# ThomasZiegler/RS-aware-differential-SfM

Hardware: AMD Instinct MI355X
Metric: Mpixels/sec RS depth+pose solve, 1280x720 pair (higher is better)
Workload: dtype f64

## Files before the change

### include/rsdsfm.h

```cpp
#ifndef RSDSFM_H
#define RSDSFM_H

#include <stddef.h>
#include <stdint.h>

#ifdef __cplusplus
extern "C" {
#endif

#define RSDSFM_OK 0
#define RSDSFM_ERR_INVALID (-1)
#define RSDSFM_ERR_HIP (-2)
#define RSDSFM_ERR_NO_DEVICE (-3)
#define RSDSFM_ERR_NUMERIC (-4)
#define RSDSFM_ERR_PENDING (-5)
#define RSDSFM_ERR_PEER (-6)

#define RSDSFM_DEPTH_CLOSED_FORM 0
#define RSDSFM_DEPTH_CERES_LM 1

#define RSDSFM_K_COMPAT 0
#define RSDSFM_K_FIXED 1

#define RSDSFM_FLOW_COMPAT_RANK 0
// ... 82 lines not shown
                  const double v_in[3], const double w_in[3], double k_in, int const_acceleration,
                  int flow_index_mode, double* inliers_out_3m, double v_out[3], double w_out[3], double* k_out,
                  rsdsfm_lm_summary* summary_or_null);
int rsdsfm_last_ransac_tag(rsdsfm_ctx* ctx, uint64_t* tag, int64_t* cache_hits_or_null);
int rsdsfm_refine_from_ransac(rsdsfm_ctx* ctx, uint64_t ransac_tag, const double* flow2n, int64_t n_flow, int64_t m, const double* inliers_3m,
                              const double* alpha_m, const double* alpha_k_m, const int64_t* inlier_idx_or_null, const double v_in[3],
                              const double w_in[3], double k_in, int const_acceleration, int flow_index_mode, double* inliers_out_3m,
                              double v_out[3], double w_out[3], double* k_out, rsdsfm_lm_summary* summary_or_null);
#define RSDSFM_REFINE_TRACE_COLS 8
#define RSDSFM_TRACE_REJECTED 0.0
#define RSDSFM_TRACE_ACCEPTED 1.0
#define RSDSFM_TRACE_INVALID 2.0
#define RSDSFM_TRACE_PARAMETER_TOL 3.0
#define RSDSFM_TRACE_FUNCTION_TOL 4.0
#define RSDSFM_TRACE_ACCEPTED_GRADIENT_TOL 5.0
int rsdsfm_set_refine_trace(rsdsfm_ctx* ctx, int32_t rows);
int rsdsfm_get_refine_trace(rsdsfm_ctx* ctx, double* trace_rows_x_8, int32_t rows);
int rsdsfm_flatten(rsdsfm_ctx* ctx, const double* flow_img_rows_cols_2, int32_t rows, int32_t cols, double fx,
                   double fy, double cx, double cy, double gamma, double flow_threshold, double* q2n,
                   double* u2n, double* alpha_n, double* alpha_k_n, int64_t* n_out);
int rsdsfm_depth_map(rsdsfm_ctx* ctx, double* inliers_3m_inout, int64_t m, double v_inout[3], double fx,
                     double fy, double cx, double cy, int32_t rows, int32_t cols,
                     double* depth_map_colmajor, int32_t* xs_or_null, int32_t* ys_or_null, int* flipped);
int rsdsfm_pose_table(rsdsfm_ctx* ctx, const double v[3], const double w[3], double k, double gamma,
                      int32_t rows, double* R_rows9, double* t_rows3);

int rsdsfm_estimate_inverse_depths_dev(rsdsfm_ctx* ctx, const double* d_q2n, const double* d_u2n, int64_t n,
                                       const double v[3], const double w[3], double k, const double* d_alpha_n,
                                       const double* d_alpha_k_n, int depth_mode, double* d_inv_depth_n);
int rsdsfm_flatten_dev(rsdsfm_ctx* ctx, const double* d_flow_img, int32_t rows, int32_t cols, double fx, double fy,
                       double cx, double cy, double gamma, double flow_threshold, double* d_q2n, double* d_u2n,
                       double* d_alpha_n, double* d_alpha_k_n, int64_t* n_out);
int rsdsfm_depth_map_dev(rsdsfm_ctx* ctx, double* d_inliers_3m_inout, int64_t m, double v_inout[3], double fx, double fy,
                         double cx, double cy, int32_t rows, int32_t cols, double* d_depth_map_colmajor,
                         int32_t* d_xs_or_null, int32_t* d_ys_or_null, int* flipped);
int rsdsfm_pose_table_dev(rsdsfm_ctx* ctx, const double v[3], const double w[3], double k, double gamma, int32_t rows,
                          double* d_R_rows9, double* d_t_rows3);
typedef struct rsdsfm_frame_params {
    int32_t ransac_trials;
    int32_t use_acceleration_mode;
    int32_t use_refinement;
    int32_t depth_mode;
    int32_t k_sign_mode;
    int32_t flow_index_mode;
    int32_t use_global_shutter_mode;
    int32_t struct_bytes;
    double ransac_tol;
    double flow_threshold;
    uint64_t seed;
} rsdsfm_frame_params;

void rsdsfm_frame_params_init(rsdsfm_frame_params* params);

typedef struct rsdsfm_frame_result {
    int64_t n_points, num_inliers;
    int32_t best_trial, flipped;
    double ransac_w[3], ransac_v[3], ransac_k;
    double w[3], v[3], k;
    rsdsfm_lm_summary refine_summary;
    const double* d_inliers;
    const int64_t* d_inlier_idx;
    const int32_t* d_scanline;
} rsdsfm_frame_result;

int rsdsfm_solve_frame_dev(rsdsfm_ctx* ctx, const double* d_flow_img, int32_t rows, int32_t cols, double fx, double fy,
                           double cx, double cy, double gamma, const rsdsfm_frame_params* params,
                           double* d_depth_map_colmajor, double* d_R_rows9_or_null, double* d_t_rows3_or_null,
                           rsdsfm_frame_result* result);
typedef struct rsdsfm_frame_job {
    const double* d_flow_img;
    int32_t rows, cols;
    double fx, fy, cx, cy, gamma;
    double* d_depth_map_colmajor;
    double* d_R_rows9_or_null;
    double* d_t_rows3_or_null;
    uint64_t seed;
} rsdsfm_frame_job;
int rsdsfm_solve_frames_dev(rsdsfm_ctx* ctx, const rsdsfm_frame_job* jobs, int32_t count, const rsdsfm_frame_params* params,
                            rsdsfm_frame_result* results);
int rsdsfm_set_sequence_lanes(rsdsfm_ctx* ctx, int32_t lanes);
int rsdsfm_set_frame_side_flatten(rsdsfm_ctx* ctx, int mode);
int rsdsfm_set_frame_tail(rsdsfm_ctx* ctx, int mode);
int rsdsfm_set_frame_handoff(rsdsfm_ctx* ctx, int mode);
int rsdsfm_set_frame_predict(rsdsfm_ctx* ctx, int mode);
int rsdsfm_lma_predict_stats(rsdsfm_ctx* ctx, int64_t* hypotheses, int64_t* ended_where_predicted);
int rsdsfm_set_lma_operands(rsdsfm_ctx* ctx, int mode);
int rsdsfm_ransac_dev(rsdsfm_ctx* ctx, const double* d_q2n, const double* d_u2n, const double* d_alpha_n,
                      const double* d_alpha_k_n, int64_t n, int use_alpha_k, int32_t iterations, double tolerance,
                      const int32_t* samples_9xT_or_null, uint64_t seed, int depth_mode, int k_sign_mode,
                      rsdsfm_ransac_out* out);
int rsdsfm_refine_dev(rsdsfm_ctx* ctx, const double* d_flow2n, int64_t n_flow, int64_t m, const double* d_inliers_3m,
                      const double* d_alpha_m, const double* d_alpha_k_m, const int64_t* d_inlier_idx_or_null,
                      const double v_in[3], const double w_in[3], double k_in, int const_acceleration,
                      int flow_index_mode, double* d_inliers_out_3m, double v_out[3], double w_out[3], double* k_out,
                      rsdsfm_lm_summary* summary_or_null);
int rsdsfm_estimate_inverse_depths_batch_dev(rsdsfm_ctx* const* ctxs, int32_t count, const double* const* d_q2n,
                                             const double* const* d_u2n, const int64_t* n, const double* v_count_x3,
                                             const double* w_count_x3, const double* k_count, const double* const* d_alpha_n,
                                             const double* const* d_alpha_k_n, double* const* d_inv_depth_n);
int rsdsfm_depth_lm_batch_launch_dev(rsdsfm_ctx* const* ctxs, int32_t count, const double* const* d_q2n, const double* const* d_u2n,
                                     const int64_t* n, const double* v_count_x3, const double* w_count_x3, const double* k_count,
                                     const double* const* d_alpha_n, const double* const* d_alpha_k_n, double* const* d_inv_depth_n);
int rsdsfm_depth_lm_launch_dev(rsdsfm_ctx* ctx, const double* d_q2n, const double* d_u2n, int64_t n,
                               const double v[3], const double w[3], double k, const double* d_alpha_n,
                               const double* d_alpha_k_n, double* d_inv_depth_n, int launch_id);
int rsdsfm_depth_lm_sums_row_size(void);
int rsdsfm_depth_lm_reduce_dev(rsdsfm_ctx* ctx, int64_t n_shard, double* d_row_out);
int rsdsfm_depth_lm_decide_rows_dev(rsdsfm_ctx* ctx, const double* d_rows, int32_t nrows, int64_t n_total, int launch_id);
int rsdsfm_depth_lm_state(rsdsfm_ctx* ctx, int32_t* status, int32_t* next_launch, rsdsfm_lm_summary* summary_or_null);
int rsdsfm_depth_finish_dev(rsdsfm_ctx* ctx, const double* d_q2n, const double* d_u2n, int64_t n,
                            const double v[3], const double w[3], double k, const double* d_alpha_n,
                            const double* d_alpha_k_n, double* d_inv_depth_n, rsdsfm_lm_summary* summary_or_null,
                            int32_t* extra_launches);

int rsdsfm_flatten_slab_dev(rsdsfm_ctx* ctx, const double* d_img_slab, int32_t rows, int32_t slab_cols, int32_t col0,
                            double fx, double fy, double cx, double cy, double gamma, double thr, double* d_q2n,
                            double* d_u2n, double* d_alpha_n, double* d_alpha_k_n, int64_t* n_out);
int rsdsfm_sample_indices(int64_t n, int32_t iterations, uint64_t seed, int32_t* samples);
int rsdsfm_minimal9_dev(rsdsfm_ctx* ctx, const double* d_q9, const double* d_u9, const double* d_alpha9,
                        const double* d_alpha_k9, int32_t count, int use_alpha_k, int k_sign_mode, double* d_hyp);
int rsdsfm_minimal9_probe_dev(rsdsfm_ctx* ctx, const double* d_q9, const double* d_u9, const double* d_alpha9, const double* d_alpha_k9,
                              int32_t count, int use_alpha_k, int k_sign_mode, int use_cores, double* d_hyp, double* d_probe4);
size_t rsdsfm_tile_lm_state_bytes(void);
size_t rsdsfm_tile_best_bytes(void);
int32_t rsdsfm_tile_ransac_row_size(void);
int32_t rsdsfm_tile_ransac_batch(void);
int rsdsfm_tile_ransac_lm_rows_dev(rsdsfm_ctx* ctx, const double* d_q2n, const double* d_u2n, const double* d_alpha_n,
                                   const double* d_alpha_k_n, int64_t n_shard, const double* d_hyp, int32_t count,
                                   const void* d_states, int32_t round, double tolerance, double* d_rows);
int rsdsfm_tile_ransac_decide_dev(rsdsfm_ctx* ctx, const double* d_rows_all, int32_t nranks, int32_t count, void* d_states,
                                  int64_t n_total, int32_t round, int32_t* d_flags, int32_t* d_scored, double* d_trial_count,
                                  double* d_trial_err);
int rsdsfm_tile_ransac_score_rows_dev(rsdsfm_ctx* ctx, const double* d_q2n, const double* d_u2n, const double* d_alpha_n,
                                      const double* d_alpha_k_n, int64_t n_shard, const double* d_hyp, int32_t count,
                                      const void* d_states, int depth_mode, double tolerance, const int32_t* d_scored_or_null,
                                      double* d_rows);
int rsdsfm_tile_ransac_score_merge_dev(rsdsfm_ctx* ctx, const double* d_rows_all, int32_t nranks, int32_t count,
                                       const int32_t* d_scored_or_null, double* d_trial_count, double* d_trial_err);
int rsdsfm_tile_ransac_pick_dev(rsdsfm_ctx* ctx, const double* d_trial_count, const double* d_trial_err, int32_t iterations,
                                const double* d_hyp, void* d_best);
int rsdsfm_tile_ransac_final_dev(rsdsfm_ctx* ctx, const double* d_q2n, const double* d_u2n, const double* d_alpha_n,
                                 const double* d_alpha_k_n, int64_t n_shard, void* d_best, const void* d_states, int depth_mode,
                                 double tolerance, double* d_inv_depth_n, uint8_t* d_mask_n, int64_t* d_inlier_idx,
                                 double* d_inliers3m, double* d_out_alpha, double* d_out_alpha_k, rsdsfm_ransac_out* out);
int64_t rsdsfm_tile_ransac_global_inliers(rsdsfm_ctx* ctx, const void* d_best);
int rsdsfm_tile_refine_begin_dev(rsdsfm_ctx* ctx, const double* d_flow2n, int64_t n_flow, int64_t m_shard, const double* d_inl3m,
                                 const double* d_alpha_m, const double* d_alpha_k_m, const int64_t* d_inlier_idx,
                                 const double v_in[3], const double w_in[3], double k_in, int const_acceleration,
                                 int flow_index_mode);
int32_t rsdsfm_tile_refine_row_size(int const_acceleration, int32_t stage);
int rsdsfm_tile_refine_rows_dev(rsdsfm_ctx* ctx, int32_t stage, double* d_row);
int rsdsfm_tile_refine_apply_dev(rsdsfm_ctx* ctx, int32_t stage, const double* d_rows_all, int32_t nranks, int64_t m_total);
int rsdsfm_tile_refine_poll(rsdsfm_ctx* ctx, double v_out[3], double w_out[3], double* k_out, rsdsfm_lm_summary* summary);
int rsdsfm_tile_refine_finish_dev(rsdsfm_ctx* ctx, double* d_inl_out3m);
int rsdsfm_tile_zsum_dev(rsdsfm_ctx* ctx, const double* d_inl3m, int64_t m_shard, double* d_zsum1);
int rsdsfm_tile_depth_map_dev(rsdsfm_ctx* ctx, double* d_inl3m, int64_t m_shard, const double* d_zsums_all, int32_t nranks,
                              int64_t m_total, double v_inout[3], double fx, double fy, double cx, double cy, int32_t rows,
                              int32_t col0, int32_t slab_cols, double* d_depth_slab, int32_t* d_xs_or_null,
                              int32_t* d_ys_or_null, int* flipped);

#define RSDSFM_DIST_ID_BYTES 128
int rsdsfm_dist_unique_id(void* id_128_bytes);
int rsdsfm_dist_init(rsdsfm_ctx* ctx, int32_t nranks, int32_t rank, const void* id_128_bytes);
int rsdsfm_dist_adopt(rsdsfm_ctx* ctx, void* nccl_comm, int32_t nranks, int32_t rank);
typedef int (*rsdsfm_all_gather_fn)(void* user, const void* d_send, void* d_recv, size_t bytes_per_rank, void* hip_stream);
typedef int (*rsdsfm_all_reduce_sum_f64_fn)(void* user, double* d_buf, size_t count, void* hip_stream);
// ... 78 lines not shown
```

### rs-aware-differential-sfm_amd/csrc/capi.hip

```cpp
#include <string.h>

#include <algorithm>
#include <new>
#include <vector>

#include <chrono>
#include <thread>

#include "rsdsfm_internal.hpp"

namespace rsdsfm {

int fail(Ctx* c, int code, const char* msg) {
    if (c) c->err = msg;
    return code;
}

int ensure_stage(Ctx* c, size_t bytes) {
    c->stage_gen += 1;
    if (bytes <= c->stage_bytes) return RSDSFM_OK;
    RSDSFM_HIP_CHECK(c, hipStreamSynchronize(c->stream));
    if (c->d_stage) RSDSFM_HIP_CHECK(c, hipFree(c->d_stage));
    c->d_stage = nullptr;
    c->stage_bytes = 0;
// ... 126 lines not shown
              hipHostMalloc(reinterpret_cast<void**>(&c->h_lm), sizeof(LmState), hipHostMallocDefault) == hipSuccess &&
              hipMemset(c->d_tickets, 0, sizeof(unsigned) * 64) == hipSuccess &&
              hipMemset(c->d_lm, 0, sizeof(LmState)) == hipSuccess;
    if (ok) {
        memset(c->h_lm, 0, sizeof(LmState));
        c->h_lm->predict = 1;
        c->h_lm->status = 1;
        ok = hipMemcpy(c->d_lm, c->h_lm, sizeof(LmState), hipMemcpyHostToDevice) == hipSuccess;
    }
    if (!ok) {
        rsdsfm_destroy(ctx);
        return RSDSFM_ERR_HIP;
    }
    *out = ctx;
    return RSDSFM_OK;
}

void rsdsfm_destroy(rsdsfm_ctx* ctx) {
    if (!ctx) return;
    Ctx* c = &ctx->c;
    DeviceGuard device_guard_(c);
    (void)hipSetDevice(c->device);
    if (c->stream) (void)hipStreamSynchronize(c->stream);
    frame_release(c);
    flow_release(c);
    flow_check_release(c);
    rectify_dense_release(c);
    link_release(c);
    fuse_release(c);
    last_frame_release(c);
    if (c->d_partials) (void)hipFree(c->d_partials);
    if (c->d_tickets) (void)hipFree(c->d_tickets);
    if (c->d_lm) (void)hipFree(c->d_lm);
    if (c->h_lm) (void)hipHostFree(c->h_lm);
    if (c->d_stage) (void)hipFree(c->d_stage);
    if (c->d_ws) (void)hipFree(c->d_ws);
    if (c->d_frame) (void)hipFree(c->d_frame);
    if (c->d_tile) (void)hipFree(c->d_tile);
    if (c->d_refine_trace) (void)hipFree(c->d_refine_trace);
    if (c->d_core_flag) (void)hipFree(c->d_core_flag);
    delete static_cast<RefineBuffers*>(c->tile_session);
    if (c->h_pinned) (void)hipHostFree(c->h_pinned);
    dist_release(c);
    for (unsigned* p : c->d_claim)
        if (p) (void)hipFree(p);
    if (c->ev_ready) (void)hipEventDestroy(c->ev_ready);
    for (hipEvent_t e : c->ev_prof)
        if (e) (void)hipEventDestroy(e);
    if (c->d_clk_probe) (void)hipFree(c->d_clk_probe);
    if (c->d_lma_list) (void)hipFree(c->d_lma_list);
    if (c->own_stream && c->stream) (void)hipStreamDestroy(c->stream);
    delete ctx;
}

const char* rsdsfm_last_error(const rsdsfm_ctx* ctx) { return ctx ? ctx->c.err.c_str() : "null context"; }

int rsdsfm_synchronize(rsdsfm_ctx* ctx) {
    CTX_OR_FAIL(ctx);
    RSDSFM_HIP_CHECK(c, hipStreamSynchronize(c->stream));
    return RSDSFM_OK;
}

int rsdsfm_set_depth_variant(rsdsfm_ctx* ctx, int variant) {
    CTX_OR_FAIL(ctx);
    if (variant < 0 || variant > 3) return fail(c, RSDSFM_ERR_INVALID, "depth variant must be 0 (default), 1 (LDS-DMA), 2 (decision fused into launch 0) or 3 (separate decide kernel)");
    RSDSFM_HIP_CHECK(c, hipStreamSynchronize(c->stream));
    c->depth_variant = variant;
    return RSDSFM_OK;
}

int rsdsfm_set_profiling(rsdsfm_ctx* ctx, int on) {
    CTX_OR_FAIL(ctx);
    if (on && !c->ev_prof[0]) {
        RSDSFM_HIP_CHECK(c, hipEventCreate(&c->ev_prof[0]));
        RSDSFM_HIP_CHECK(c, hipEventCreate(&c->ev_prof[1]));
        RSDSFM_HIP_CHECK(c, hipMalloc((void**)&c->d_clk_probe, 4 * sizeof(unsigned long long)));
        RSDSFM_HIP_CHECK(c, hipMemsetAsync(c->d_clk_probe, 0, 4 * sizeof(unsigned long long), c->stream));
    }
    c->profile = on != 0;
    c->prof_pending = false;
    return RSDSFM_OK;
}

int rsdsfm_profile_last_ms(rsdsfm_ctx* ctx, const char* what, double* ms) {
    CTX_OR_FAIL(ctx);
    if (what && ms && !strncmp(what, "refine_rf_phase", 15) && ((what[15] >= '0' && what[15] <= '9') || (what[15] >= 'a' && what[15] <= 'f')) && !what[16]) {
        static unsigned long long h[16];
        if (what[15] == '0') {
            int rc = refine_rf_read_stamps(c, h);
            if (rc != RSDSFM_OK) return fail(c, RSDSFM_ERR_INVALID, "no phase stamps: set RSDSFM_RF_STAMPS=1 before the first refinement");
        }
        const int k = what[15] <= '9' ? what[15] - '0' : what[15] - 'a' + 10;
        *ms = k == 4 ? (double)h[4] : k >= 8 ? (double)(long long)(h[k] - h[8]) * 0.01 : (double)h[k] * 0.01;
        return RSDSFM_OK;
    }
    const bool clock = what && !strcmp(what, "ransac_lm_round0_clock_mhz");
    const int which = !what ? -1 : clock || !strcmp(what, "ransac_lm_round0") ? 0 : !strcmp(what, "depth_lm_batch") ? 1 : -1;
    if (which < 0 || !ms)
        return fail(c, RSDSFM_ERR_INVALID, "unknown profile record (known: \"ransac_lm_round0\", \"ransac_lm_round0_clock_mhz\", \"depth_lm_batch\")");
    if (!c->prof_pending || c->prof_what != which)
        return fail(c, RSDSFM_ERR_INVALID, "no such profile record: enable rsdsfm_set_profiling and run a RANSAC (LM mode) / a batched dense depth solve first");
    RSDSFM_HIP_CHECK(c, hipEventSynchronize(c->ev_prof[1]));
    if (clock) {
        unsigned long long h[4];
        RSDSFM_HIP_CHECK(c, hipMemcpyAsync(h, c->d_clk_probe, sizeof(h), hipMemcpyDeviceToHost, c->stream));
        RSDSFM_HIP_CHECK(c, hipStreamSynchronize(c->stream));
        if (h[3] <= h[1] || h[2] <= h[0]) return fail(c, RSDSFM_ERR_INVALID, "the bracketed launch left no clock stamps");
        *ms = (double)(h[2] - h[0]) * 100.0 / (double)(h[3] - h[1]);
        return RSDSFM_OK;
    }
    float f = 0.f;
    RSDSFM_HIP_CHECK(c, hipEventElapsedTime(&f, c->ev_prof[0], c->ev_prof[1]));
    *ms = (double)f;
    return RSDSFM_OK;
}

int rsdsfm_set_refine_trace(rsdsfm_ctx* ctx, int32_t rows) {
    CTX_OR_FAIL(ctx);
    if (rows < 0 || rows > 4096) return fail(c, RSDSFM_ERR_INVALID, "refine trace: 0 <= rows <= 4096");
    if (rows != c->refine_trace_rows) {
        RSDSFM_HIP_CHECK(c, hipStreamSynchronize(c->stream));
        if (c->d_refine_trace) RSDSFM_HIP_CHECK(c, hipFree(c->d_refine_trace));
        c->d_refine_trace = nullptr;
        c->refine_trace_rows = 0;
        if (rows > 0) {
            RSDSFM_HIP_CHECK(c, hipMalloc((void**)&c->d_refine_trace, (size_t)rows * kRefineTraceCols * sizeof(double)));
            c->refine_trace_rows = rows;
        }
    }
    if (c->d_refine_trace)
        RSDSFM_HIP_CHECK(c, hipMemsetAsync(c->d_refine_trace, 0xFF, (size_t)rows * kRefineTraceCols * sizeof(double), c->stream));
    return RSDSFM_OK;
}

int rsdsfm_get_refine_trace(rsdsfm_ctx* ctx, double* out, int32_t rows) {
    CTX_OR_FAIL(ctx);
    if (!out || rows < 1) return fail(c, RSDSFM_ERR_INVALID, "refine trace: null output or rows < 1");
    if (!c->d_refine_trace) return fail(c, RSDSFM_ERR_INVALID, "no refine trace: call rsdsfm_set_refine_trace(ctx, rows) before the refinement");
    if (rows > c->refine_trace_rows) return fail(c, RSDSFM_ERR_INVALID, "refine trace: more rows requested than rsdsfm_set_refine_trace reserved");
    RSDSFM_HIP_CHECK(c, hipMemcpyAsync(out, c->d_refine_trace, (size_t)rows * kRefineTraceCols * sizeof(double), hipMemcpyDeviceToHost, c->stream));
    RSDSFM_HIP_CHECK(c, hipStreamSynchronize(c->stream));
    return RSDSFM_OK;
}

int rsdsfm_set_ransac_speculation(rsdsfm_ctx* ctx, int k0) {
    CTX_OR_FAIL(ctx);
    if (k0 != 0 && k0 != 2 && k0 != KMAX) return fail(c, RSDSFM_ERR_INVALID, "ransac speculation depth must be 0 (automatic, default), 2 or 3");
    c->ransac_k0 = k0;
    return RSDSFM_OK;
}

int rsdsfm_set_ransac_math(rsdsfm_ctx* ctx, int mode) {
    CTX_OR_FAIL(ctx);
    if (mode < 0 || mode > 1) return fail(c, RSDSFM_ERR_INVALID, "ransac math: 0 = in-range function cores with restart (default), 1 = standard functions");
    c->ransac_math_mode = mode;
    return RSDSFM_OK;
}

int rsdsfm_ransac_restarts(rsdsfm_ctx* ctx, int64_t* count) {
    CTX_OR_FAIL(ctx);
    if (!count) return fail(c, RSDSFM_ERR_INVALID, "ransac restarts: null output");
    int64_t total = c->ransac_restarts;
    for (rsdsfm_ctx* lane : c->lanes) total += lane->c.ransac_restarts;
    *count = total;
    return RSDSFM_OK;
}

int rsdsfm_set_lm_arithmetic(rsdsfm_ctx* ctx, int mode) {
    CTX_OR_FAIL(ctx);
    if (mode < 0 || mode > 2)
        return fail(c, RSDSFM_ERR_INVALID, "LM arithmetic: 0 = analytic trajectory with guards (default), 1 = iterate by iterate, 2 = 0 with the frame solve's count-only pass forced");
    c->lm_arithmetic = mode == 1 ? 1 : 0;
    c->lma_count_only_force = mode == 2;
    c->lma_hold = c->lma_unique_run = 0;
    dist_reset_hold(c);
    for (rsdsfm_ctx* lane : c->lanes)
        lane->c.lm_arithmetic = c->lm_arithmetic, lane->c.lma_count_only_force = c->lma_count_only_force, lane->c.lma_hold = lane->c.lma_unique_run = 0;
    return RSDSFM_OK;
}

int rsdsfm_lma_count_only(rsdsfm_ctx* ctx, int64_t* runs, int64_t* lazy_runs) {
    CTX_OR_FAIL(ctx);
    if (!runs) return fail(c, RSDSFM_ERR_INVALID, "lma count only: null output");
    int64_t a = c->lma_count_only_runs, b = c->lma_lazy_runs;
    for (rsdsfm_ctx* lane : c->lanes) a += lane->c.lma_count_only_runs, b += lane->c.lma_lazy_runs;
    *runs = a;
    if (lazy_runs) *lazy_runs = b;
    return RSDSFM_OK;
}

int rsdsfm_lma_predict_stats(rsdsfm_ctx* ctx, int64_t* hypotheses, int64_t* ended_where_predicted) {
    CTX_OR_FAIL(ctx);
    if (!hypotheses || !ended_where_predicted) return fail(c, RSDSFM_ERR_INVALID, "lma predict stats: null output");
    int64_t h = 0, e = 0;
    auto add = [&](Ctx* x) -> int {
        if (!x->d_core_flag) return RSDSFM_OK;
        DeviceGuard guard(x);
        unsigned long long w[2] = {0, 0};
        RSDSFM_HIP_CHECK(c, hipStreamSynchronize(x->stream));
        RSDSFM_HIP_CHECK(c, hipMemcpy(w, x->d_core_flag + 4, sizeof(w), hipMemcpyDeviceToHost));
        h += (int64_t)w[0], e += (int64_t)w[1];
        return RSDSFM_OK;
    };
    int rc = add(c);
    for (rsdsfm_ctx* lane : c->lanes)
        if (rc == RSDSFM_OK) rc = add(&lane->c);
    if (rc != RSDSFM_OK) return rc;
    *hypotheses = h;
    *ended_where_predicted = e;
    return RSDSFM_OK;
}

int rsdsfm_lma_restarts(rsdsfm_ctx* ctx, int64_t* count, int32_t* last_guards) {
    CTX_OR_FAIL(ctx);
    if (!count) return fail(c, RSDSFM_ERR_INVALID, "lma restarts: null output");
    int64_t total = c->lma_restarts;
    int guards = c->lma_last_guard;
    for (rsdsfm_ctx* lane : c->lanes) total += lane->c.lma_restarts, guards |= lane->c.lma_last_guard;
    *count = total;
    if (last_guards) *last_guards = guards;
    return RSDSFM_OK;
}

int rsdsfm_set_refine_arithmetic(rsdsfm_ctx* ctx, int mode) {
    CTX_OR_FAIL(ctx);
    if (mode != 0 && mode != 1) return fail(c, RSDSFM_ERR_INVALID, "refine arithmetic: 0 = radius-factorised (default), 1 = iterate by iterate");
    c->refine_arithmetic = mode;
    for (rsdsfm_ctx* lane : c->lanes) lane->c.refine_arithmetic = mode;
    return RSDSFM_OK;
}

int rsdsfm_refine_restarts(rsdsfm_ctx* ctx, int64_t* runs, int64_t* restarts, int64_t* resolves_or_null, int32_t* last_guard_or_null) {
    CTX_OR_FAIL(ctx);
    if (!runs || !restarts) return fail(c, RSDSFM_ERR_INVALID, "refine restarts: null output");
    int64_t n = c->refine_rf_runs, r = c->refine_rf_restarts, s = c->refine_rf_resolves;
    int guard = c->refine_rf_last_guard;
    for (rsdsfm_ctx* lane : c->lanes) {
        n += lane->c.refine_rf_runs, r += lane->c.refine_rf_restarts, s += lane->c.refine_rf_resolves;
        if (lane->c.refine_rf_last_guard) guard = lane->c.refine_rf_last_guard;
    }
    *runs = n, *restarts = r;
    if (resolves_or_null) *resolves_or_null = s;
    if (last_guard_or_null) *last_guard_or_null = guard;
    return RSDSFM_OK;
}

int rsdsfm_depth_restarts(rsdsfm_ctx* ctx, int64_t* count) {
    CTX_OR_FAIL(ctx);
    if (!count) return fail(c, RSDSFM_ERR_INVALID, "depth restarts: null output");
    *count = c->depth_restarts;
    return RSDSFM_OK;
}

int rsdsfm_set_true_flow_search(rsdsfm_ctx* ctx, int mode) {
    CTX_OR_FAIL(ctx);
    if (mode < 0 || mode > 2) return fail(c, RSDSFM_ERR_INVALID, "true-flow search mode: 0 = automatic, 1 = exhaustive, 2 = interval-pruned");
    c->true_flow_exhaustive = mode;
    return RSDSFM_OK;
}

const char* rsdsfm_kernel_name(const char* entry_point) {
    if (!entry_point) return "";
    if (!strcmp(entry_point, "estimate_inverse_depths_lm")) return RSDSFM_FUSED ? "depth_lm_kernel<1, false>" : "depth_lm_kernel<1, true>";
    if (!strcmp(entry_point, "estimate_inverse_depths_closed_form")) return "depth_closed_form_kernel";
    return "";
}

int rsdsfm_estimate_inverse_depths_dev(rsdsfm_ctx* ctx, const double* d_q, const double* d_u, int64_t n,
                                       const double v[3], const double w[3], double k, const double* d_alpha,
                                       const double* d_alpha_k, int depth_mode, double* d_rho) {
    CTX_OR_FAIL(ctx);
    if (n < 0 || !v || !w) return fail(c, RSDSFM_ERR_INVALID, "bad arguments");
    if (n > 0 && (!d_q || !d_u || !d_alpha || !d_alpha_k || !d_rho)) return fail(c, RSDSFM_ERR_INVALID, "null device pointer");
    if (!aligned_to(16, d_q, d_u, d_alpha, d_alpha_k, d_rho)) return fail(c, RSDSFM_ERR_INVALID, "device pointers must be 16-byte aligned");
    Pose pose;
    memcpy(pose.v, v, sizeof(pose.v));
    memcpy(pose.w, w, sizeof(pose.w));
    pose.k = k;
    if (depth_mode == RSDSFM_DEPTH_CLOSED_FORM) return depth_closed_form_launch(c, d_q, d_u, d_alpha, d_alpha_k, n, pose, d_rho);
    if (depth_mode != RSDSFM_DEPTH_CERES_LM) return fail(c, RSDSFM_ERR_INVALID, "unknown depth_mode");
    if (c->depth_variant == 2) {
        int rcf = depth_lm_fused_launch(c, d_q, d_u, d_alpha, d_alpha_k, n, pose, d_rho);
        if (rcf != RSDSFM_OK) return rcf;
        rcf = depth_lm_launch(c, d_q, d_u, d_alpha, d_alpha_k, n, pose, d_rho, 1);
        c->lm_issued_k = 2;
        c->lm_issued_d = 1;
        return rcf;
    }
    if (depth_lma_allowed(c, n)) {
        Ctx* cs1[1] = {c};
        const double *q1[1] = {d_q}, *u1[1] = {d_u}, *a1[1] = {d_alpha}, *ak1[1] = {d_alpha_k};
        double* r1[1] = {d_rho};
        int rc0 = depth_lma_batch_launch(cs1, 1, q1, u1, a1, ak1, &n, &pose, r1);
        c->lm_issued_k = 1;
        c->lm_issued_d = 1;
        return rc0;
    }
    if (c->depth_variant == 0) {
        int rc0 = depth_lm_launch(c, d_q, d_u, d_alpha, d_alpha_k, n, pose, d_rho, 0, true);
        if (rc0 != RSDSFM_OK) return rc0;
        rc0 = depth_lm_decide_apply_launch(c, d_q, d_u, d_alpha, d_alpha_k, n, pose, d_rho);
        c->lm_issued_k = 1;
        c->lm_issued_d = 1;
        return rc0;
    }
    int rc = depth_lm_launch(c, d_q, d_u, d_alpha, d_alpha_k, n, pose, d_rho, 0);
    if (rc != RSDSFM_OK) return rc;
    rc = depth_lm_decide_launch(c, n, 0);
    if (rc != RSDSFM_OK) return rc;
    rc = depth_lm_launch(c, d_q, d_u, d_alpha, d_alpha_k, n, pose, d_rho, 1);
    c->lm_issued_k = 2;
    c->lm_issued_d = 1;
    return rc;
}

static int depth_batch_common(rsdsfm_ctx* const* ctxs, int32_t count, const double* const* d_q, const double* const* d_u, const int64_t* n,
                              const double* v3, const double* w3, const double* k, const double* const* d_alpha,
                              const double* const* d_alpha_k, double* const* d_rho, int launch0_only) {
    if (!ctxs || count < 1 || !ctxs[0]) return RSDSFM_ERR_INVALID;
    Ctx* c = &ctxs[0]->c;
    DeviceGuard device_guard_(c);
    if (count > kDepthBatchMax) return fail(c, RSDSFM_ERR_INVALID, "at most 8 solves per batched launch");
    if (!d_q || !d_u || !n || !v3 || !w3 || !k || !d_alpha || !d_alpha_k || !d_rho) return fail(c, RSDSFM_ERR_INVALID, "null argument array");
    Ctx* cs[kDepthBatchMax];
    Pose poses[kDepthBatchMax];
    for (int i = 0; i < count; ++i) {
// ... 238 lines not shown
```

### rs-aware-differential-sfm_amd/csrc/frame_host.hip

```cpp
#include <stdlib.h>
#include <string.h>

#include <atomic>

#include <algorithm>
#include <new>

#include "rsdsfm_internal.hpp"
#include "sequence_host.hpp"

namespace rsdsfm {

static std::atomic<int> g_frames_in_flight[64];
int frames_in_flight(const Ctx* c) { return g_frames_in_flight[c->device & 63].load(std::memory_order_relaxed); }

int alpha_ones_launch(Ctx* c, double* d_alpha, int64_t n);
int flatten_device(Ctx* c, const double* d_img, int32_t rows, int32_t cols, int32_t col0, double fx, double fy, double cx, double cy, double gamma,
                   double thr, double* d_q, double* d_u, double* d_alpha, double* d_alpha_k, int64_t* n_out);

struct FrameRun {
    rsdsfm_frame_job job;
    rsdsfm_frame_params prm;
    size_t N = 0;
    int64_t n = 0;
// ... 124 lines not shown
                RSDSFM_HIP_CHECK(c, hipMalloc(reinterpret_cast<void**>(&c->d_flat_counters), 2 * sizeof(unsigned long long)));
                RSDSFM_HIP_CHECK(c, hipMemsetAsync(c->d_flat_counters, 0, 2 * sizeof(unsigned long long), c->stream));
            }
            F->dense = DenseFlatten();
            F->dense.thr = prm->flow_threshold;
            F->dense.d_q = F->d_q, F->dense.d_u = F->d_u, F->dense.d_alpha = F->d_a, F->dense.d_alpha_k = F->d_ak;
            F->dense.d_counters = c->d_flat_counters;
            F->dense.total_out = count_host(c);
            F->dense_in_launch = true;
        } else if (side == 2) {
            F->join = [c, F, d_flat_counts, d_flat_offsets]() -> int {
                const rsdsfm_frame_job& J2 = F->job;
                int rc2 = flatten_launch(c, J2.d_flow_img, J2.rows, J2.cols, 0, J2.fx, J2.fy, J2.cx, J2.cy, J2.gamma, F->prm.flow_threshold, F->d_q, F->d_u, F->d_a,
                                         F->d_ak, d_flat_counts, d_flat_offsets, count_host(c), nullptr);
                if (rc2 == RSDSFM_OK && F->prm.use_global_shutter_mode) rc2 = alpha_ones_launch(c, F->d_a, (int64_t)F->N);
                return rc2;
            };
        } else if (side == 1) {
            rc = ensure_side_stream(c);
            if (rc != RSDSFM_OK) return rc;
            RSDSFM_HIP_CHECK(c, hipEventRecord(c->ev_fork, c->stream));
            RSDSFM_HIP_CHECK(c, hipStreamWaitEvent(c->aux_stream, c->ev_fork, 0));
            {
                StreamSwap on_side(c, c->aux_stream);
                rc = flatten_launch(c, J.d_flow_img, rows, cols, 0, fx, fy, cx, cy, gamma, prm->flow_threshold, F->d_q, F->d_u, F->d_a, F->d_ak,
                                    d_flat_counts, d_flat_offsets, count_host(c), nullptr);
                if (rc == RSDSFM_OK && prm->use_global_shutter_mode) rc = alpha_ones_launch(c, F->d_a, n);
            }
            if (rc != RSDSFM_OK) return rc;
            RSDSFM_HIP_CHECK(c, hipEventRecord(c->ev_join, c->aux_stream));
            F->join = [c]() -> int {
                RSDSFM_HIP_CHECK(c, hipStreamWaitEvent(c->stream, c->ev_join, 0));
                return RSDSFM_OK;
            };
        } else {
            rc = flatten_enqueue(c, J.d_flow_img, rows, cols, fx, fy, cx, cy, gamma, prm->flow_threshold, F->d_q, F->d_u, F->d_a, F->d_ak, count_host(c));
            if (rc != RSDSFM_OK) return rc;
        }
    } else {
        rc = flatten_device(c, J.d_flow_img, rows, cols, 0, fx, fy, cx, cy, gamma, prm->flow_threshold, F->d_q, F->d_u, F->d_a, F->d_ak, &n);
        if (rc != RSDSFM_OK) return rc;
        *count_host(c) = n;
    }
    if (prm->use_global_shutter_mode && !F->side_flatten) {
        rc = alpha_ones_launch(c, F->d_a, n);
        if (rc != RSDSFM_OK) return rc;
    }
    F->n = n;
    memset(&F->ro, 0, sizeof(F->ro));
    F->ro.inlier_idx = F->d_idx;
    F->ro.inliers = F->d_inl;
    F->ro.alpha = F->d_in_a;
    F->ro.alpha_k = F->d_in_ak;
    F->ro.mask = F->d_mask;
    F->m_known = -1;
    F->tail = [c, F](const RefineBuffers& B) -> int {
        const rsdsfm_frame_job& J2 = F->job;
        const RefineState* st = B.state;
        const int64_t m_arg = F->m_known >= 0 ? F->m_known : F->n;
        const int64_t* m_dev = F->m_known >= 0 ? nullptr : &st->m;
        PoseTableOut pt;
        if (J2.d_R_rows9_or_null && J2.d_t_rows3_or_null)
            pt.R = J2.d_R_rows9_or_null, pt.t = J2.d_t_rows3_or_null, pt.rows = J2.rows, pt.gamma = J2.gamma, pt.wk_dev = st->p + 3;
        if (B.claim.on)
            return depth_map_decided_launch(c, F->d_inl_ref, m_arg, F->d_zpartials, refine_finish_grid(c, B), B, J2.d_depth_map_colmajor, F->d_zheader,
                                            header_host(c), st->p, m_dev, &pt);
        return depth_map_slab_launch(c, F->d_inl_ref, m_arg, F->d_zpartials, refine_finish_grid(c, B), m_arg, nullptr, J2.fx, J2.fy, J2.cx, J2.cy, J2.rows,
                                     0, J2.cols, J2.d_depth_map_colmajor, nullptr, F->d_ys, F->d_zheader, header_host(c), st->p, m_dev, &pt);
    };
    F->claim = FinishClaim();
    if (c->frame_tail == 0) {
        F->claim.on = true;
        F->claim.fx = J.fx, F->claim.fy = J.fy, F->claim.cx = J.cx, F->claim.cy = J.cy;
        F->claim.rows = rows, F->claim.cols = cols;
        F->claim.ys = F->d_ys;
    }
    F->spec_tail = [c, F](const RansacBest* d_best) -> int {
        return refine_begin(c, F->d_u, F->n, F->n, F->d_inl, F->d_in_a, F->d_in_ak, F->d_idx, nullptr, nullptr, 0.0, F->prm.use_acceleration_mode,
                            F->prm.flow_index_mode, F->d_inl_ref, &F->tail, d_best, F->d_refine_ws, &F->refine, state_host(c), F->d_zpartials, false,
                            &F->claim, F->ransac.direct_final ? &F->ransac.handoff : nullptr);
    };
    F->refinement_enqueued = false;
    F->ahead = prm->use_refinement && c->ransac_spec_miss < 2;
    F->d_local_idx = (c->frame_handoff == 0 && F->ahead && F->claim.on && c->lm_arithmetic == 0 && c->refine_arithmetic == 0 && !c->refine_stage_separate)
                         ? d_local_idx : nullptr;
    F->open = true;
    g_frames_in_flight[c->device & 63].fetch_add(1, std::memory_order_relaxed);
    F->counted = true;
    F->rc_begin = ransac_begin(c, F->d_q, F->d_u, F->d_a, F->d_ak, n, prm->use_acceleration_mode, prm->ransac_trials, prm->ransac_tol, nullptr, J.seed,
                               prm->depth_mode, prm->k_sign_mode, &F->ro, prm->use_refinement ? &F->spec_tail : nullptr, &F->refinement_enqueued, &F->ransac,
                               F->side_flatten ? &F->direct : nullptr, F->side_flatten && !F->dense_in_launch ? &F->join : nullptr,
                               F->dense_in_launch ? &F->dense : nullptr, F->ahead, true,
                               F->claim.on && prm->use_refinement ? refine_flag_words(F->d_refine_ws) : nullptr, F->d_local_idx);
    return RSDSFM_OK;
}

int frame_finish(Ctx* c, FrameRun* F, rsdsfm_frame_result* res) {
    if (!F->open) return fail(c, RSDSFM_ERR_INVALID, "no frame solve in flight");
    F->open = false;
    FrameInFlightEnd in_flight_end_{c, F};
    const rsdsfm_frame_job& J = F->job;
    const rsdsfm_frame_params* prm = &F->prm;
    memset(res, 0, sizeof(*res));
    int rc = F->rc_begin;
    if (rc == RSDSFM_OK) rc = ransac_finish(c, &F->ransac);
    if (rc != RSDSFM_OK) RSDSFM_HIP_CHECK(c, hipStreamSynchronize(c->stream));
    if (F->side_flatten && c->aux_stream) RSDSFM_HIP_CHECK(c, hipStreamSynchronize(c->aux_stream));
    int64_t n = F->n;
    if (*count_host(c) < 0) {
        c->frame_dense_hint = 1;
        return rc != RSDSFM_OK ? rc : fail(c, RSDSFM_ERR_NUMERIC, "frame solve: the point count did not arrive");
    }
    bool counted = true;
    if (*count_host(c) != n) {
        if (F->dense_in_launch) {
            int64_t n_real = 0;
            rc = flatten_device(c, J.d_flow_img, J.rows, J.cols, 0, J.fx, J.fy, J.cx, J.cy, J.gamma, prm->flow_threshold, F->d_q, F->d_u, F->d_a, F->d_ak, &n_real);
            if (rc == RSDSFM_OK && prm->use_global_shutter_mode) rc = alpha_ones_launch(c, F->d_a, n_real);
            if (rc != RSDSFM_OK) return rc;
            *count_host(c) = n_real;
        }
        n = *count_host(c);
        F->n = n;
        F->refinement_enqueued = false;
        counted = false;
        rc = ransac_begin(c, F->d_q, F->d_u, F->d_a, F->d_ak, n, prm->use_acceleration_mode, prm->ransac_trials, prm->ransac_tol, nullptr, J.seed,
                          prm->depth_mode, prm->k_sign_mode, &F->ro, prm->use_refinement ? &F->spec_tail : nullptr, &F->refinement_enqueued, &F->ransac, nullptr, nullptr,
                          nullptr, F->ahead, true,
                               F->claim.on && prm->use_refinement ? refine_flag_words(F->d_refine_ws) : nullptr, F->d_local_idx);
        if (rc == RSDSFM_OK) rc = ransac_finish(c, &F->ransac);
        counted = rc == RSDSFM_OK;
    }
    c->frame_dense_hint = n == (int64_t)F->N ? 1 : 0;
    if (rc != RSDSFM_OK) return rc;
    if (counted) ransac_commit_hints(c, F->ransac);
    const rsdsfm_ransac_out& ro = F->ro;
    res->n_points = n;
    res->num_inliers = ro.num_inliers;
    res->best_trial = ro.best_trial;
    memcpy(res->ransac_w, ro.w, sizeof(ro.w));
    memcpy(res->ransac_v, ro.v, sizeof(ro.v));
    res->ransac_k = ro.k;
    double v[3], w[3], k = ro.k;
    for (int i = 0; i < 3; ++i) v[i] = ro.v[i], w[i] = ro.w[i];
    double* d_final = F->d_inl;
    int flipped = 0;
    F->m_known = ro.num_inliers;
    if (prm->use_refinement) {
        bool exact = false;
        if (F->refinement_enqueued) {
            rc = refine_poll(c, &F->refine, v, w, &k, &res->refine_summary);
            exact = rc == kRcRefineRestartExact;
        }
        if ((!F->refinement_enqueued || exact) && F->ransac.direct_final) {
            rc = ransac_scatter_launch(c, F->ransac.handoff);
            if (rc != RSDSFM_OK) return rc;
            F->ransac.direct_final = false;
        }
        if (!F->refinement_enqueued || exact)
            rc = refine_device(c, F->d_u, n, ro.num_inliers, F->d_inl, F->d_in_a, F->d_in_ak, F->d_idx, v, w, k, prm->use_acceleration_mode,
                               prm->flow_index_mode, F->d_inl_ref, v, w, &k, &res->refine_summary, &F->tail, F->d_zpartials, exact, &F->claim);
        if (rc != RSDSFM_OK) return rc;
        d_final = F->d_inl_ref;
        const double* h_header = header_host(c);
        flipped = h_header[0] != 0.0;
        v[0] = h_header[1], v[1] = h_header[2], v[2] = h_header[3];
    } else {
        rc = depth_map_device(c, d_final, ro.num_inliers, v, J.fx, J.fy, J.cx, J.cy, J.rows, J.cols, J.d_depth_map_colmajor, nullptr, F->d_ys, &flipped, w,
                              k, J.gamma, J.d_R_rows9_or_null, J.d_t_rows3_or_null);
        if (rc != RSDSFM_OK) return rc;
    }
    res->flipped = flipped;
    memcpy(res->v, v, sizeof(v));
    memcpy(res->w, w, sizeof(w));
    res->k = k;
    res->d_inliers = d_final;
    res->d_inlier_idx = F->d_idx;
    res->d_scanline = F->d_ys;
    return RSDSFM_OK;
}

FrameRun* frame_run_of(Ctx* c) {
    if (!c->frame_run) c->frame_run = new (std::nothrow) FrameRun();
    return static_cast<FrameRun*>(c->frame_run);
}

}

void frame_release(Ctx* c) {
    frame_uncount(c, static_cast<FrameRun*>(c->frame_run));
    delete static_cast<FrameRun*>(c->frame_run);
    c->frame_run = nullptr;
    for (rsdsfm_ctx* lane : c->lanes) rsdsfm_destroy(lane);
    c->lanes.clear();
    if (c->ev_fork) (void)hipEventDestroy(c->ev_fork);
    if (c->ev_join) (void)hipEventDestroy(c->ev_join);
    if (c->ev_seq) (void)hipEventDestroy(c->ev_seq);
    if (c->aux_stream) (void)hipStreamDestroy(c->aux_stream);
    if (c->d_flat_counters) (void)hipFree(c->d_flat_counters);
    c->d_flat_counters = nullptr;
    c->ev_fork = c->ev_join = c->ev_seq = nullptr;
    c->aux_stream = nullptr;
}

}

using namespace rsdsfm;

extern "C" {

void rsdsfm_frame_params_init(rsdsfm_frame_params* p) {
    if (!p) return;
    memset(p, 0, sizeof(*p));
    p->ransac_trials = 5;
    p->use_acceleration_mode = 0;
    p->use_refinement = 1;
    p->depth_mode = RSDSFM_DEPTH_CERES_LM;
    p->k_sign_mode = RSDSFM_K_COMPAT;
    p->flow_index_mode = RSDSFM_FLOW_COMPAT_RANK;
    p->use_global_shutter_mode = 0;
    p->struct_bytes = (int32_t)sizeof(rsdsfm_frame_params);
    p->ransac_tol = 0.05;
    p->flow_threshold = 1e-10;
    p->seed = 1;
}

int rsdsfm_solve_frame_dev(rsdsfm_ctx* ctx, const double* d_flow_img, int32_t rows, int32_t cols, double fx, double fy, double cx,
                           double cy, double gamma, const rsdsfm_frame_params* prm, double* d_depth_map, double* d_R_rows9,
                           double* d_t_rows3, rsdsfm_frame_result* res) {
    if (!ctx) return RSDSFM_ERR_INVALID;
    Ctx* c = &ctx->c;
    DeviceGuard device_guard_(c);
    if (!prm || !res) return fail(c, RSDSFM_ERR_INVALID, "bad arguments");
    FrameRun* F = frame_run_of(c);
// ... 1 lines not shown
    F->prm = *prm;
    F->job = rsdsfm_frame_job{d_flow_img, rows, cols, fx, fy, cx, cy, gamma, d_depth_map, d_R_rows9, d_t_rows3, prm->seed};
    int rc = frame_begin(c, F);
    if (rc != RSDSFM_OK) return rc;
    return frame_finish(c, F, res);
}

int rsdsfm_set_sequence_lanes(rsdsfm_ctx* ctx, int32_t lanes) {
    if (!ctx) return RSDSFM_ERR_INVALID;
    Ctx* c = &ctx->c;
    DeviceGuard device_guard_(c);
    if (lanes < 0 || lanes > 16) return fail(c, RSDSFM_ERR_INVALID, "lanes must be 0 (default) .. 16");
    c->seq_lanes = lanes;
    return RSDSFM_OK;
}

int rsdsfm_set_frame_tail(rsdsfm_ctx* ctx, int mode) {
    if (!ctx) return RSDSFM_ERR_INVALID;
    if (mode < 0 || mode > 1) return fail(&ctx->c, RSDSFM_ERR_INVALID, "mode must be 0 (short launch tail) or 1 (stage-by-stage launches)");
    ctx->c.frame_tail = mode;
    return RSDSFM_OK;
}

int rsdsfm_set_frame_handoff(rsdsfm_ctx* ctx, int mode) {
    if (!ctx) return RSDSFM_ERR_INVALID;
    if (mode < 0 || mode > 1) return fail(&ctx->c, RSDSFM_ERR_INVALID, "mode must be 0 (the first refinement pass gathers its inliers) or 1 (the compaction launch)");
    ctx->c.frame_handoff = mode;
    return RSDSFM_OK;
}

int rsdsfm_set_frame_predict(rsdsfm_ctx* ctx, int mode) {
    if (!ctx) return RSDSFM_ERR_INVALID;
    if (mode < 0 || mode > 2) return fail(&ctx->c, RSDSFM_ERR_INVALID, "mode must be 0 (the pixel pass fuses each hypothesis' predicted iterate), 1 (the two-iterate pass) or 2 (0 with the prediction inverted)");
    ctx->c.frame_predict = mode;
    for (rsdsfm_ctx* lane : ctx->c.lanes) lane->c.frame_predict = mode;
    return RSDSFM_OK;
}

int rsdsfm_set_lma_operands(rsdsfm_ctx* ctx, int mode) {
    if (!ctx) return RSDSFM_ERR_INVALID;
    if (mode < 0 || mode > 2) return fail(&ctx->c, RSDSFM_ERR_INVALID, "mode must be 0 (the pixel pass stages each pixel's operands once per workgroup), 1 (every lane loads its pixel's operands) or 2 (0 for every hypothesis count)");
    ctx->c.lma_operands = mode;
    for (rsdsfm_ctx* lane : ctx->c.lanes) lane->c.lma_operands = mode;
    return RSDSFM_OK;
}

int rsdsfm_set_frame_side_flatten(rsdsfm_ctx* ctx, int mode) {
    if (!ctx) return RSDSFM_ERR_INVALID;
    if (mode < 0 || mode > 3) return fail(&ctx->c, RSDSFM_ERR_INVALID, "mode must be 0 (flatten first), 1 (flatten on a second stream), 2 (flatten behind the minimal solver) or 3 (flatten inside the solver's launch)");
    ctx->c.frame_side_flatten = mode;
    return RSDSFM_OK;
}

}

namespace rsdsfm {

int sequence_lane_count(const Ctx* c, int count) { return std::max(1, std::min<int>(count, c->seq_lanes > 0 ? c->seq_lanes : kSequenceLanesDefault)); }

int solve_frames_run(Ctx* c, const rsdsfm_frame_job* jobs, int32_t count, const rsdsfm_frame_params* prm, rsdsfm_frame_result* results, const PairHook* hook) {
    const int L = sequence_lane_count(c, count);
    while ((int)c->lanes.size() < L - 1) {
        rsdsfm_ctx* lane = nullptr;
        int rc = rsdsfm_create(&lane, c->device, nullptr);
        if (rc != RSDSFM_OK) return fail(c, rc, "could not create a sequence lane");
        c->lanes.push_back(lane);
    }
    auto lane_ctx = [&](int l) -> Ctx* { return l == 0 ? c : &c->lanes[(size_t)l - 1]->c; };
    if (L > 1) {
        if (!c->ev_seq) RSDSFM_HIP_CHECK(c, hipEventCreateWithFlags(&c->ev_seq, hipEventDisableTiming));
        RSDSFM_HIP_CHECK(c, hipEventRecord(c->ev_seq, c->stream));
    }
    for (int l = 1; l < L; ++l) {
        Ctx* lc = lane_ctx(l);
        RSDSFM_HIP_CHECK(c, hipStreamWaitEvent(lc->stream, c->ev_seq, 0));
        lc->ransac_k0 = c->ransac_k0;
        lc->ransac_math_mode = c->ransac_math_mode;
        lc->lm_arithmetic = c->lm_arithmetic;
        lc->refine_arithmetic = c->refine_arithmetic;
        lc->lma_count_only_force = c->lma_count_only_force;
        lc->frame_side_flatten = c->frame_side_flatten;
        lc->frame_tail = c->frame_tail;
        lc->frame_handoff = c->frame_handoff;
        lc->frame_predict = c->frame_predict;
        lc->lma_operands = c->lma_operands;
        lc->refine_stage_mode = c->refine_stage_mode;
    }
    for (int l = 0; l < L; ++l) lane_ctx(l)->refine_stage_separate = L > 1;
    int first_error = RSDSFM_OK;
    int in_flight[16];
    for (int l = 0; l < 16; ++l) in_flight[l] = -1;
    auto finish_lane = [&](int l) {
        const int i = in_flight[l];
        if (i < 0) return;
        in_flight[l] = -1;
        Ctx* lc = lane_ctx(l);
        int rc = frame_finish(lc, static_cast<FrameRun*>(lc->frame_run), &results[i]);
        if (rc != RSDSFM_OK && first_error == RSDSFM_OK) {
            first_error = rc;
            if (lc != c) c->err = "pair " + std::to_string(i) + ": " + lc->err;
        }
        if (rc == RSDSFM_OK && hook && first_error == RSDSFM_OK) {
            rc = (*hook)(lc, i, static_cast<FrameRun*>(lc->frame_run)->job, results[i]);
            if (rc != RSDSFM_OK) {
                first_error = rc;
                c->err = "pair " + std::to_string(i) + ": " + std::string(lc->err);
            }
        }
    };
    for (int i = 0; i < count && first_error == RSDSFM_OK; ++i) {
        const int l = i % L;
        finish_lane(l);
        if (first_error != RSDSFM_OK) break;
        Ctx* lc = lane_ctx(l);
        FrameRun* F = frame_run_of(lc);
        if (!F) {
            first_error = fail(c, RSDSFM_ERR_INVALID, "out of host memory");
            break;
        }
        F->prm = *prm;
        F->job = jobs[i];
        int rc = frame_begin(lc, F);
        if (rc != RSDSFM_OK) {
            first_error = rc;
            if (lc != c) c->err = "pair " + std::to_string(i) + ": " + lc->err;
            break;
        }
        in_flight[l] = i;
    }
    for (;;) {
        int best = -1;
        for (int l = 0; l < L; ++l)
            if (in_flight[l] >= 0 && (best < 0 || in_flight[l] < in_flight[best])) best = l;
        if (best < 0) break;
        finish_lane(best);
    }
    for (int l = 0; l < L; ++l) lane_ctx(l)->refine_stage_separate = false;
    return first_error;
}

}

extern "C" {

int rsdsfm_solve_frames_dev(rsdsfm_ctx* ctx, const rsdsfm_frame_job* jobs, int32_t count, const rsdsfm_frame_params* prm, rsdsfm_frame_result* results) {
    if (!ctx) return RSDSFM_ERR_INVALID;
    Ctx* c = &ctx->c;
    DeviceGuard device_guard_(c);
    if (count < 0 || !prm || (count > 0 && (!jobs || !results))) return fail(c, RSDSFM_ERR_INVALID, "bad arguments");
    if (count == 0) return RSDSFM_OK;
    for (int32_t i = 0; i < count; ++i)
        if (frame_job_check_aligned(c, jobs[i]) != RSDSFM_OK) return RSDSFM_ERR_INVALID;
    return solve_frames_run(c, jobs, count, prm, results, nullptr);
}

int rsdsfm_set_refine_stage(rsdsfm_ctx* ctx, int mode) {
    if (!ctx) return RSDSFM_ERR_INVALID;
    Ctx* c = &ctx->c;
    if (mode < 0 || mode > 2) return fail(c, RSDSFM_ERR_INVALID, "refine stage: 0 (automatic), 1 (in the next pass's prologue) or 2 (a launch of its own)");
    c->refine_stage_mode = mode;
    return RSDSFM_OK;
}

}
```

### rs-aware-differential-sfm_amd/csrc/refine_common.hpp

```cpp
#pragma once
#include "device_math.hpp"
#include "rsdsfm_internal.hpp"

namespace rsdsfm {
namespace {


constexpr int kFB = 512;
constexpr int kWorkgroupsPerCu = 1;

struct PassShape {
    int64_t m;
    int grid;
    bool live;
};
__device__ __forceinline__ PassShape pass_shape(const RefineState* __restrict__ st, int64_t m_arg) {
    PassShape ps;
    if (m_arg >= 0) {
        ps.m = m_arg, ps.grid = (int)gridDim.x, ps.live = true;
    } else {
        ps.m = st->m, ps.grid = st->grid, ps.live = (int)blockIdx.x < ps.grid;
    }
    return ps;
}
// ... 215 lines not shown
    __syncthreads();
    (void)s_red;
}

template <int NA, int NB>
__device__ __forceinline__ bool reduce_two_ranges_groups(const double* __restrict__ rows, int nblocks, int stride, int offA, int maxA, bool doA,
                                                         double (*s_grpA)[NA], int offB, int maxB, bool doB, double (*s_grpB)[NB], int tid) {
    using SA = ReduceShape<NA>;
    using SB = ReduceShape<NB>;
    static_assert(SA::W == 2 && SB::W == 2, "slot pairs");
    constexpr int U = 16;
    if (nblocks > U * SA::G || nblocks > U * SB::G) return false;
    const int gA = tid / SA::NH, spA = tid - gA * SA::NH, gB = tid / SB::NH, spB = tid - gB * SB::NH;
    const bool onA = doA && gA < SA::G, onB = doB && gB < SB::G;
    double2 vA[U], vB[U];
#pragma unroll
    for (int j = 0; j < U; ++j) {
        const int bj = gA + j * SA::G;
        vA[j] = (onA && bj < nblocks) ? reinterpret_cast<const double2*>(rows + (int64_t)bj * stride + offA)[spA] : make_double2(0.0, 0.0);
    }
#pragma unroll
    for (int j = 0; j < U; ++j) {
        const int bj = gB + j * SB::G;
        vB[j] = (onB && bj < nblocks) ? reinterpret_cast<const double2*>(rows + (int64_t)bj * stride + offB)[spB] : make_double2(0.0, 0.0);
    }
    if (onA) {
        const bool mx0 = (2 * spA == maxA), mx1 = (2 * spA + 1 == maxA);
        double a0 = 0.0, a1 = 0.0;
#pragma unroll
        for (int j = 0; j < U; ++j) {
            a0 = mx0 ? fmax(a0, vA[j].x) : a0 + vA[j].x;
            a1 = mx1 ? fmax(a1, vA[j].y) : a1 + vA[j].y;
        }
        s_grpA[gA][2 * spA] = a0;
        s_grpA[gA][2 * spA + 1] = a1;
    }
    if (onB) {
        const bool mx0 = (2 * spB == maxB), mx1 = (2 * spB + 1 == maxB);
        double a0 = 0.0, a1 = 0.0;
#pragma unroll
        for (int j = 0; j < U; ++j) {
            a0 = mx0 ? fmax(a0, vB[j].x) : a0 + vB[j].x;
            a1 = mx1 ? fmax(a1, vB[j].y) : a1 + vB[j].y;
        }
        s_grpB[gB][2 * spB] = a0;
        s_grpB[gB][2 * spB + 1] = a1;
    }
    return true;
}

template <int NP>
struct Counts {
    static constexpr int TRI = NP * (NP + 1) / 2;
    static constexpr int NINIT = 1 + NP + NP + 1 + 1 + 1;
    static constexpr int INIT_MAX = 1 + 2 * NP;
    static constexpr int NSCHUR = 2 * TRI + 2 * NP;
    static constexpr int NBACK = 3 + 1 + NP + 1 + 1 + 1 + 1;
    static constexpr int BACK_MAX = 3 + 1 + NP;
};

template <int NP>
struct SlotRow {
    using CT = Counts<NP>;
    static constexpr int OFF_BACK = CT::NSCHUR;
    static constexpr int NW = CT::NSCHUR + CT::NBACK + ((CT::NBACK & 1) ? 1 : 0);
    static constexpr bool SPECULATES = NP == 6;
};


__device__ __forceinline__ double uniform_d(double x) {
    const int lo = __builtin_amdgcn_readfirstlane(__double2loint(x)), hi = __builtin_amdgcn_readfirstlane(__double2hiint(x));
    return __hiloint2double(hi, lo);
}

__device__ __forceinline__ void state_to_lds(RefineState* s_st, const RefineState* __restrict__ st_in) {
    static_assert(sizeof(RefineState) % 8 == 0 && sizeof(RefineState) / 8 <= kFB, "copied as 8-byte words, one per thread");
    if (threadIdx.x < sizeof(RefineState) / 8) reinterpret_cast<double*>(s_st)[threadIdx.x] = reinterpret_cast<const double*>(st_in)[threadIdx.x];
    __syncthreads();
}
__device__ __forceinline__ void state_from_lds(RefineState* __restrict__ st_out, const RefineState* s_st) {
    if (threadIdx.x < sizeof(RefineState) / 8) reinterpret_cast<double*>(st_out)[threadIdx.x] = reinterpret_cast<const double*>(s_st)[threadIdx.x];
}

}
}
```

### rs-aware-differential-sfm_amd/csrc/refine_host.hip

```cpp
#include <string.h>

#include <algorithm>

#include "rsdsfm_internal.hpp"

namespace rsdsfm {

int refine_begin(Ctx* c, const double* d_flow, int64_t n_flow, int64_t m, const double* d_inl, const double* d_alpha,
                 const double* d_alpha_k, const int64_t* d_inlier_idx, const double v_in[3], const double w_in[3], double k_in,
                 int const_acceleration, int flow_index_mode, double* d_inl_out, const RefineTail* tail, const RansacBest* d_best,
                 void* ws_base, RefineRun* run, RefineState* hs_prefetch, double* d_zpartials, bool exact, const FinishClaim* claim,
                 const FrameHandoff* handoff) {
    const bool direct = handoff && handoff->local_idx;
    if (m < 0 || n_flow < 0 || (!d_best && (!v_in || !w_in))) return fail(c, RSDSFM_ERR_INVALID, "bad arguments");
    if (flow_index_mode != RSDSFM_FLOW_COMPAT_RANK && flow_index_mode != RSDSFM_FLOW_GATHERED) return fail(c, RSDSFM_ERR_INVALID, "unknown flow_index_mode");
    if (flow_index_mode == RSDSFM_FLOW_GATHERED && m > 0 && !d_inlier_idx) return fail(c, RSDSFM_ERR_INVALID, "gathered mode needs inlier_idx");
    if (m > 0 && (!d_flow || !d_inl || !d_alpha || !d_alpha_k || !d_inl_out)) return fail(c, RSDSFM_ERR_INVALID, "null device pointer");
    const int np = const_acceleration ? 7 : 6;
    const size_t M = (size_t)std::max<int64_t>(m, 1);
    const size_t npart = (size_t)(d_best ? refine_partials_doubles_cap(c) : refine_partials_doubles(c, m));
    int rc = RSDSFM_OK;
    if (!ws_base) {
        rc = ensure_ws(c, refine_workspace_bytes(c, m, d_best != nullptr));
        if (rc != RSDSFM_OK) return rc;
        ws_base = c->d_ws;
    }
    rc = ensure_pinned(c, sizeof(RefineState) + 64);
    if (rc != RSDSFM_OK) return rc;
    Arena ws(ws_base);
    RefineBuffers& B = run->B;
    B = RefineBuffers();
    B.flow = d_flow;
    B.n_flow = n_flow;
    B.m = m;
    B.m_on_device = d_best != nullptr;
    B.inl = d_inl;
    B.alpha = d_alpha;
    B.alpha_k = d_alpha_k;
    B.inlier_idx = d_inlier_idx;
    B.flow_index_mode = flow_index_mode;
    static_assert(sizeof(RefineState) % sizeof(int) == 0, "flag follows the state");
    char* state_block = ws.take<char>(sizeof(RefineState) + 64);
    B.state = reinterpret_cast<RefineState*>(state_block);
    B.uu = ws.take<double>(4 * M);
    B.beta = ws.take<double>(M);
    B.rho_a = ws.take<double>(M);
    B.rho_b = ws.take<double>(M);
    B.srho = ws.take<double>(M);
    B.partials = ws.take<double>(npart);
    B.bad_index = reinterpret_cast<int*>(state_block + sizeof(RefineState));
    B.zpartials = d_zpartials;
    if (claim && claim->on && d_zpartials) B.claim = *claim;
    run->np = np;
    run->rf = !exact && c->lm_arithmetic == 0 && c->refine_arithmetic == 0;
    if (run->rf) c->refine_rf_runs += 1;
    run->d_inl_out = d_inl_out;
    run->tail = tail;
    run->launched = 0;
    run->hint_prev = c->refine_iters_hint;
    run->hs = hs_prefetch ? hs_prefetch : static_cast<RefineState*>(c->h_pinned);
    run->prefetch = hs_prefetch != nullptr;
    run->prefetched = false;
    B.state_host = hs_prefetch;
    if (d_best && claim && claim->on && run->rf && !c->refine_stage_separate) {
        B.best_dev = d_best;
        if (direct) {
            B.handoff = *handoff;
            B.fin_xy = B.uu, B.fin_stride = 4;
        }
    } else if (direct) {
        return fail(c, RSDSFM_ERR_INVALID, "refinement: direct hand-off without the start state in the first pass");
    } else if (d_best) {
        rc = refine_state_from_best_launch(c, d_best, B, np);
        if (rc != RSDSFM_OK) return rc;
    } else {
        RefineState* hs = static_cast<RefineState*>(c->h_pinned);
        int* h_bad = reinterpret_cast<int*>(static_cast<char*>(c->h_pinned) + sizeof(RefineState));
        memset(hs, 0, sizeof(RefineState));
        hs->np = np;
        for (int i = 0; i < 3; ++i) {
            hs->p[i] = v_in[i];
            hs->p[3 + i] = w_in[i];
        }
        hs->p[6] = k_in;
        hs->termination = -1;
        hs->radius = kInitialRadius;
        hs->need_schur = 1;
        memset(h_bad, 0, kRefineStateBlockTail);
        RSDSFM_HIP_CHECK(c, hipMemcpyAsync(B.state, hs, sizeof(RefineState) + kRefineStateBlockTail, hipMemcpyHostToDevice, c->stream));
    }
    rc = refine_trace_reset(c);
    if (rc != RSDSFM_OK) return rc;
    if (!run->rf) {
        rc = refine_init_launch(c, B, np);
        if (rc != RSDSFM_OK) return rc;
    }
    const int hp = run->hint_prev;
    run->chunk = (hp >= 0 && hp <= 3) ? hp + 1 : (hp > 8 ? std::min(hp + 1, 28) : 7);
    return refine_enqueue_chunk(c, run);
}

int refine_enqueue_chunk(Ctx* c, RefineRun* run) {
    static const bool watch = getenv("RSDSFM_SYNC_WATCHDOG_S") != nullptr;
    if (watch) {
        const RefineBuffers B = run->B;
        const int launched = run->launched, chunk = run->chunk, rf = run->rf ? 1 : 0;
        set_sync_dumper([B, launched, chunk, rf](Ctx* cc) {
            fprintf(stderr, "[rsdsfm] last refinement chunk enqueued: slots [%d, %d), radius-factorised %d\n", launched, launched + chunk, rf);
            refine_rf_debug_dump(cc, B);
        });
    }
    if (run->rf) {
        for (int i = 0; i <= run->chunk; ++i) {
            const int g = run->launched + i;
            int rc = refine_rf_pass_launch(c, run->B, run->np, g, run->launched, nullptr, 0, -1, nullptr, i == run->chunk);
            if (rc != RSDSFM_OK) return rc;
        }
        run->launched += 1;
    } else {
        for (int i = 0; i < run->chunk; ++i) {
            int rc = refine_iter_launch(c, run->B, run->np, i, run->chunk);
            if (rc != RSDSFM_OK) return rc;
        }
    }
    run->launched += run->chunk;
    int rc = RSDSFM_OK;
    if (run->B.claim.on) {
        FinishClaim& C = run->B.claim;
        const int64_t npix = (int64_t)C.rows * C.cols;
        if (run->B.m >= ((int64_t)1 << 31)) return fail(c, RSDSFM_ERR_INVALID, "depth map: more than 2^31 inliers");
        rc = claim_map_acquire(c, 2, (size_t)std::max<int64_t>(std::max<int64_t>(npix, run->B.m), 1), &C.owner, &C.tag, &C.mask);
        if (rc != RSDSFM_OK) return rc;
    }
    rc = refine_finish_launch(c, run->B, run->d_inl_out);
    if (rc != RSDSFM_OK) return rc;
    run->tail_done = false;
    if (run->tail && !(run->hint_prev > run->launched + 1)) {
        rc = (*run->tail)(run->B);
        run->tail_done = true;
    }
    if (rc != RSDSFM_OK) return rc;
    if (run->prefetch) run->prefetched = true;
    return rc;
}

int refine_poll(Ctx* c, RefineRun* run, double v_out[3], double w_out[3], double* k_out, rsdsfm_lm_summary* summary) {
    if (!v_out || !w_out || !k_out) return fail(c, RSDSFM_ERR_INVALID, "bad arguments");
    RefineState* hs = run->hs;
    int* h_bad = reinterpret_cast<int*>(reinterpret_cast<char*>(hs) + sizeof(RefineState));
    for (bool first = true;; first = false) {
        if (!(first && run->prefetch && run->prefetched)) {
            if (!run->prefetch) RSDSFM_HIP_CHECK(c, hipMemcpyAsync(hs, run->B.state, sizeof(RefineState) + sizeof(int), hipMemcpyDeviceToHost, c->stream));
            if (int rcs = sync_stream(c, "refine_poll line 168")) return rcs;
        }
        if (*h_bad) return fail(c, RSDSFM_ERR_INVALID, "flow index out of range (flow has fewer columns than inliers / bad inlier_idx)");
        if (hs->termination == kTermRestartExact) {
            c->refine_rf_restarts += 1;
            c->refine_rf_last_guard = hs->rf_guard;
            return kRcRefineRestartExact;
        }
        if (hs->termination >= 0) {
            if (run->tail && !run->tail_done) {
                int rc = (*run->tail)(run->B);
                if (rc != RSDSFM_OK) return rc;
                run->tail_done = true;
                if (int rcs = sync_stream(c, "refine_poll line 181")) return rcs;
            }
            break;
        }
        if (run->launched > 8 * kMaxIter + 16) return fail(c, RSDSFM_ERR_NUMERIC, "refinement did not terminate");
        run->chunk = std::min(8, std::max(2, run->hint_prev - run->launched));
        int rc = refine_enqueue_chunk(c, run);
        if (rc != RSDSFM_OK) return rc;
    }
    c->refine_iters_hint = hs->slots;
    if (run->rf) c->refine_rf_resolves += hs->rf_resolves;
    for (int i = 0; i < 3; ++i) {
        v_out[i] = hs->p[i];
        w_out[i] = hs->p[3 + i];
    }
    *k_out = hs->p[6];
    if (summary) {
        summary->num_iterations = hs->iteration;
        summary->num_successful_steps = hs->num_successful;
        summary->num_unsuccessful_steps = hs->num_unsuccessful;
        summary->termination = hs->termination;
        summary->initial_cost = hs->initial_cost;
        summary->final_cost = hs->cost;
        summary->final_radius = hs->radius;
    }
    return RSDSFM_OK;
}

int* refine_flag_words(void* ws_base) {
    Arena ws(ws_base);
    return reinterpret_cast<int*>(ws.take<char>(sizeof(RefineState) + 64) + sizeof(RefineState));
}

size_t refine_workspace_bytes(const Ctx* c, int64_t m, bool m_on_device) {
    const size_t M = (size_t)std::max<int64_t>(m, 1);
    const size_t npart = (size_t)(m_on_device ? refine_partials_doubles_cap(c) : refine_partials_doubles(c, m));
    return Arena::need(sizeof(RefineState) + 64) + Arena::need(32 * M) + 4 * Arena::need(8 * M) + Arena::need(8 * npart) + Arena::need(64) + 1024;
}

int refine_device(Ctx* c, const double* d_flow, int64_t n_flow, int64_t m, const double* d_inl, const double* d_alpha,
                  const double* d_alpha_k, const int64_t* d_inlier_idx, const double v_in[3], const double w_in[3], double k_in,
                  int const_acceleration, int flow_index_mode, double* d_inl_out, double v_out[3], double w_out[3], double* k_out,
                  rsdsfm_lm_summary* summary, const RefineTail* tail, double* d_zpartials, bool exact, const FinishClaim* claim) {
    if (!v_out || !w_out || !k_out) return fail(c, RSDSFM_ERR_INVALID, "bad arguments");
    const double v0[3] = {v_in[0], v_in[1], v_in[2]}, w0[3] = {w_in[0], w_in[1], w_in[2]};
    for (int attempt = 0;; ++attempt) {
        RefineRun run;
        int rc = refine_begin(c, d_flow, n_flow, m, d_inl, d_alpha, d_alpha_k, d_inlier_idx, v0, w0, k_in, const_acceleration, flow_index_mode,
                              d_inl_out, tail, nullptr, nullptr, &run, nullptr, d_zpartials, exact || attempt > 0, claim);
        if (rc != RSDSFM_OK) return rc;
        rc = refine_poll(c, &run, v_out, w_out, k_out, summary);
        if (rc != kRcRefineRestartExact || attempt > 0) return rc == kRcRefineRestartExact ? fail(c, RSDSFM_ERR_NUMERIC, "refinement: restart loop") : rc;
    }
}

}

using namespace rsdsfm;

extern "C" {

int rsdsfm_refine_dev(rsdsfm_ctx* ctx, const double* d_flow, int64_t n_flow, int64_t m, const double* d_inl, const double* d_alpha,
                      const double* d_alpha_k, const int64_t* d_inlier_idx, const double v_in[3], const double w_in[3], double k_in,
                      int const_acceleration, int flow_index_mode, double* d_inl_out, double v_out[3], double w_out[3], double* k_out,
                      rsdsfm_lm_summary* summary) {
    if (!ctx) return RSDSFM_ERR_INVALID;
    DeviceGuard device_guard_(&ctx->c);
    if (!aligned_to(16, d_flow) || !aligned_to(8, d_inl, d_alpha, d_alpha_k, d_inlier_idx, d_inl_out))
        return fail(&ctx->c, RSDSFM_ERR_INVALID, "refine: the flow must be 16-byte aligned, the inlier arrays 8-byte aligned");
    return refine_device(&ctx->c, d_flow, n_flow, m, d_inl, d_alpha, d_alpha_k, d_inlier_idx, v_in, w_in, k_in, const_acceleration,
                         flow_index_mode, d_inl_out, v_out, w_out, k_out, summary, nullptr, nullptr);
}

// ... 82 lines not shown
```

### rs-aware-differential-sfm_amd/csrc/refine_kernels.hip

```cpp
#include "refine_common.hpp"

namespace rsdsfm {


template <int NP>
__global__ __launch_bounds__(kFB) void refine_init_kernel(const double2* __restrict__ flow, int64_t n_flow, int64_t m,
                                                         const double* __restrict__ inl, const double* __restrict__ alpha,
                                                         const double* __restrict__ alpha_k,
                                                         const int64_t* __restrict__ inlier_idx, int flow_index_mode,
                                                         const RefineState* __restrict__ st, double4* __restrict__ xyuv,
                                                         double* __restrict__ beta_out, double* __restrict__ rho0,
                                                         double* __restrict__ srho, double* __restrict__ partials,
                                                         int* __restrict__ bad_index, int want_zsum) {
    using CT = Counts<NP>;
    __shared__ double s_red[kFB / 64][CT::NINIT];
    const PassShape ps = pass_shape(st, m);
    if (!ps.live) return;
    m = ps.m;
    double p[7];
#pragma unroll
    for (int c = 0; c < 7; ++c) p[c] = st->p[c];
    double acc[CT::NINIT];
#pragma unroll
    for (int s = 0; s < CT::NINIT; ++s) acc[s] = 0.0;
// ... 366 lines not shown
        }
        st->cur ^= 1;
        st->zsum = s[CT::BACK_MAX + 2];
        st->cost = 0.5 * s[3];
        st->gmax = gmax;
        st->x_norm = sqrt(xsq);
        st->radius = radius_accept(st->radius, rel);
        st->decrease_factor = 2.0;
        st->num_successful += 1;
        if (gmax <= kGradientTol) st->termination = RSDSFM_TERM_GRADIENT;
        if (tr) tr[7] = gmax <= kGradientTol ? RSDSFM_TRACE_ACCEPTED_GRADIENT_TOL : RSDSFM_TRACE_ACCEPTED;
    } else {
        if (tr) tr[7] = RSDSFM_TRACE_REJECTED;
        st->num_unsuccessful += 1;
        st->radius = st->radius / st->decrease_factor;
        st->decrease_factor *= 2.0;
    }
    return st->termination < 0 && st->num_successful > successful_before ? 1 : 0;
}

template <int NP>
__global__ __launch_bounds__(kFB) void refine_decide_kernel(const double* __restrict__ partials, int nblocks,
                                                           RefineState* st, double* __restrict__ trace, int trace_rows) {
    using CT = Counts<NP>;
    __shared__ double s_red[kFB / 64][CT::NBACK];
    __shared__ double s[CT::NBACK];
    if (st->termination >= 0) return;
    const int solve_ok = st->solve_ok;
    if (solve_ok) reduce_partials<CT::NBACK>(partials, nblocks >= 0 ? nblocks : st->grid, CT::BACK_MAX, s_red, s);
    if (threadIdx.x != 0) return;
    (void)decide_serial<NP>(st, s, solve_ok, trace, trace_rows);
}

__global__ __launch_bounds__(kFB) void refine_finish_kernel(int64_t m, const double* __restrict__ inl,
                                                           const double* __restrict__ rho_a, const double* __restrict__ rho_b,
                                                           const RefineState* __restrict__ st, double* __restrict__ inl_out,
                                                           double* __restrict__ zpartials, RefineState* __restrict__ state_host,
                                                           const int* __restrict__ bad_index) {
    __shared__ double s_red[kFB / 64];
    if (state_host && blockIdx.x == 0) {
        static_assert(sizeof(RefineState) % 8 == 0, "copied as 8-byte words");
        for (int i = threadIdx.x; i < (int)(sizeof(RefineState) / 8); i += kFB)
            reinterpret_cast<double*>(state_host)[i] = reinterpret_cast<const double*>(st)[i];
        if (threadIdx.x == 0) *reinterpret_cast<int*>(reinterpret_cast<char*>(state_host) + sizeof(RefineState)) = *bad_index;
    }
    const double* __restrict__ rho = st->cur ? rho_b : rho_a;
    if (m < 0) m = st->m;
    const int64_t stride = (int64_t)gridDim.x * kFB;
    double acc = 0.0;
    for (int64_t i = (int64_t)blockIdx.x * kFB + threadIdx.x; i < m; i += stride) {
        inl_out[3 * i] = inl[3 * i];
        inl_out[3 * i + 1] = inl[3 * i + 1];
        const double z = 1.0 / rho[i];
        inl_out[3 * i + 2] = z;
        acc += z;
    }
    if (zpartials) {
        const double r = wave_sum(acc);
        if ((threadIdx.x & 63) == 0) s_red[threadIdx.x >> 6] = r;
        __syncthreads();
        if (threadIdx.x == 0) {
            double t = s_red[0];
            for (int w2 = 1; w2 < kFB / 64; ++w2) t += s_red[w2];
            zpartials[blockIdx.x] = t;
        }
    }
}

__global__ __launch_bounds__(kFB) void refine_finish_claim_kernel(int64_t m, const double* __restrict__ inl, const double* __restrict__ rho_a,
                                                                 const double* __restrict__ rho_b, const RefineState* __restrict__ st,
                                                                 double* __restrict__ inl_out, double* __restrict__ zpartials,
                                                                 RefineState* __restrict__ state_host, const int* __restrict__ bad_index,
                                                                 double fx, double fy, double cx, double cy, int rows, int ncols,
                                                                 unsigned* __restrict__ owner, unsigned tag, int32_t* __restrict__ ys,
                                                                 int xy_stride) {
    __shared__ double s_red[kFB / 64];
    if (state_host && blockIdx.x == 0) {
        for (int i = threadIdx.x; i < (int)(sizeof(RefineState) / 8); i += kFB)
            reinterpret_cast<double*>(state_host)[i] = reinterpret_cast<const double*>(st)[i];
        if (threadIdx.x == 0) *reinterpret_cast<int*>(reinterpret_cast<char*>(state_host) + sizeof(RefineState)) = *bad_index;
    }
    const double* __restrict__ rho = st->cur ? rho_b : rho_a;
    if (m < 0) m = st->m;
    const int64_t stride = (int64_t)gridDim.x * kFB;
    double acc = 0.0;
    for (int64_t i = (int64_t)blockIdx.x * kFB + threadIdx.x; i < m; i += stride) {
        const double xn = inl[xy_stride * i], yn = inl[xy_stride * i + 1];
        inl_out[3 * i] = xn;
        inl_out[3 * i + 1] = yn;
        const double z = 1.0 / rho[i];
        inl_out[3 * i + 2] = z;
        acc += z;
        const int x = (int)(fx * xn + cx + 0.5);
        const int y = (int)(fy * yn + cy + 0.5);
        ys[i] = y;
        if (x >= 0 && x < ncols && y >= 0 && y < rows) atomicMax(&owner[(int64_t)x * rows + y], tag | (unsigned)i);
    }
    const double r = wave_sum(acc);
    if ((threadIdx.x & 63) == 0) s_red[threadIdx.x >> 6] = r;
    __syncthreads();
    if (threadIdx.x == 0) {
        double t = s_red[0];
        for (int w2 = 1; w2 < kFB / 64; ++w2) t += s_red[w2];
        zpartials[blockIdx.x] = t;
    }
}

__global__ void refine_state_from_best_kernel(const RansacBest* __restrict__ best, RefineState* __restrict__ st, int np, int cap,
                                              int* __restrict__ bad_index) {
    if (threadIdx.x != 0 || blockIdx.x != 0) return;
    RefineState z;
    memset(&z, 0, sizeof(z));
    z.np = np;
    for (int i = 0; i < 3; ++i) {
        z.p[i] = best->hyp[3 + i];
        z.p[3 + i] = best->hyp[i];
    }
    z.p[6] = best->hyp[6];
    z.termination = -1;
    z.radius = kInitialRadius;
    z.need_schur = 1;
    const int64_t m = best->undecided ? 0 : best->num_inliers_scan;
    z.m = m;
    int64_t b = (m + kFB - 1) / kFB;
    if (b < 1) b = 1;
    if (b > cap) {
        const int64_t iters = (b + cap - 1) / cap;
        b = (b + iters - 1) / iters;
    }
    z.grid = (int)b;
    *st = z;
    bad_index[0] = 0;
    bad_index[4] = bad_index[5] = bad_index[6] = 0;
}

static inline int refine_grid_cap(const Ctx* c) { return c->num_cus * kWorkgroupsPerCu; }
static inline int refine_grid(const Ctx* c, int64_t m) {
    int64_t b = (m + kFB - 1) / kFB;
    const int64_t cap = (int64_t)c->num_cus * kWorkgroupsPerCu;
    if (b < 1) b = 1;
    if (b > cap) {
        const int64_t iters = (b + cap - 1) / cap;
        b = (b + iters - 1) / iters;
    }
    return (int)b;
}

static inline int refine_partials_half(const Ctx* c) { return refine_grid_cap(c) * SlotRow<7>::NW; }
constexpr int kStateDoubles = (int)((sizeof(RefineState) + 63) / 64 * 8);
int refine_partials_doubles_cap(const Ctx* c) { return 2 * refine_partials_half(c) + 2 * kStateDoubles + 8 + refine_rf_extra_doubles(); }
int refine_partials_half_doubles(const Ctx* c) { return refine_partials_half(c); }
int refine_state_doubles() { return kStateDoubles; }
int refine_partials_doubles(const Ctx* c, int64_t m) { (void)m; return refine_partials_doubles_cap(c); }
static inline double* rows_buffer(const Ctx* c, const RefineBuffers& B, int which) { return B.partials + (size_t)(which & 1) * refine_partials_half(c); }
static inline RefineState* chunk_state(const Ctx* c, const RefineBuffers& B, int which) {
    return reinterpret_cast<RefineState*>(B.partials + 2 * (size_t)refine_partials_half(c) + (size_t)(which & 1) * kStateDoubles);
}
static inline const RefineState* slot_state_in(const Ctx* c, const RefineBuffers& B, int j) { return j == 0 ? B.state : chunk_state(c, B, j - 1); }

int refine_state_from_best_launch(Ctx* c, const RansacBest* d_best, const RefineBuffers& B, int np) {
    hipLaunchKernelGGL(refine_state_from_best_kernel, dim3(1), dim3(64), 0, c->stream, d_best, B.state, np, refine_grid_cap(c), B.bad_index);
    RSDSFM_HIP_CHECK(c, hipGetLastError());
    return RSDSFM_OK;
}

template <int NP>
static int refine_init_t(Ctx* c, const RefineBuffers& B) {
    const int grid = B.m_on_device ? refine_grid_cap(c) : refine_grid(c, B.m);
    const int64_t m_arg = B.m_on_device ? -1 : B.m;
    hipLaunchKernelGGL(refine_init_kernel<NP>, dim3(grid), dim3(kFB), 0, c->stream, reinterpret_cast<const double2*>(B.flow), B.n_flow,
                       m_arg, B.inl, B.alpha, B.alpha_k, B.inlier_idx, B.flow_index_mode, B.state, reinterpret_cast<double4*>(B.uu),
                       B.beta, B.rho_a, B.srho, B.partials, B.bad_index, B.want_zsum ? 1 : 0);
    RSDSFM_HIP_CHECK(c, hipGetLastError());
    hipLaunchKernelGGL(refine_init_decide_kernel<NP>, dim3(1), dim3(kFB), 0, c->stream, B.partials, B.m_on_device ? -1 : grid, B.state, m_arg);
    RSDSFM_HIP_CHECK(c, hipGetLastError());
    return RSDSFM_OK;
}

template <int NV>
__global__ __launch_bounds__(kFB) void refine_row_kernel(const double* __restrict__ partials, int nblocks, int max_slot,
                                                        double* __restrict__ row, const RefineState* __restrict__ st = nullptr) {
    __shared__ double s_red[kFB / 64][NV];
    __shared__ double s[NV];
    if (nblocks < 0) nblocks = st->grid;
    reduce_partials<NV>(partials, nblocks, max_slot, s_red, s);
    if (threadIdx.x < NV) row[threadIdx.x] = s[threadIdx.x];
}

// ... 335 lines not shown
```

### rs-aware-differential-sfm_amd/csrc/refine_rf_kernels.hip

```cpp
#include "refine_common.hpp"

#ifndef RF_LOADS_ONLY
#define RF_LOADS_ONLY 0
#endif
#ifndef RF_NP7_PREFETCH
#define RF_NP7_PREFETCH 0
#endif

namespace rsdsfm {

namespace {

constexpr int kRfListCap = 64;
constexpr int kRfEntry = 8;

template <int NP>
struct RfRow {
    static constexpr int TRI = NP * (NP + 1) / 2;
    static constexpr int OFF_JTJ = 0, OFF_B = TRI, OFF_JTB = 2 * TRI, OFF_C = 2 * TRI + NP;
    static constexpr int NSCHUR = 2 * TRI + 2 * NP;
    static constexpr int MODEL = NSCHUR, STEPSQ = NSCHUR + 1, COST2 = NSCHUR + 2, XSQ = NSCHUR + 3, ZSUM = NSCHUR + 4, GMAX = NSCHUR + 5;
    static constexpr int NW = NSCHUR + 6;
    static constexpr int NF = TRI + NP;
    static_assert(NW % 2 == 0, "rows are read as double2");
};

struct RfExt {
    double sums[RfRow<7>::NSCHUR];
    double nlist;
    double list[kRfListCap * kRfEntry];
};
constexpr int kRfExtDoubles = (int)((sizeof(RfExt) + 63) / 64 * 8);
constexpr int kRfListDoubles = 2 + kRfListCap * kRfEntry;

enum RfGuard : int {
    kRfGuardNonFinite = 1, kRfGuardGradient = 2, kRfGuardModel = 3, kRfGuardParameter = 4, kRfGuardFunction = 5, kRfGuardQuality = 6,
    kRfGuardPivot = 7, kRfGuardList = 8, kRfGuardRadius = 9
};
constexpr double kBandGradient = 1e-4, kBandParameter = 1e-2, kBandFunction = 1e-4, kBandQuality = 1e-4, kBandModel = 1e-12, kBandPivot = 1e-9;

struct RfPoint {
    double v0, v1, v2, w0, w1, w2, k, c1, c2;
};
__device__ __forceinline__ RfPoint rf_point(const double* p) {
    RfPoint P;
    P.v0 = p[0], P.v1 = p[1], P.v2 = p[2], P.w0 = p[3], P.w1 = p[4], P.w2 = p[5], P.k = p[6];
    const double t = 2.0 + p[6];
    P.c1 = 2.0 / t;
    P.c2 = 2.0 / (t * t);
    return P;
}
__device__ __forceinline__ RfPoint rf_point_uniform(const RfPoint& Q) {
    RfPoint P;
    P.v0 = uniform_d(Q.v0), P.v1 = uniform_d(Q.v1), P.v2 = uniform_d(Q.v2), P.w0 = uniform_d(Q.w0), P.w1 = uniform_d(Q.w1), P.w2 = uniform_d(Q.w2);
    P.k = uniform_d(Q.k), P.c1 = uniform_d(Q.c1), P.c2 = uniform_d(Q.c2);
    return P;
}

struct RfGeom {
    double x, y, xy, xx1, yy1;
};
__device__ __forceinline__ RfGeom rf_geom(double x, double y) {
    RfGeom g;
    g.x = x, g.y = y, g.xy = x * y, g.xx1 = __builtin_fma(x, x, 1.0), g.yy1 = __builtin_fma(y, y, 1.0);
    return g;
}
__device__ __forceinline__ void rf_av(const RfGeom& g, double v0, double v1, double v2, double& a0, double& a1) {
    a0 = __builtin_fma(g.x, v2, -v0);
    a1 = __builtin_fma(g.y, v2, -v1);
}
__device__ __forceinline__ void rf_bw(const RfGeom& g, double w0, double w1, double w2, double& b0, double& b1) {
    b0 = __builtin_fma(g.y, w2, __builtin_fma(-g.xx1, w1, g.xy * w0));
    b1 = __builtin_fma(-g.x, w2, __builtin_fma(-g.xy, w1, g.yy1 * w0));
}
template <int NP>
__device__ __forceinline__ void rf_beta(double ab, double ak, const RfPoint& P, double& be, double& dbe) {
    if (NP == 6) {
        be = ab, dbe = 0.0;
    } else {
        be = P.c1 * __builtin_fma(P.k, ak, ab);
        dbe = P.c2 * __builtin_fma(2.0, ak, -ab);
    }
}
__device__ __forceinline__ bool rf_flagged(double h, double h0) { return !(h >= __builtin_fma(2.02e-6, h0, 2.02e-6) && h <= 1e30); }

template <int NP>
struct RfEval {
    double r0, r1, J0, J1, h, in0, in1;
    double P0[NP], P1[NP];
};
template <int NP>
__device__ __forceinline__ void rf_resid(const RfGeom& g, double ux, double uy, double be, const RfPoint& P, double rho, RfEval<NP>& o) {
    double a0, a1, b0, b1;
    rf_av(g, P.v0, P.v1, P.v2, a0, a1);
    rf_bw(g, P.w0, P.w1, P.w2, b0, b1);
    o.in0 = __builtin_fma(rho, a0, b0);
    o.in1 = __builtin_fma(rho, a1, b1);
// ... 181 lines not shown
        for (int a = 0; a < NP; ++a) {
            double ra = __builtin_fma(-psi, cur[RR::OFF_C + a], cur[RR::OFF_JTB + a]);
            if (have_F) ra -= F[RR::TRI + a];
            rhs[a] = ra * sp[a];
#pragma unroll
            for (int b = a; b < NP; ++b) {
                double mab = __builtin_fma(-psi, cur[RR::OFF_B + tri], cur[RR::OFF_JTJ + tri]);
                if (have_F) mab -= F[tri];
                double sab = (mab * sp[a]) * sp[b];
                if (a == b) sab = __builtin_fma(clampd((cur[RR::OFF_JTJ + tri] * sp[a]) * sp[a], kMinLmDiag, kMaxLmDiag), inv_radius, sab);
                S[a][b] = sab;
                S[b][a] = sab;
                ++tri;
            }
        }
    }
    int status = 1;
    double inv_d[NP];
#pragma unroll
    for (int j = 0; j < NP; ++j) {
        if (status == 1) {
            const double sjj = S[j][j];
            double d = sjj;
#pragma unroll
            for (int t = 0; t < j; ++t) d = __builtin_fma(-S[j][t], S[j][t], d);
            if (!(fabs(d) > kBandPivot * fabs(sjj)) || !(fabs(d) > 1e-200 && fabs(d) < 1e200)) {
                status = -1;
            } else if (d < 0.0) {
                status = 0;
            } else {
                const double id = rcp_core(sqrt_core(d));
                inv_d[j] = id;
#pragma unroll
                for (int i = j + 1; i < NP; ++i) {
                    double sacc = S[i][j];
#pragma unroll
                    for (int t = 0; t < j; ++t) sacc = __builtin_fma(-S[i][t], S[j][t], sacc);
                    S[i][j] = sacc * id;
                }
            }
        }
    }
    if (status != 1) return status;
    double yv[NP], yp[NP];
#pragma unroll
    for (int i = 0; i < NP; ++i) {
        double sacc = rhs[i];
#pragma unroll
        for (int t = 0; t < i; ++t) sacc = __builtin_fma(-S[i][t], yv[t], sacc);
        yv[i] = sacc * inv_d[i];
    }
#pragma unroll
    for (int i = NP - 1; i >= 0; --i) {
        double sacc = yv[i];
#pragma unroll
        for (int t = i + 1; t < NP; ++t) sacc = __builtin_fma(-S[t][i], yp[t], sacc);
        yp[i] = sacc * inv_d[i];
    }
    double stepsq = 0.0;
#pragma unroll
    for (int c = 0; c < 7; ++c) st->pc[c] = st->p[c], st->dp[c] = 0.0;
#pragma unroll
    for (int c = 0; c < NP; ++c) {
        const double d = -(yp[c] * sp[c]);
        st->yp[c] = yp[c];
        st->dp[c] = d;
        st->pc[c] = st->p[c] + d;
        stepsq = __builtin_fma(d, d, stepsq);
    }
    st->stepsq_p = stepsq;
    return 1;
}

__device__ __forceinline__ bool rf_in_band(double value, double threshold, double band) { return fabs(value - threshold) <= band * fabs(threshold); }

__device__ __forceinline__ void rf_restart(RefineState* st, int guard) {
    st->termination = kTermRestartExact;
    st->rf_guard = guard;
}

template <int NP>
__device__ __forceinline__ void rf_apply_body(RefineState* st, RfStageLds<NP>& L, const double* __restrict__ rows, int nrows, int row_stride, RfLists lists,
                              const RfExt* __restrict__ ext_in, RfExt* __restrict__ ext_out, int64_t m_total, double* __restrict__ trace, int trace_rows,
                              unsigned long long* tks = nullptr, unsigned long long* beat = nullptr) {
    using RR = RfRow<NP>;
    const int tid = threadIdx.x;
#define RF_BEAT(code) do { if (beat && tid == 0) beat[1] = (beat[1] & ~255ull) | (code); } while (0)
    RF_BEAT(10);
    if (tid == 0) L.bad = 0;
    rf_reduce_rows_groups<RR::NW>(rows, nrows, row_stride, L.grp, tid);
    int ntot = 0;
    bool overflow = false;
    for (int r = 0; r < lists.nlists; ++r) {
        const int n = lists.counts[(size_t)r * lists.count_stride];
        overflow = overflow || n > kRfListCap || n < 0;
        ntot += n;
    }
    overflow = overflow || ntot > kRfListCap;
    __syncthreads();
    reduce_partials_slots<RR::NW>(L.grp, RR::GMAX, L.s, tid);
    if (tid < RR::NW && !(fabs(L.s[tid]) < 1e300)) L.bad = 1;
    __syncthreads();
    if (tks) tks[0] = wall_clock64();
    RF_BEAT(11);
    const bool first = st->iteration == 0 && st->num_unsuccessful == 0 && st->slots == 0;
    if (tid == 0) {
        const double* s = L.s;
        int action = 0;
        st->slots += 1;
        double* tr = (trace && st->iteration >= 1 && st->iteration <= trace_rows) ? trace + (int64_t)(st->iteration - 1) * kRefineTraceCols : nullptr;
        const bool finite = L.bad == 0;
        if (!finite || overflow) {
            rf_restart(st, overflow ? kRfGuardList : kRfGuardNonFinite);
            action = 2;
        } else if (first) {
            double gmax = s[RR::GMAX], xsq = s[RR::XSQ];
            int tri = 0;
#pragma unroll
            for (int c = 0; c < NP; ++c) {
                st->sp[c] = 1.0 / (1.0 + sqrt(s[RR::OFF_JTJ + tri]));
                tri += NP - c;
                gmax = fmax(gmax, fabs(s[RR::OFF_JTB + c]));
                xsq = __builtin_fma(st->p[c], st->p[c], xsq);
            }
            st->cost = 0.5 * s[RR::COST2];
            st->initial_cost = st->cost;
            st->zsum = s[RR::ZSUM];
            st->gmax = gmax;
            st->x_norm = sqrt(xsq);
            st->radius = kInitialRadius;
            st->decrease_factor = 2.0;
            action = 1;
            if (m_total == 0 || gmax <= kGradientTol) st->termination = RSDSFM_TERM_GRADIENT, action = 2;
            if (m_total != 0 && rf_in_band(gmax, kGradientTol, kBandGradient)) rf_restart(st, kRfGuardGradient), action = 2;
        } else {
            const double model_change = s[RR::MODEL];
            if (tr) {
                tr[0] = (double)st->iteration, tr[1] = st->cost, tr[3] = model_change, tr[5] = st->radius;
                tr[2] = tr[4] = tr[6] = __builtin_nan("");
            }
            if (fabs(model_change) <= kBandModel * st->cost) {
                rf_restart(st, kRfGuardModel);
                action = 2;
            } else if (!(model_change > 0.0)) {
                if (tr) tr[7] = RSDSFM_TRACE_INVALID;
                st->num_unsuccessful += 1;
                st->invalid_run += 1;
                if (st->invalid_run >= kMaxInvalid)
                    st->termination = RSDSFM_TERM_FAILURE, action = 2;
                else
                    st->radius *= 0.5;
            } else {
                st->invalid_run = 0;
                const double step_norm = sqrt(st->stepsq_p + s[RR::STEPSQ]);
                const double ccost = 0.5 * s[RR::COST2];
                const double ptol = kParameterTol * (st->x_norm + kParameterTol);
                const double cost_change = st->cost - ccost;
                const double ftol = kFunctionTol * st->cost;
                const double rel = cost_change / model_change;
                if (tr) tr[2] = ccost, tr[6] = step_norm;
                if (rf_in_band(step_norm, ptol, kBandParameter)) {
                    rf_restart(st, kRfGuardParameter), action = 2;
                } else if (step_norm <= ptol) {
                    if (tr) tr[7] = RSDSFM_TRACE_PARAMETER_TOL;
                    st->termination = RSDSFM_TERM_PARAMETER, action = 2;
                } else if (rf_in_band(fabs(cost_change), ftol, kBandFunction)) {
                    rf_restart(st, kRfGuardFunction), action = 2;
                } else if (fabs(cost_change) <= ftol) {
                    if (tr) tr[7] = RSDSFM_TRACE_FUNCTION_TOL;
// ... 123 lines not shown
        if (!again) break;
        resolve = true;
    }
    RF_BEAT(30);
    if (ext_out) {
        if (tid < RR::NSCHUR) ext_out->sums[tid] = L.cur[tid];
        const int n = L.nlist;
        for (int q = tid; q < n * kRfEntry; q += kFB) ext_out->list[q] = L.list[q];
        if (tid == 0) ext_out->nlist = (double)n;
    }
    RF_BEAT(31);
#undef RF_BEAT
}

struct RfPassArgs {
    int64_t m;
    const double4* xyuv_in;
    double4* xyuv_out;
    double* beta;
    const double* alpha;
    const double* alpha_k;
    double* rho_a;
    double* rho_b;
    const RefineState* st_in;
    RefineState* st_out;
    const double* rows_prev;
    int nrows_prev, row_stride;
    RfLists lists_prev;
    int* list_count;
    double* list_entries;
    int* list_count_zero;
    const RfExt* ext_in;
    RfExt* ext_out;
    double* partials;
    double* trace;
    int trace_rows;
    int64_t m_total;
    const int64_t* m_total_dev;
    const double2* flow;
    int64_t n_flow;
    const double* inl;
    const int64_t* inlier_idx;
    int flow_index_mode;
    int* bad_index;
    unsigned long long* beat;
    int slot;
    const RansacBest* best;
    int grid_cap;
    unsigned long long* stamps;
    const uint32_t* local_idx;
    const int64_t* block_counts;
    int nblocks;
    int64_t chunk;
    const double2* q_px;
    const double* alpha_px;
    const double* alpha_k_px;
    const double* rho_px;
    int64_t* inlier_idx_out;
    double* alpha_out;
    double* alpha_k_out;
    RansacBest* best_pub;
    RansacBest* best_host;
};

struct RfLoad {
    double4 c4;
    double rho, ab, ak;
};
template <int NP>
__device__ __forceinline__ RfLoad rf_load(const RfPassArgs& A, const double* __restrict__ rho, int64_t i, bool live) {
    RfLoad l;
    l.c4 = make_double4(0.0, 0.0, 0.0, 0.0), l.rho = 0.0, l.ab = 0.0, l.ak = 0.0;
    if (live) {
        l.c4 = A.xyuv_in[i];
        l.rho = rho[i];
        if (NP == 6) {
            l.ab = A.beta[i];
        } else {
            l.ab = A.alpha[i], l.ak = A.alpha_k[i];
        }
    }
    return l;
}

}

template <int NP, bool FIRST, bool ZSUM, bool DIRECT = false>
__global__ __launch_bounds__(kFB) void refine_rf_pass_kernel(const RfPassArgs A) {
    static_assert(FIRST || !DIRECT, "only the first pass gathers");
    using RR = RfRow<NP>;
    __shared__ uint32_t s_off[DIRECT ? kRfHandoffBlocks + 1 : 1];
    __shared__ uint32_t s_coarse[64];
    static_assert(kRfHandoffBlocks == 64 * 32, "rounds of the search");
    __shared__ uint32_t s_wtot[kFB / 64];
    __shared__ RfStageLds<NP> s_stage;
    __shared__ double s_red[kFB / 64][RR::NW];
    __shared__ RefineState s_state;
    const bool stamp = A.stamps && blockIdx.x == 0 && threadIdx.x == 0;
    if (A.beat && threadIdx.x == 0) {
        if (A.beat[7]) atomicAdd(&A.beat[2], 1ull);
        if (blockIdx.x == 0) A.beat[0] = ((unsigned long long)A.slot << 8) | 1;
        if (blockIdx.x < 512) A.beat[8 + blockIdx.x] = ((unsigned long long)A.slot << 8) | 1;
    }
    __shared__ unsigned long long tk[8];
    if (stamp) {
#pragma unroll
        for (int i = 0; i < 8; ++i) tk[i] = 0;
    }
    if (stamp) tk[0] = wall_clock64();
    int64_t m_direct = 0;
    if (DIRECT) {
        const int tid = threadIdx.x, lane = tid & 63, wv = tid >> 6;
        const int nb = A.nblocks;
        if (!A.best->undecided) {
            constexpr int kPer = (kRfHandoffBlocks + kFB - 1) / kFB;
            const int per = (nb + kFB - 1) / kFB;
            uint32_t cnt[kPer], sum = 0;
#pragma unroll
            for (int j = 0; j < kPer; ++j) {
                const int b = tid * per + j;
                cnt[j] = (j < per && b < nb) ? (uint32_t)A.block_counts[b] : 0u;
                sum += cnt[j];
            }
            uint32_t inc = sum;
#pragma unroll
            for (int off = 1; off < 64; off <<= 1) {
                const uint32_t t = __shfl_up(inc, off, 64);
                if (lane >= off) inc += t;
            }
            if (lane == 63) s_wtot[wv] = inc;
            __syncthreads();
            uint32_t wbase = 0, total = 0;
#pragma unroll
            for (int w2 = 0; w2 < kFB / 64; ++w2) {
                const uint32_t v = s_wtot[w2];
                if (w2 < wv) wbase += v;
                total += v;
            }
            uint32_t run = wbase + inc - sum;
#pragma unroll
            for (int j = 0; j < kPer; ++j) {
                const int b = tid * per + j;
                if (j < per && b < nb) {
                    s_off[b] = run;
                    run += cnt[j];
                }
            }
            if (tid == 0) s_off[nb] = total;
            m_direct = (int64_t)total;
            __syncthreads();
            if (tid < 64) s_coarse[tid] = tid * 32 < nb ? s_off[tid * 32] : 0xFFFFFFFFu;
            if (blockIdx.x == 0 && tid == 0) {
                A.best_pub->num_inliers_scan = m_direct;
                if (A.best_host) A.best_host->num_inliers_scan = m_direct;
            }
        }
    }
    if (FIRST && A.best) {
        if (threadIdx.x < sizeof(RefineState) / 8) reinterpret_cast<unsigned long long*>(&s_state)[threadIdx.x] = 0ull;
        __syncthreads();
        if (threadIdx.x == 0) {
            RefineState& z = s_state;
            z.np = NP;
            for (int i = 0; i < 3; ++i) {
                z.p[i] = A.best->hyp[3 + i];
                z.p[3 + i] = A.best->hyp[i];
// ... 80 lines not shown
            const double ihm = flagged ? 0.0 : rcp_core(flagged ? 1.0 : o.h);
            rf_schur_accumulate<NP>(o, ihm, acc);
            if (flagged) rf_list_append(A.list_count, A.list_entries, x, y, f.x, f.y, ab, ak, rho, i);
        };
        if (DIRECT) {
            const int lane = threadIdx.x & 63;
            auto rank_pixel = [&](int64_t iw) -> int64_t {
                if (iw >= m) return 0;
                const uint32_t r0 = (uint32_t)iw, r = r0 + (uint32_t)lane;
                const int c = __popcll(__ballot(s_coarse[lane] <= r0)) - 1;
                const int t = c * 32 + lane;
                const int b_lo = c * 32 + __popcll(__ballot(lane < 32 && t <= A.nblocks && s_off[t] <= r0)) - 1;
                if (r >= (uint32_t)m) return 0;
                int b = b_lo;
                while (s_off[b + 1] <= r) ++b;
                return (int64_t)A.local_idx[(int64_t)b * A.chunk + (r - s_off[b])];
            };
            struct Rec {
                double2 q, f;
                double rho, al, ak;
                int64_t p;
            };
            auto load = [&](int64_t i, int64_t p) {
                Rec r;
                r.q = r.f = make_double2(0.0, 0.0), r.rho = r.al = r.ak = 0.0, r.p = p;
                if (i < m) {
                    int64_t fi = (A.flow_index_mode == RSDSFM_FLOW_GATHERED) ? p : i;
                    if (fi < 0 || fi >= A.n_flow) {
                        *A.bad_index = 1;
                        fi = 0;
                    }
                    r.f = A.flow[fi];
                    r.q = A.q_px[p];
                    r.rho = A.rho_px[p];
                    r.al = A.alpha_px[p], r.ak = A.alpha_k_px[p];
                }
                return r;
            };
            auto turn = [&](const Rec& r, int64_t i) {
                const double z = 1.0 / r.rho;
                const double rho = 1.0 / z;
                A.inlier_idx_out[i] = r.p;
                if (NP == 7) A.alpha_out[i] = r.al, A.alpha_k_out[i] = r.ak;
                body(i, r.q.x, r.q.y, rho, r.al, r.ak, r.f);
            };
            const int64_t iw0 = i0 - lane;
            if (NP == 6) {
                Rec r0 = load(i0, rank_pixel(iw0));
                Rec r1 = load(i0 + stride, rank_pixel(iw0 + stride));
                int64_t p2 = rank_pixel(iw0 + 2 * stride);
                for (int64_t iw = iw0; iw < m; iw += stride) {
                    const int64_t i = iw + lane;
                    const Rec r2 = load(i + 2 * stride, p2);
                    p2 = rank_pixel(iw + 3 * stride);
                    if (i < m) turn(r0, i);
                    r0 = r1;
                    r1 = r2;
                }
            } else {
                int64_t p0 = rank_pixel(iw0), p1 = rank_pixel(iw0 + stride);
                for (int64_t iw = iw0; iw < m; iw += stride) {
                    const int64_t i = iw + lane;
                    const Rec r = load(i, p0);
                    p0 = p1;
                    p1 = rank_pixel(iw + 2 * stride);
                    if (i < m) turn(r, i);
                }
            }
        } else {
            for (int64_t i = i0; i < m; i += stride) {
                int64_t fi = (A.flow_index_mode == RSDSFM_FLOW_GATHERED) ? A.inlier_idx[i] : i;
                if (fi < 0 || fi >= A.n_flow) {
                    *A.bad_index = 1;
                    fi = 0;
                }
                const double2 f = A.flow[fi];
                const double x = A.inl[3 * i], y = A.inl[3 * i + 1];
                const double rho = 1.0 / A.inl[3 * i + 2];
                const double al = A.alpha[i], ak = A.alpha_k[i];
                body(i, x, y, rho, al, ak, f);
            }
        }
    } else {
        RfPoint Pq = rf_point(st->p), Pcq = rf_point(st->pc);
        const RfPoint P = rf_point_uniform(Pq), Pc = rf_point_uniform(Pcq);
        double dp[7];
#pragma unroll
        for (int c = 0; c < 7; ++c) dp[c] = uniform_d(st->dp[c]);
        const double inv_radius = uniform_d(1.0 / st->radius);
        const double psi = uniform_d(1.0 / (1.0 + 1.0 / st->radius));
        const double* __restrict__ rho = st->cur ? A.rho_b : A.rho_a;
        double* __restrict__ cand = st->cur ? A.rho_a : A.rho_b;
        auto body = [&](const RfLoad& l0, int64_t i) {
            const double x = l0.c4.x, y = l0.c4.y, ux = l0.c4.z, uy = l0.c4.w, rh = l0.rho;
            const RfGeom g = rf_geom(x, y);
            double be, dbe, bec, dbec, be0, dbe0;
            rf_beta<NP>(l0.ab, l0.ak, P, be, dbe);
            rf_beta<NP>(l0.ab, l0.ak, Pc, bec, dbec);
            rf_beta<NP>(l0.ab, l0.ak, P0, be0, dbe0);
            RfEval<NP> o;
            rf_resid<NP>(g, ux, uy, be, P, rh, o);
            double da0, da1, db0, db1;
            rf_av(g, dp[0], dp[1], dp[2], da0, da1);
            rf_bw(g, dp[3], dp[4], dp[5], db0, db1);
            double t0 = be * __builtin_fma(rh, da0, db0), t1 = be * __builtin_fma(rh, da1, db1);
            if (NP == 7) {
                const double dk = dbe * dp[6];
                t0 = __builtin_fma(dk, o.in0, t0);
                t1 = __builtin_fma(dk, o.in1, t1);
            }
            double a00, a10;
            rf_av(g, P0.v0, P0.v1, P0.v2, a00, a10);
            const double h0 = (be0 * be0) * __builtin_fma(a00, a00, a10 * a10);
            const double gJ = __builtin_fma(o.J0, o.r0, o.J1 * o.r1), tJ = __builtin_fma(o.J0, t0, o.J1 * t1);
            const bool flagged = rf_flagged(o.h, h0);
            double drho = -((psi * (gJ + tJ)) * rcp_core(flagged ? 1.0 : o.h));
            if (__builtin_amdgcn_ballot_w64(flagged) != 0) {
                if (flagged) {
                    asm volatile("; listed inlier: exact e-block inverse" ::: "memory");
                    double sr, E0, E1;
                    const double ete_inv = rf_ete_inv_exact(o.J0, o.J1, h0, inv_radius, sr, E0, E1);
                    drho = -((ete_inv * (sr * (gJ + tJ))) * sr);
                }
            }
            const double m0 = __builtin_fma(o.J0, drho, t0), m1 = __builtin_fma(o.J1, drho, t1);
            acc[RR::MODEL] -= __builtin_fma(m0, __builtin_fma(0.5, m0, o.r0), m1 * __builtin_fma(0.5, m1, o.r1));
            const double cd = rh + drho;
            cand[i] = cd;
            acc[RR::STEPSQ] = __builtin_fma(drho, drho, acc[RR::STEPSQ]);
            RfEval<NP> oc;
            rf_resid<NP>(g, ux, uy, bec, Pc, cd, oc);
            rf_jac<NP>(g, bec, dbec, cd, oc);
            acc[RR::COST2] = __builtin_fma(oc.r0, oc.r0, __builtin_fma(oc.r1, oc.r1, acc[RR::COST2]));
            acc[RR::GMAX] = fmax(acc[RR::GMAX], fabs(__builtin_fma(oc.J0, oc.r0, oc.J1 * oc.r1)));
            acc[RR::XSQ] = __builtin_fma(cd, cd, acc[RR::XSQ]);
            if (ZSUM) acc[RR::ZSUM] += 1.0 / cd;
            const bool flagged_c = rf_flagged(oc.h, h0);
            const double ihm = flagged_c ? 0.0 : rcp_core(flagged_c ? 1.0 : oc.h);
            rf_schur_accumulate<NP>(oc, ihm, acc, lds_c);
            if (flagged_c) rf_list_append(A.list_count, A.list_entries, x, y, ux, uy, l0.ab, l0.ak, cd, i);
        };
        const int64_t last = m - 1;
        if (NP == 6) {
            RfLoad l0 = rf_load<NP>(A, rho, i0, i0 <= last);
            RfLoad l1 = rf_load<NP>(A, rho, i0 + stride, i0 + stride <= last);
            for (int64_t i = i0; i < m; i += stride) {
                const int64_t i2 = i + 2 * stride;
                const RfLoad l2 = rf_load<NP>(A, rho, i2, i2 <= last);
#if RF_LOADS_ONLY
                acc[0] += l0.c4.x + l0.c4.y + l0.c4.z + l0.c4.w + l0.rho + l0.ab;
                cand[i] = l0.rho;
#else
                body(l0, i);
#endif
                l0 = l1;
                l1 = l2;
            }
        } else {
#if RF_NP7_PREFETCH == 1
            RfLoad l0 = rf_load<NP>(A, rho, i0, i0 <= last);
            for (int64_t i = i0; i < m; i += stride) {
                const RfLoad l1 = rf_load<NP>(A, rho, i + stride, i + stride <= last);
                body(l0, i);
                l0 = l1;
            }
#else
            for (int64_t i = i0; i < m; i += stride) body(rf_load<NP>(A, rho, i, true), i);
#endif
        }
    }
    if (kLdsC) {
        int tri = 0;
#pragma unroll
        for (int a = 0; a < NP; ++a) {
            acc[RR::OFF_C + a] = lds_c[a * kFB];
            tri += NP - 1 - a;
            acc[RR::OFF_JTJ + tri] = lds_c[(NP + a) * kFB];
            acc[RR::OFF_B + tri] = lds_c[(2 * NP + a) * kFB];
            tri += 1;
        }
    }
    if (A.beat && threadIdx.x == 0 && blockIdx.x < 512) A.beat[8 + blockIdx.x] = ((unsigned long long)A.slot << 8) | 3;
    if (A.beat && (threadIdx.x & 63) == 0 && blockIdx.x < 64) A.beat[8 + 256 + blockIdx.x * 4 + 0] |= 1ull << (threadIdx.x >> 6);
    if (A.beat && blockIdx.x == 0 && threadIdx.x == 0) A.beat[0] = ((unsigned long long)A.slot << 8) | 3;
    if (stamp) tk[3] = wall_clock64();
    if (A.stamps && blockIdx.x == 0 && (threadIdx.x & 63) == 0) A.stamps[8 + (threadIdx.x >> 6)] += wall_clock64();
    static_assert(RR::GMAX == RR::NW - 1, "the max slot is the row's last");
    block_reduce_store_halving<RR::NW>(acc, s_red, A.partials + (int64_t)blockIdx.x * RR::NW);
    if (A.beat && threadIdx.x == 0) {
        if (A.beat[7]) atomicAdd(&A.beat[3], 1ull);
        if (blockIdx.x == 0) A.beat[0] = ((unsigned long long)A.slot << 8) | 4;
        if (blockIdx.x < 512) A.beat[8 + blockIdx.x] = ((unsigned long long)A.slot << 8) | 4;
    }
    if (stamp) {
        tk[4] = wall_clock64();
        A.stamps[0] += tk[1] - tk[0], A.stamps[1] += tk[2] - tk[1], A.stamps[2] += tk[3] - tk[2], A.stamps[3] += tk[4] - tk[3], A.stamps[4] += 1;
        if (tk[4 + 0]) A.stamps[5] += tk[4 + 0] - tk[1], A.stamps[6] += tk[4 + 1] - tk[4 + 0], A.stamps[7] += tk[2] - tk[4 + 1];
    }
}

template <int NP>
__global__ __launch_bounds__(kFB) void refine_rf_apply_kernel(const double* __restrict__ rows, int nrows, int row_stride, RfLists lists,
                                                             const RefineState* __restrict__ st_in, RefineState* __restrict__ st_out,
                                                             const RfExt* __restrict__ ext_in, RfExt* __restrict__ ext_out, int64_t m_total,
                                                             const int64_t* __restrict__ m_total_dev, double* __restrict__ trace, int trace_rows,
                                                             unsigned long long* __restrict__ beat, int slot) {
    __shared__ RfStageLds<NP> s_stage;
    __shared__ RefineState s_state;
    if (beat && threadIdx.x == 0) beat[1] = ((unsigned long long)slot << 8) | 1;
    state_to_lds(&s_state, st_in);
    RefineState* st = &s_state;
    if (st->termination < 0 && st->pending_apply) {
        const int64_t mt = m_total_dev ? *m_total_dev : (m_total >= 0 ? m_total : st->m);
        rf_apply_body<NP>(st, s_stage, rows, nrows >= 0 ? nrows : st->grid, row_stride, lists, ext_in, ext_out, mt, trace, trace_rows, nullptr, beat);
    }
    __syncthreads();
    if (beat && threadIdx.x == 0) beat[1] = ((unsigned long long)slot << 8) | 40;
    if (threadIdx.x == 0) st->pending_apply = 0;
    __syncthreads();
    state_from_lds(st_out, st);
}

template <int NP>
__global__ __launch_bounds__(kFB) void refine_rf_row_kernel(const double* __restrict__ partials, int nblocks, const RefineState* __restrict__ st,
                                                           const int* __restrict__ list_count, const double* __restrict__ list_entries,
                                                           double* __restrict__ row) {
    using RR = RfRow<NP>;
    __shared__ double s_grp[ReduceShape<RR::NW>::G][RR::NW];
    __shared__ double s[RR::NW];
    if (nblocks < 0) nblocks = st->grid;
    reduce_partials_groups<RR::NW>(partials, nblocks, RR::GMAX, s_grp, threadIdx.x, RR::NW, 0);
    __syncthreads();
    reduce_partials_slots<RR::NW>(s_grp, RR::GMAX, s, threadIdx.x);
    __syncthreads();
    if (threadIdx.x < RR::NW) row[threadIdx.x] = s[threadIdx.x];
    const int n = *list_count;
    double* lr = row + RR::NW;
    if (threadIdx.x == 0) {
        reinterpret_cast<int*>(lr)[0] = n;
        reinterpret_cast<int*>(lr)[1] = 0;
        lr[1] = 0.0;
    }
    if ((int)threadIdx.x < n && n <= kRfListCap) {
        const double* e = list_entries + (size_t)threadIdx.x * kRfEntry;
        int rank = 0;
        for (int j = 0; j < n; ++j) rank += (list_entries[(size_t)j * kRfEntry + 7] < e[7]) ? 1 : 0;
#pragma unroll
        for (int q = 0; q < kRfEntry; ++q) lr[2 + (size_t)rank * kRfEntry + q] = e[q];
    }
}


int refine_rf_extra_doubles() { return 3 * kRfListCap * kRfEntry + 2 * kRfExtDoubles + 8; }
int refine_rf_row_doubles(int np) { return (np == 7 ? RfRow<7>::NW : RfRow<6>::NW) + kRfListDoubles; }

namespace {
static_assert(kWorkgroupsPerCu == 1, "rf_grid_cap and the cap of RefineState::grid (refine_state_from_best_kernel) agree only at one workgroup per CU");
inline int rf_grid_cap(const Ctx* c) { return c->num_cus; }
inline int rf_grid(const Ctx* c, int64_t m) {
    int64_t b = (m + kFB - 1) / kFB;
    const int64_t cap = rf_grid_cap(c);
    if (b < 1) b = 1;
    if (b > cap) {
        const int64_t iters = (b + cap - 1) / cap;
        b = (b + iters - 1) / iters;
    }
    return (int)b;
}
struct RfLayout {
    double* rows[2];
    RefineState* cs[2];
    double* list[3];
    RfExt* ext[2];
};
static_assert(RfRow<7>::NW <= SlotRow<7>::NW && RfRow<6>::NW <= SlotRow<7>::NW, "the rows buffer is sized by SlotRow<7>::NW doubles per workgroup");
inline RfLayout rf_layout(const Ctx* c, const RefineBuffers& B) {
    RfLayout Lo;
    double* base = B.partials;
    const size_t half = (size_t)refine_partials_half_doubles(c);
    Lo.rows[0] = base, Lo.rows[1] = base + half;
    double* p = base + 2 * half;
    const size_t sd = (size_t)refine_state_doubles();
    Lo.cs[0] = reinterpret_cast<RefineState*>(p), Lo.cs[1] = reinterpret_cast<RefineState*>(p + sd);
    p += 2 * sd + 8;
    for (int i = 0; i < 3; ++i) Lo.list[i] = p + (size_t)i * kRfListCap * kRfEntry;
    p += 3 * kRfListCap * kRfEntry;
    Lo.ext[0] = reinterpret_cast<RfExt*>(p), Lo.ext[1] = reinterpret_cast<RfExt*>(p + kRfExtDoubles);
    return Lo;
}
inline int rf_mod3(int g) { return ((g % 3) + 3) % 3; }
inline int* rf_list_count(const RefineBuffers& B, int g) { return refine_rf_counters(B) + rf_mod3(g); }
inline double* rf_list_entries(const RfLayout& Lo, int g) { return Lo.list[rf_mod3(g)]; }
inline RfLists rf_lists_of(const RfLayout& Lo, const RefineBuffers& B, int g, const double* rows_all, int nranks, int nw) {
    RfLists l;
    if (rows_all) {
        l.counts = reinterpret_cast<const int*>(rows_all + nw), l.count_stride = 2 * (nw + kRfListDoubles);
        l.entries = rows_all + nw + 2, l.entry_stride = nw + kRfListDoubles, l.nlists = nranks;
    } else {
        l.counts = rf_list_count(B, g), l.count_stride = 0, l.entries = rf_list_entries(Lo, g), l.entry_stride = 0, l.nlists = 1;
    }
    return l;
}

struct RfBeat {
    const Ctx* c;
    unsigned long long* words;
};
RfBeat g_beats[32];
int g_nbeats = 0;
unsigned long long* rf_beat(Ctx* c) {
    static const bool on = getenv("RSDSFM_SYNC_WATCHDOG_S") != nullptr && getenv("RSDSFM_NO_BEAT") == nullptr;
    if (!on) return nullptr;
    for (int i = 0; i < g_nbeats; ++i)
        if (g_beats[i].c == c) return g_beats[i].words;
    if (g_nbeats >= 32) return nullptr;
    unsigned long long* w = nullptr;
    if (hipHostMalloc((void**)&w, 64 + 8 * 512, hipHostMallocDefault) != hipSuccess) return nullptr;
    for (int i = 0; i < 8 + 512; ++i) w[i] = 0;
    w[7] = getenv("RSDSFM_BEAT_COUNT_WORKGROUPS") ? 1 : 0;
    g_beats[g_nbeats].c = c, g_beats[g_nbeats].words = w;
    ++g_nbeats;
    return w;
}
unsigned long long* rf_stamps(Ctx* c) {
    static int on = -1;
    static unsigned long long* buf = nullptr;
    if (on < 0) {
        const char* e = getenv("RSDSFM_RF_STAMPS");
        on = (e && e[0] == '1') ? 1 : 0;
        if (on && (hipMalloc(&buf, 128) != hipSuccess || hipMemset(buf, 0, 128) != hipSuccess)) buf = nullptr;
    }
    (void)c;
    return buf;
}
template <int NP, bool ZSUM>
void rf_pass_launch_t(Ctx* c, const RfPassArgs& A, bool first, int grid) {
    if (first && A.local_idx)
        hipLaunchKernelGGL((refine_rf_pass_kernel<NP, true, ZSUM, true>), dim3(grid), dim3(kFB), 0, c->stream, A);
    else if (first)
        hipLaunchKernelGGL((refine_rf_pass_kernel<NP, true, ZSUM>), dim3(grid), dim3(kFB), 0, c->stream, A);
    else
        hipLaunchKernelGGL((refine_rf_pass_kernel<NP, false, ZSUM>), dim3(grid), dim3(kFB), 0, c->stream, A);
}
}

int refine_rf_pass_launch(Ctx* c, const RefineBuffers& B, int np, int g, int g_first, const double* rows_all_prev, int nranks, int64_t m_total,
                          const int64_t* m_total_dev, bool publish) {
    const RfLayout Lo = rf_layout(c, B);
    const int grid = B.m_on_device ? rf_grid_cap(c) : rf_grid(c, B.m);
    const int nw = np == 7 ? RfRow<7>::NW : RfRow<6>::NW;
    RfPassArgs A = {};
    A.m = B.m_on_device ? -1 : B.m;
    A.xyuv_in = reinterpret_cast<const double4*>(B.uu);
    A.xyuv_out = reinterpret_cast<double4*>(B.uu);
    A.beta = B.beta;
    A.alpha = B.alpha;
    A.alpha_k = B.alpha_k;
    A.rho_a = B.rho_a;
    A.rho_b = B.rho_b;
    A.st_in = g == g_first ? B.state : Lo.cs[(g - 1) & 1];
    A.st_out = publish ? B.state : Lo.cs[g & 1];
    if (rows_all_prev)
        A.rows_prev = rows_all_prev, A.nrows_prev = nranks, A.row_stride = nw + kRfListDoubles;
    else
        A.rows_prev = Lo.rows[(g - 1) & 1], A.nrows_prev = B.m_on_device ? -1 : grid, A.row_stride = nw;
    A.lists_prev = rf_lists_of(Lo, B, g - 1, rows_all_prev, nranks, nw);
    A.list_count = rf_list_count(B, g);
    A.list_entries = rf_list_entries(Lo, g);
    A.list_count_zero = rf_list_count(B, g + 1);
    A.ext_in = Lo.ext[(g - 1) & 1];
    A.ext_out = Lo.ext[g & 1];
    A.partials = Lo.rows[g & 1];
    A.trace = c->d_refine_trace;
    A.trace_rows = c->refine_trace_rows;
    A.m_total = m_total;
    A.m_total_dev = m_total_dev;
    A.flow = reinterpret_cast<const double2*>(B.flow);
    A.n_flow = B.n_flow;
    A.inl = B.inl;
    A.inlier_idx = B.inlier_idx;
    A.flow_index_mode = B.flow_index_mode;
    A.bad_index = B.bad_index;
    A.best = g == 0 ? B.best_dev : nullptr;
    A.grid_cap = rf_grid_cap(c);
    A.stamps = rf_stamps(c);
    A.beat = rf_beat(c);
    A.slot = g;
    const bool first = g == 0;
    if (first && B.handoff.local_idx) {
        const FrameHandoff& H = B.handoff;
        if (!A.best || H.nblocks > kRfHandoffBlocks || H.n > (int64_t)INT32_MAX) return fail(c, RSDSFM_ERR_INVALID, "refinement: direct hand-off without its preconditions");
        A.local_idx = H.local_idx, A.block_counts = H.block_counts, A.nblocks = H.nblocks, A.chunk = H.chunk;
        A.q_px = reinterpret_cast<const double2*>(H.q), A.alpha_px = H.alpha, A.alpha_k_px = H.alpha_k, A.rho_px = H.rho;
        A.inlier_idx_out = H.inlier_idx, A.alpha_out = H.out_alpha, A.alpha_k_out = H.out_alpha_k;
        A.best_pub = H.best, A.best_host = H.best_host;
    }
    if (np == 7) {
        if (B.want_zsum) rf_pass_launch_t<7, true>(c, A, first, grid); else rf_pass_launch_t<7, false>(c, A, first, grid);
    } else {
        if (B.want_zsum) rf_pass_launch_t<6, true>(c, A, first, grid); else rf_pass_launch_t<6, false>(c, A, first, grid);
    }
    RSDSFM_HIP_CHECK(c, hipGetLastError());
    return RSDSFM_OK;
}

int refine_rf_apply_launch(Ctx* c, const RefineBuffers& B, int np, int g, bool to_published, const double* rows_all, int nranks, int64_t m_total,
                           const int64_t* m_total_dev) {
    const RfLayout Lo = rf_layout(c, B);
    const int grid = B.m_on_device ? rf_grid_cap(c) : rf_grid(c, B.m);
    const int nw = np == 7 ? RfRow<7>::NW : RfRow<6>::NW;
    const double* rows = rows_all ? rows_all : Lo.rows[g & 1];
    const int nrows = rows_all ? nranks : (B.m_on_device ? -1 : grid);
    const int stride = rows_all ? nw + kRfListDoubles : nw;
    const RfLists lists = rf_lists_of(Lo, B, g, rows_all, nranks, nw);
    RefineState* st_io = Lo.cs[g & 1];
    if (np == 7)
        hipLaunchKernelGGL(refine_rf_apply_kernel<7>, dim3(1), dim3(kFB), 0, c->stream, rows, nrows, stride, lists, st_io, to_published ? B.state : st_io,
                           Lo.ext[g & 1], Lo.ext[(g + 1) & 1], m_total, m_total_dev, c->d_refine_trace, c->refine_trace_rows, rf_beat(c), g);
    else
        hipLaunchKernelGGL(refine_rf_apply_kernel<6>, dim3(1), dim3(kFB), 0, c->stream, rows, nrows, stride, lists, st_io, to_published ? B.state : st_io,
                           Lo.ext[g & 1], Lo.ext[(g + 1) & 1], m_total, m_total_dev, c->d_refine_trace, c->refine_trace_rows, rf_beat(c), g);
    RSDSFM_HIP_CHECK(c, hipGetLastError());
    return RSDSFM_OK;
}

int refine_rf_row_launch(Ctx* c, const RefineBuffers& B, int np, int g, double* row) {
    const RfLayout Lo = rf_layout(c, B);
    const int grid = B.m_on_device ? rf_grid_cap(c) : rf_grid(c, B.m);
    if (np == 7)
        hipLaunchKernelGGL(refine_rf_row_kernel<7>, dim3(1), dim3(kFB), 0, c->stream, Lo.rows[g & 1], B.m_on_device ? -1 : grid, static_cast<const RefineState*>(Lo.cs[g & 1]),
                           rf_list_count(B, g), rf_list_entries(Lo, g), row);
    else
        hipLaunchKernelGGL(refine_rf_row_kernel<6>, dim3(1), dim3(kFB), 0, c->stream, Lo.rows[g & 1], B.m_on_device ? -1 : grid, static_cast<const RefineState*>(Lo.cs[g & 1]),
                           rf_list_count(B, g), rf_list_entries(Lo, g), row);
    RSDSFM_HIP_CHECK(c, hipGetLastError());
    return RSDSFM_OK;
}

void refine_rf_debug_dump(Ctx* c, const RefineBuffers& B) {
    const RfLayout Lo = rf_layout(c, B);
    hipStream_t s2 = nullptr;
    if (hipStreamCreateWithFlags(&s2, hipStreamNonBlocking) != hipSuccess) return;
    RefineState h[3];
    int cnt[8] = {0, 0, 0, 0, 0, 0, 0, 0};
    const RefineState* src[3] = {B.state, Lo.cs[0], Lo.cs[1]};
    for (int i = 0; i < 3; ++i) (void)hipMemcpyAsync(&h[i], src[i], sizeof(RefineState), hipMemcpyDeviceToHost, s2);
    (void)hipMemcpyAsync(cnt, B.bad_index, sizeof(int) * 8, hipMemcpyDeviceToHost, s2);
    if (hipStreamSynchronize(s2) != hipSuccess) {
        fprintf(stderr, "[rsdsfm] refinement dump: the copies did not complete either\n");
        return;
    }
    const char* names[3] = {"published", "chunk state 0", "chunk state 1"};
    for (int i = 0; i < 3; ++i)
        fprintf(stderr, "[rsdsfm] %s: np %d termination %d iteration %d slots %d pending_apply %d rf %d guard %d cur %d solve_ok %d m %lld grid %d radius %g cost %g successful %d unsuccessful %d invalid_run %d\n",
                names[i], h[i].np, h[i].termination, h[i].iteration, h[i].slots, h[i].pending_apply, h[i].rf, h[i].rf_guard, h[i].cur, h[i].solve_ok, (long long)h[i].m, h[i].grid, h[i].radius,
                h[i].cost, h[i].num_successful, h[i].num_unsuccessful, h[i].invalid_run);
    fprintf(stderr, "[rsdsfm] bad_index %d, list counters %d %d %d (m_on_device %d, m %lld)\n", cnt[0], cnt[4], cnt[5], cnt[6], (int)B.m_on_device, (long long)B.m);
    for (int i = 0; i < g_nbeats; ++i)
        fprintf(stderr, "[rsdsfm] context %p%s: last pass slot %llu phase %llu; pass workgroups started %llu, left %llu; last stage kernel slot %llu phase %llu\n", (const void*)g_beats[i].c, g_beats[i].c == c ? " (the waiting one)" : "",
                g_beats[i].words[0] >> 8, g_beats[i].words[0] & 255, g_beats[i].words[2], g_beats[i].words[3], g_beats[i].words[1] >> 8, g_beats[i].words[1] & 255);
    for (int i = 0; i < g_nbeats; ++i) {
        if (g_beats[i].c != c) continue;
        int hist[16] = {0};
        const unsigned long long last = g_beats[i].words[0] >> 8;
        fprintf(stderr, "[rsdsfm] workgroups of the waiting context's pass (slot %llu) not at phase 4 / 9:", last);
        for (int b = 0; b < 256; ++b) {
            const unsigned long long w = g_beats[i].words[8 + b];
            hist[w & 15] += 1;
            if ((w & 255) != 4 && (w & 255) != 9) fprintf(stderr, " [%d: slot %llu phase %llu]", b, w >> 8, w & 255);
        }
        fprintf(stderr, "\n[rsdsfm] phase histogram:");
        for (int p = 0; p < 10; ++p) fprintf(stderr, " %d:%d", p, hist[p]);
        fprintf(stderr, "\n");
    }
}

int refine_rf_read_stamps(Ctx* c, unsigned long long out[16]) {
    unsigned long long* b = rf_stamps(c);
    if (!b) return RSDSFM_ERR_INVALID;
    RSDSFM_HIP_CHECK(c, hipStreamSynchronize(c->stream));
    RSDSFM_HIP_CHECK(c, hipMemcpy(out, b, 128, hipMemcpyDeviceToHost));
    RSDSFM_HIP_CHECK(c, hipMemset(b, 0, 128));
    return RSDSFM_OK;
}

}
```

### rs-aware-differential-sfm_amd/csrc/rsdsfm_internal.hpp

```cpp
#pragma once

#include <hip/hip_runtime.h>
#include <stdint.h>

#include <functional>
#include <string>
#include <vector>

#include "../../include/rsdsfm.h"

namespace rsdsfm {

constexpr int kMaxIter = 50;
constexpr int kRefineTraceCols = RSDSFM_REFINE_TRACE_COLS;
constexpr double kInitialRadius = 1e4;
constexpr double kMaxRadius = 1e16;
constexpr double kMinRadius = 1e-32;
constexpr double kMinRelDecrease = 1e-3;
constexpr double kMinLmDiag = 1e-6;
constexpr double kMaxLmDiag = 1e32;
constexpr double kFunctionTol = 1e-6;
constexpr double kGradientTol = 1e-10;
static_assert(kGradientTol < 1.0, "the indicator encoding of the gradient-maximum slots needs kGradientTol < 1");
constexpr double kParameterTol = 1e-8;
// ... 76 lines not shown
    double* d_partials = nullptr;
    unsigned* d_tickets = nullptr;
    LmState* d_lm = nullptr;
    LmState* h_lm = nullptr;
    int lm_issued_k = 0;
    int true_flow_exhaustive = 0;
    int ransac_fused_base = 2;
    int ransac_score_idle = kScoreIdleLimit;
    int refine_iters_hint = -1;
    int ransac_standard_math = 0;
    int* d_core_flag = nullptr;
    int core_epoch = 0;
    int ransac_math_mode = 0;
    int64_t ransac_restarts = 0;
    int lm_arithmetic = 0;
    int lma_hold = 0;
    bool lma_count_only_force = false;
    int64_t lma_count_only_runs = 0, lma_lazy_runs = 0;
    int lma_unique_run = 0;
    int64_t lma_restarts = 0;
    int64_t lma_handed_over = 0;
    int lma_last_guard = 0;
    int* d_lma_list = nullptr;
    int depth_lma_parity = 0;
    int lma_cand[2] = {2, 1};
    int ransac_spec_miss = 0;
    int frame_dense_hint = 1;
    int lm_issued_d = 0;
    int depth_epoch = 0;
    int depth_standard_math = 0;
    int64_t depth_restarts = 0;
    int depth_core_launch = 0;
    int prof_what = 0;
    void* d_stage = nullptr;
    size_t stage_bytes = 0;
    void* d_ws = nullptr;
    size_t ws_bytes = 0;
    void* d_frame = nullptr;
    size_t frame_bytes = 0;
    void* h_pinned = nullptr;
    hipEvent_t ev_ready = nullptr;
    size_t pinned_bytes = 0;
    int num_cus = 256;
    int ransac_k0 = 0;
    int ransac_not_one_step = -1;
    bool profile = false;
    hipEvent_t ev_prof[2] = {nullptr, nullptr};
    unsigned long long* d_clk_probe = nullptr;
    bool prof_pending = false;
    double* d_refine_trace = nullptr;
    int refine_trace_rows = 0;
    int depth_variant = 0;
    void* d_tile = nullptr;
    size_t tile_bytes = 0;
    void* tile_session = nullptr;
    int tile_np = 0;
    void* flow_pair = nullptr;
    void* flow_clip = nullptr;
    int flow_batch = 0;
    void* flow_check = nullptr;
    void* link = nullptr;
    void* fuse = nullptr;
    void* last_frame = nullptr;
    void* rectify_dense = nullptr;
    unsigned* d_claim[3] = {nullptr, nullptr, nullptr};
    size_t claim_words[3] = {0, 0, 0};
    unsigned claim_epoch[3] = {0, 0, 0};
    void* dist = nullptr;
    void* frame_run = nullptr;
    hipStream_t aux_stream = nullptr;
    hipEvent_t ev_fork = nullptr, ev_join = nullptr, ev_seq = nullptr;
    int frame_side_flatten = 3;
    int frame_tail = 0;
    int frame_handoff = 0;
    int frame_predict = 0;
    int lma_operands = 0;
    unsigned long long* d_flat_counters = nullptr;
    int seq_lanes = 0;
    int refine_stage_mode = 0;
    bool refine_stage_separate = false;
    int refine_arithmetic = 0;
    int64_t refine_rf_runs = 0, refine_rf_restarts = 0, refine_rf_resolves = 0;
    int refine_rf_last_guard = 0;
    struct RansacCache {
        uint64_t tag = 0, stage_gen = 0;
        const double *d_u = nullptr, *d_inl = nullptr, *d_alpha = nullptr, *d_alpha_k = nullptr;
        const int64_t* d_idx = nullptr;
        int64_t n = 0, m = 0;
        const void* h_u = nullptr;
        double u_probe[16] = {0};
        double inl_probe[16] = {0};
    } ransac_cache;
    uint64_t stage_gen = 0, ransac_tag_counter = 0;
    int64_t refine_cache_hits = 0;
    std::vector<rsdsfm_ctx*> lanes;
    int occlusion_search = 0;
    int plate_estimator = 0;
};
constexpr int kSequenceLanesDefault = 3;
void dist_release(Ctx* c);
void dist_reset_hold(Ctx* c);
void frame_release(Ctx* c);
void flow_release(Ctx* c);
void flow_check_release(Ctx* c);
void rectify_dense_release(Ctx* c);
void link_release(Ctx* c);
void fuse_release(Ctx* c);
void last_frame_release(Ctx* c);

constexpr int kDepthBlock = 256;
constexpr int kDepthMaxBlocks = 512;
constexpr int kDecideBlock = 256;
constexpr int kDepthBatchMax = 8;

#define RSDSFM_HIP_CHECK(ctx, expr)                                                            \
    do {                                                                                       \
        hipError_t _e = (expr);                                                                \
        if (_e != hipSuccess) {                                                                \
            (ctx)->err = std::string(#expr) + ": " + hipGetErrorString(_e);                    \
            return RSDSFM_ERR_HIP;                                                             \
        }                                                                                      \
    } while (0)

struct DeviceGuard {
    int prev = -1;
    bool switched = false;
    explicit DeviceGuard(const Ctx* c) {
        if (hipGetDevice(&prev) == hipSuccess && prev != c->device) switched = hipSetDevice(c->device) == hipSuccess;
    }
    ~DeviceGuard() {
        if (switched) (void)hipSetDevice(prev);
    }
    DeviceGuard(const DeviceGuard&) = delete;
    DeviceGuard& operator=(const DeviceGuard&) = delete;
};

int fail(Ctx* c, int code, const char* msg);
template <class... P>
inline bool aligned_to(uintptr_t bytes, const P*... p) {
    return ((reinterpret_cast<uintptr_t>(p) | ... | (uintptr_t)0) & (bytes - 1)) == 0;
}
int ensure_stage(Ctx* c, size_t bytes);
struct XferItem {
    void* host;
    const void* dev;
    size_t bytes;
};
struct XferUp {
    void* dev;
    const void* host;
    size_t bytes;
};
int xfer_h2d(Ctx* c, void* d_dst, const void* h_src, size_t bytes);
int xfer_h2d_many(Ctx* c, const XferUp* items, int count);
int xfer_d2h(Ctx* c, void* h_dst, const void* d_src, size_t bytes);
int xfer_d2h_many(Ctx* c, const XferItem* items, int count);
bool xfer_trace_on();
void xfer_trace(const char* label);
void xfer_trace_span(const char* label, double us);
void xfer_trace_dump(const char* what);
int ensure_ws(Ctx* c, size_t bytes);
int sync_stream(Ctx* c, const char* where);
void set_sync_dumper(std::function<void(Ctx*)> f);
int ensure_pinned(Ctx* c, size_t bytes);

struct Arena {
// ... 78 lines not shown
int minimal9_launch(Ctx* c, const double* q, const double* u, const double* alpha, const double* alpha_k,
                    const int32_t* samples, int T, int use_alpha_k, int k_sign_mode, double* hyp_out, void* zero_begin = nullptr,
                    size_t zero_bytes = 0, const Minimal9Direct* direct = nullptr);
struct DenseFlatten {
    double thr = 0.0;
    double *d_q = nullptr, *d_u = nullptr, *d_alpha = nullptr, *d_alpha_k = nullptr;
    unsigned long long* d_counters = nullptr;
    int64_t* total_out = nullptr;
};
int minimal9_flatten_launch(Ctx* c, const int32_t* samples, int T, int use_alpha_k, int k_sign_mode, double* hyp_out, void* zero_begin, size_t zero_bytes,
                            const Minimal9Direct& direct, double thr, double* d_q, double* d_u, double* d_alpha, double* d_alpha_k,
                            unsigned long long* d_counters, int64_t* total_out, int* pred_steps = nullptr, int pred_invert = 0);
}

namespace rsdsfm {
int ransac_pixel_grid(const Ctx* c, int64_t n);
int ransac_lm_partials_doubles(const Ctx* c, int64_t n, int batch);
int ransac_lm_round_launch(Ctx* c, const double* q, const double* u, const double* a, const double* ak, int64_t n,
                           const double* hyp, int T, LmState* states, double* partials, int* flags, int* scored,
                           double* trial_count, double* trial_err, int round, double tol, int k0, int fused_base, bool core_math,
                           const int* m9_core_flag = nullptr, int m9_core_epoch = 0, int* unscored_list = nullptr);
int ransac_score_launch(Ctx* c, const double* q, const double* u, const double* a, const double* ak, int64_t n,
                        const double* hyp, int T, const LmState* states, int depth_mode, double tol, const int* scored,
                        double* partials, double* trial_count, double* trial_err, const int* unscored_list = nullptr, const int* unscored_count = nullptr);
int ransac_pick_launch(Ctx* c, const double* trial_count, const double* trial_err, int T, const double* hyp, RansacBest* best,
                       RansacBest* best_host = nullptr, const int* d_flags = nullptr, int* h_flags = nullptr, int scored_ahead = 0,
                       const double* cnt_rt = nullptr, int cnt_stride = 0, int nranks = 0, int64_t* m_all = nullptr, double tie_margin = 0.0,
                       PickLazy lazy = PickLazy());
int ransac_final_launch(Ctx* c, const double* q, const double* u, const double* a, const double* ak, int64_t n,
                        RansacBest* best, const LmState* states, int depth_mode, double tol, double* rho, uint8_t* mask,
                        int64_t* block_counts, int64_t* block_offsets, int64_t* inlier_idx, double* inliers,
                        double* out_alpha, double* out_alpha_k, RansacBest* best_host = nullptr, int* zero_words = nullptr,
                        uint32_t* local_idx = nullptr, FrameHandoff* handoff = nullptr);
int ransac_scatter_launch(Ctx* c, const FrameHandoff& H);
int ransac_rows_doubles();
int ransac_lm_rows_launch(Ctx* c, const double* q, const double* u, const double* a, const double* ak, int64_t n,
                          const double* hyp, int T, const LmState* states, double* partials, int round, double tol, double* rows,
                          int* core_flags = nullptr, const int* m9_flag = nullptr, int m9_epoch = 0);
int ransac_rows_payload_doubles(int T, bool core_trailer);
int ransac_decide_rows_launch(Ctx* c, const double* rows_all, int nranks, int T, LmState* states, int64_t n_total, int round,
                              int* flags, int* scored, double* trial_count, double* trial_err, bool core_trailer = false,
                              double* cnt_rt = nullptr, int cnt_stride = 0);
int ransac_score_rows_launch(Ctx* c, const double* q, const double* u, const double* a, const double* ak, int64_t n,
                             const double* hyp, int T, const LmState* states, int depth_mode, double tol, const int* scored,
                             double* partials, double* rows);
int ransac_score_merge_launch(Ctx* c, const double* rows_all, int nranks, int T, const int* scored, double* trial_count,
                              double* trial_err, double* cnt_rt = nullptr, int cnt_stride = 0);
void sample_indices(int64_t n, int T, uint64_t seed, int32_t* out);
int64_t ransac_lma_partials_doubles(const Ctx* c, int64_t n, int batch);
size_t ransac_lma_list_ints(int batch);
int ransac_lma_launch(Ctx* c, const double* q, const double* u, const double* a, const double* ak, int64_t n, const double* hyp, int T,
                      LmState* states, double* partials, int* flags, int* scored, double* trial_count, double* trial_err, double tol,
                      const int* cand_steps, int ncand, int* irr_count, int* irr_list, int* unscored_list, int* guard_word,
                      const int* m9_core_flag = nullptr, int m9_core_epoch = 0, bool count_only = false, const int* pred_steps = nullptr,
                      unsigned long long* pred_stats = nullptr, bool pred_discard = false,
                      bool k_uniform = false, double k_value = 0.0);
int ransac_lma_rows_doubles();
int ransac_lma_rows_launch(Ctx* c, const double* q, const double* u, const double* a, const double* ak, int64_t n, const double* hyp, int T,
                           double* partials, double tol, const int* cand_steps, int ncand, int* irr_count, int* irr_list, double* rows);
int ransac_lma_decide_rows_launch(Ctx* c, const double* rows_all, int nranks, int64_t rank_stride, int T, int64_t n_total, const double* hyp,
                                  LmState* states, int* flags, int* scored, double* trial_count, double* trial_err, double tol, const int* cand_steps,
                                  int ncand, int* unscored_list, int* guard_word, double* cnt_rt, int cnt_stride, const int* m9_core_flag = nullptr,
                                  int m9_core_epoch = 0);
}

namespace rsdsfm {
struct RefineState {
    int32_t np, cur, iteration, invalid_run, num_successful, num_unsuccessful, termination, solve_ok;
    double p[7], pc[7], sp[7], yp[7];
    double radius, decrease_factor, cost, initial_cost, x_norm, gmax, stepsq_p;
    int64_t m;
    int32_t grid;
    int32_t need_schur;
    double zsum;
    int32_t slots;
    int32_t spec_miss_run;
    int32_t pending_apply;
    int32_t rf;
    double dp[7];
    double p0[7];
    int32_t rf_guard, rf_resolves;
};
constexpr int kTermRestartExact = 64;
struct FinishClaim {
    bool on = false;
    double fx = 0.0, fy = 0.0, cx = 0.0, cy = 0.0;
    int rows = 0, cols = 0;
    int32_t* ys = nullptr;
    unsigned* owner = nullptr;
    unsigned tag = 0, mask = 0;
};
struct RefineBuffers {
    const double* flow;
    int64_t n_flow, m;
    bool m_on_device = false;
    const double* inl;
    const double* alpha;
    const double* alpha_k;
    const int64_t* inlier_idx;
    int flow_index_mode;
    RefineState* state;
    double* uu;
    double* beta;
    double* rho_a;
    double* rho_b;
    double* srho;
    double* partials;
    int* bad_index;
    RefineState* state_host = nullptr;
    double* zpartials = nullptr;
    const RansacBest* best_dev = nullptr;
    FinishClaim claim;
    FrameHandoff handoff;
    const double* fin_xy = nullptr;
    int fin_stride = 3;
    bool want_zsum = false;
};
size_t ransac_pinned_bytes(int T);
typedef std::function<int(const RansacBest*)> RansacSpecTail;
struct RansacRun {
    int pc = 0;
    const double *d_q = nullptr, *d_u = nullptr, *d_a = nullptr, *d_ak = nullptr;
    int64_t n = 0;
    int T = 0, Tn = 1, batch = 1, depth_mode = 0, use_alpha_k = 0, k_sign_mode = 0, k0 = 0, fused_base = 0;
    double tol = 0.0;
    rsdsfm_ransac_out* out = nullptr;
    const RansacSpecTail* spec_tail = nullptr;
    bool* spec_tail_held = nullptr;
    int core_epoch = 0;
    int* d_unscored = nullptr;
    bool core_math = true;
    bool analytic = false;
    bool lma_restarted = false;
    int* refine_flag_words = nullptr;
    uint32_t* d_local_idx = nullptr;
    FrameHandoff handoff;
    bool direct_final = false;
    bool count_only = false;
    int lazy_rounds = 0;
    int shared_best = 0;
    double tie_margin = 0.0;
    int lma_guard = 0;
    bool lma_tie_seen = false;
    int lma_cand[2] = {2, 1}, lma_cand_next[2] = {0, 0};
    int *d_irr_count = nullptr, *d_irr_list = nullptr;
    int* d_pred_steps = nullptr;
    bool own_pass = false;
    bool restarted = false;
    bool tail_ahead = true;
    const Minimal9Direct* direct = nullptr;
    const DenseFlatten* dense = nullptr;
    const std::function<int()>* after_minimal9 = nullptr;
    std::vector<int32_t> samples;
    double *d_hyp = nullptr, *d_partials = nullptr, *d_tcount = nullptr, *d_terr = nullptr, *d_rho = nullptr;
    char* zero_begin = nullptr;
    size_t zero_bytes = 0;
    LmState* d_states = nullptr;
    int *d_scored = nullptr, *d_flags = nullptr;
    RansacBest* d_best = nullptr;
    int64_t *d_bcounts = nullptr, *d_boffs = nullptr;
    uint8_t* d_mask = nullptr;
    RansacBest* h_best = nullptr;
    int* h_running = nullptr;
    double *h_tcount = nullptr, *h_terr = nullptr, *h_hyp = nullptr;
    LmState* h_states = nullptr;
    int32_t* h_samples_pinned = nullptr;
    int b0 = 0, B = 0, round = 0;
    bool need_score = true, final_done = false, spec_scored = false, tail_enqueued = false, spec_final = false;
    int not_one_step = 0, fused_base_next = 0, score_hint_next = -1;
    bool hints_ready = false;
};
int ransac_begin(Ctx* c, const double* d_q, const double* d_u, const double* d_a, const double* d_ak, int64_t n, int use_alpha_k, int T,
                 double tol, const int32_t* h_samples, uint64_t seed, int depth_mode, int k_sign_mode, rsdsfm_ransac_out* out,
                 const RansacSpecTail* spec_tail, bool* spec_tail_held, RansacRun* run, const Minimal9Direct* direct,
                 const std::function<int()>* after_minimal9, const DenseFlatten* dense = nullptr, bool tail_ahead = true, bool count_only = false,
                 int* refine_flag_words = nullptr, uint32_t* local_idx = nullptr);
int ransac_finish(Ctx* c, RansacRun* run);
void ransac_commit_hints(Ctx* c, const RansacRun& run);
int flatten_enqueue(Ctx* c, const double* d_img, int32_t rows, int32_t cols, double fx, double fy, double cx, double cy, double gamma,
                    double thr, double* d_q, double* d_u, double* d_alpha, double* d_alpha_k, int64_t* h_total);
typedef std::function<int(const RefineBuffers&)> RefineTail;
int refine_finish_grid(const Ctx* c, const RefineBuffers& B);
int depth_map_decided_launch(Ctx* c, double* d_inl, int64_t m, const double* d_zsums, int nz, const RefineBuffers& B, double* d_depth_map,
                             double* d_header, double* h_header, const double* v_dev, const int64_t* m_dev, const PoseTableOut* pt);
struct RefineRun {
    RefineBuffers B;
    int np = 6, launched = 0, chunk = 5, hint_prev = -1;
    bool rf = false;
    double* d_inl_out = nullptr;
    const RefineTail* tail = nullptr;
    RefineState* hs = nullptr;
    bool prefetch = false, prefetched = false;
    bool tail_done = false;
};
constexpr size_t kPinnedTail = 1024;
size_t refine_workspace_bytes(const Ctx* c, int64_t m, bool m_on_device);
int refine_begin(Ctx* c, const double* d_flow, int64_t n_flow, int64_t m, const double* d_inl, const double* d_alpha,
                 const double* d_alpha_k, const int64_t* d_inlier_idx, const double v_in[3], const double w_in[3], double k_in,
                 int const_acceleration, int flow_index_mode, double* d_inl_out, const RefineTail* tail, const RansacBest* d_best,
                 void* ws_base, RefineRun* run, RefineState* hs_prefetch, double* d_zpartials, bool exact = false,
                 const FinishClaim* claim = nullptr, const FrameHandoff* handoff = nullptr);
constexpr int kRcRefineRestartExact = 1;
int refine_device(Ctx* c, const double* d_flow, int64_t n_flow, int64_t m, const double* d_inl, const double* d_alpha,
                  const double* d_alpha_k, const int64_t* d_inlier_idx, const double v_in[3], const double w_in[3], double k_in,
                  int const_acceleration, int flow_index_mode, double* d_inl_out, double v_out[3], double w_out[3], double* k_out,
                  rsdsfm_lm_summary* summary, const RefineTail* tail, double* d_zpartials, bool exact = false, const FinishClaim* claim = nullptr);
int refine_enqueue_chunk(Ctx* c, RefineRun* run);
int frames_in_flight(const Ctx* c);
int refine_poll(Ctx* c, RefineRun* run, double v_out[3], double w_out[3], double* k_out, rsdsfm_lm_summary* summary);
int refine_partials_doubles(const Ctx* c, int64_t m);
int refine_partials_doubles_cap(const Ctx* c);
int refine_state_from_best_launch(Ctx* c, const RansacBest* d_best, const RefineBuffers& B, int np);
int* refine_flag_words(void* ws_base);
inline int refine_trace_reset(Ctx* c) {
    if (!c->d_refine_trace) return RSDSFM_OK;
    return hipMemsetAsync(c->d_refine_trace, 0xFF, (size_t)c->refine_trace_rows * kRefineTraceCols * sizeof(double), c->stream) == hipSuccess ? RSDSFM_OK : RSDSFM_ERR_HIP;
}
int refine_init_launch(Ctx* c, const RefineBuffers& B, int np);
int refine_rf_pass_launch(Ctx* c, const RefineBuffers& B, int np, int g, int g_first, const double* rows_all_prev, int nranks, int64_t m_total,
                          const int64_t* m_total_dev, bool publish = false);
int refine_rf_apply_launch(Ctx* c, const RefineBuffers& B, int np, int g, bool to_published, const double* rows_all, int nranks, int64_t m_total,
                           const int64_t* m_total_dev);
int refine_rf_row_launch(Ctx* c, const RefineBuffers& B, int np, int g, double* row);
int refine_rf_row_doubles(int np);
void refine_rf_debug_dump(Ctx* c, const RefineBuffers& B);
int refine_rf_read_stamps(Ctx* c, unsigned long long out[16]);
int refine_rf_extra_doubles();
int refine_partials_half_doubles(const Ctx* c);
int refine_state_doubles();
inline int* refine_rf_counters(const RefineBuffers& B) { return B.bad_index + 4; }
int refine_iter_launch(Ctx* c, const RefineBuffers& B, int np, int j, int chunk);
int refine_finish_launch(Ctx* c, const RefineBuffers& B, double* inl_out);
int refine_stage_row_doubles(int np, int stage);
int refine_slot_row_doubles(int np);
int refine_slot_partials_doubles(const Ctx* c, int64_t m);
int refine_slot_rows_launch(Ctx* c, const RefineBuffers& B, int np, double* row, int j, const double* rows_all_prev, int nranks);
int refine_slot_apply_launch(Ctx* c, const RefineBuffers& B, int np, const double* rows_all, int nranks, int chunk);
int refine_stage_rows_launch(Ctx* c, const RefineBuffers& B, int np, int stage, double* row);
int refine_stage_apply_launch(Ctx* c, const RefineBuffers& B, int np, int stage, const double* rows_all, int nranks, int64_t m_total,
                              const int64_t* m_total_dev = nullptr);
}

namespace rsdsfm {
int back_project_launch(Ctx* c, const unsigned char* d_img, const double* d_depth_cm, const double* d_R, const double* d_t, double fx,
                        double fy, double cx, double cy, int rows, int cols, int mode, int q5_mode, unsigned char* d_gs, float* d_c3d);
int interpolate_cracky_launch(Ctx* c, const unsigned char* d_in, int rows, int cols, int offset, unsigned char* d_out);
int rectify_frame_launch(Ctx* c, const double* d_inl, int64_t m, const unsigned char* d_img, const double* d_depth_cm, const double* d_R,
                         const double* d_t, double fx, double fy, double cx, double cy, int rows, int cols, int mode, int q5_mode, int offset,
                         unsigned char* d_preview, unsigned char* d_gs, float* d_c3d, unsigned char* d_fixed, double* d_partials);
int depth_preview_launch(Ctx* c, const double* d_inl, int64_t m, double fx, double fy, double cx, double cy, int rows, int cols,
                         unsigned char* d_out, double* d_partials);
}

struct rsdsfm_ctx {
    rsdsfm::Ctx c;
};
```

Baseline: 1992.

## Run radius-factorised refinement as one persistent kernel with grid barriers

Adds a persistent refine kernel that runs all LM iterations inside a single launch, with software grid barriers built on atomic counters, a done-flag wait, and a fused finish/claim step. It targets the per-iteration kernel launch and host round-trip cost of the radius-factorised refinement. If a barrier waits past its tick limit, the kernel reports a restart code and the host falls back to per-iteration launches. This brings a risk of spin-waiting and of wasted work when residency is not guaranteed. The path is the default (mode 0) when eligible: a dense frame hint is set, only one frame is in flight, and the grid fits.

```diff
diff --git a/include/rsdsfm.h b/include/rsdsfm.h
--- a/include/rsdsfm.h
+++ b/include/rsdsfm.h
@@ -188,6 +188,8 @@
 int rsdsfm_set_frame_side_flatten(rsdsfm_ctx* ctx, int mode);
 int rsdsfm_set_frame_tail(rsdsfm_ctx* ctx, int mode);
 int rsdsfm_set_frame_handoff(rsdsfm_ctx* ctx, int mode);
+int rsdsfm_set_refine_persist(rsdsfm_ctx* ctx, int mode);
+int rsdsfm_refine_persist_stats(rsdsfm_ctx* ctx, int64_t* runs, int64_t* trips);
 int rsdsfm_set_frame_predict(rsdsfm_ctx* ctx, int mode);
 int rsdsfm_lma_predict_stats(rsdsfm_ctx* ctx, int64_t* hypotheses, int64_t* ended_where_predicted);
 int rsdsfm_set_lma_operands(rsdsfm_ctx* ctx, int mode);
diff --git a/rs-aware-differential-sfm_amd/csrc/capi.hip b/rs-aware-differential-sfm_amd/csrc/capi.hip
--- a/rs-aware-differential-sfm_amd/csrc/capi.hip
+++ b/rs-aware-differential-sfm_amd/csrc/capi.hip
@@ -232,16 +232,23 @@
     return RSDSFM_OK;
 }
 
+static unsigned long long g_rf_stamps[16];
+
 int rsdsfm_profile_last_ms(rsdsfm_ctx* ctx, const char* what, double* ms) {
     CTX_OR_FAIL(ctx);
     if (what && ms && !strncmp(what, "refine_rf_phase", 15) && ((what[15] >= '0' && what[15] <= '9') || (what[15] >= 'a' && what[15] <= 'f')) && !what[16]) {
-        static unsigned long long h[16];
+        unsigned long long* const h = g_rf_stamps;
         if (what[15] == '0') {
             int rc = refine_rf_read_stamps(c, h);
             if (rc != RSDSFM_OK) return fail(c, RSDSFM_ERR_INVALID, "no phase stamps: set RSDSFM_RF_STAMPS=1 before the first refinement");
         }
         const int k = what[15] <= '9' ? what[15] - '0' : what[15] - 'a' + 10;
         *ms = k == 4 ? (double)h[4] : k >= 8 ? (double)(long long)(h[k] - h[8]) * 0.01 : (double)h[k] * 0.01;
+        return RSDSFM_OK;
+    }
+    if (what && ms && !strncmp(what, "refine_rf_persist", 17) && what[17] >= '0' && what[17] <= '2' && !what[18]) {
+        const int k = what[17] - '0';
+        *ms = k == 2 ? (double)g_rf_stamps[10] : (double)g_rf_stamps[8 + k] * 0.01;
         return RSDSFM_OK;
     }
     const bool clock = what && !strcmp(what, "ransac_lm_round0_clock_mhz");
@@ -392,6 +399,23 @@
     *runs = n, *restarts = r;
     if (resolves_or_null) *resolves_or_null = s;
     if (last_guard_or_null) *last_guard_or_null = guard;
+    return RSDSFM_OK;
+}
+
+int rsdsfm_set_refine_persist(rsdsfm_ctx* ctx, int mode) {
+    CTX_OR_FAIL(ctx);
+    if (mode < 0 || mode > 2) return fail(c, RSDSFM_ERR_INVALID, "refine persist: 0 = one persistent launch where eligible (default), 1 = one launch per iteration, 2 = 0 with the wait limit at zero");
+    c->refine_persist = mode;
+    for (rsdsfm_ctx* lane : c->lanes) lane->c.refine_persist = mode;
+    return RSDSFM_OK;
+}
+
+int rsdsfm_refine_persist_stats(rsdsfm_ctx* ctx, int64_t* runs, int64_t* trips) {
+    CTX_OR_FAIL(ctx);
+    if (!runs || !trips) return fail(c, RSDSFM_ERR_INVALID, "refine persist stats: null output");
+    int64_t n = c->refine_persist_runs, t = c->refine_persist_trips;
+    for (rsdsfm_ctx* lane : c->lanes) n += lane->c.refine_persist_runs, t += lane->c.refine_persist_trips;
+    *runs = n, *trips = t;
     return RSDSFM_OK;
 }
 
diff --git a/rs-aware-differential-sfm_amd/csrc/frame_host.hip b/rs-aware-differential-sfm_amd/csrc/frame_host.hip
--- a/rs-aware-differential-sfm_amd/csrc/frame_host.hip
+++ b/rs-aware-differential-sfm_amd/csrc/frame_host.hip
@@ -230,6 +230,7 @@
     };
     F->refinement_enqueued = false;
     F->ahead = prm->use_refinement && c->ransac_spec_miss < 2;
+    F->claim.persist_ok = F->ahead && c->frame_dense_hint != 0;
     F->d_local_idx = (c->frame_handoff == 0 && F->ahead && F->claim.on && c->lm_arithmetic == 0 && c->refine_arithmetic == 0 && !c->refine_stage_separate)
                          ? d_local_idx : nullptr;
     F->open = true;
@@ -271,6 +272,7 @@
         n = *count_host(c);
         F->n = n;
         F->refinement_enqueued = false;
+        F->claim.persist_ok = false;
         counted = false;
         rc = ransac_begin(c, F->d_q, F->d_u, F->d_a, F->d_ak, n, prm->use_acceleration_mode, prm->ransac_trials, prm->ransac_tol, nullptr, J.seed,
                           prm->depth_mode, prm->k_sign_mode, &F->ro, prm->use_refinement ? &F->spec_tail : nullptr, &F->refinement_enqueued, &F->ransac, nullptr, nullptr,
@@ -298,6 +300,14 @@
         bool exact = false;
         if (F->refinement_enqueued) {
             rc = refine_poll(c, &F->refine, v, w, &k, &res->refine_summary);
+            if (rc == kRcRefineRestartLaunches) {
+                RSDSFM_HIP_CHECK(c, hipMemsetAsync(refine_flag_words(F->d_refine_ws), 0, kRefineStateBlockTail, c->stream));
+                F->claim.persist_ok = false;
+                rc = F->spec_tail(F->ransac.d_best);
+                if (rc != RSDSFM_OK) return rc;
+                RSDSFM_HIP_CHECK(c, hipStreamSynchronize(c->stream));
+                rc = refine_poll(c, &F->refine, v, w, &k, &res->refine_summary);
+            }
             exact = rc == kRcRefineRestartExact;
         }
         if ((!F->refinement_enqueued || exact) && F->ransac.direct_final) {
@@ -465,6 +475,7 @@
         lc->frame_side_flatten = c->frame_side_flatten;
         lc->frame_tail = c->frame_tail;
         lc->frame_handoff = c->frame_handoff;
+        lc->refine_persist = c->refine_persist;
         lc->frame_predict = c->frame_predict;
         lc->lma_operands = c->lma_operands;
         lc->refine_stage_mode = c->refine_stage_mode;
diff --git a/rs-aware-differential-sfm_amd/csrc/refine_common.hpp b/rs-aware-differential-sfm_amd/csrc/refine_common.hpp
--- a/rs-aware-differential-sfm_amd/csrc/refine_common.hpp
+++ b/rs-aware-differential-sfm_amd/csrc/refine_common.hpp
@@ -321,5 +321,44 @@
     if (threadIdx.x < sizeof(RefineState) / 8) reinterpret_cast<double*>(st_out)[threadIdx.x] = reinterpret_cast<const double*>(s_st)[threadIdx.x];
 }
 
-}
-}
+struct FinishClaimArgs {
+    const double* inl;
+    int xy_stride;
+    double* inl_out;
+    double* zpartials;
+    double fx, fy, cx, cy;
+    int rows, ncols;
+    unsigned* owner;
+    unsigned tag;
+    int32_t* ys;
+};
+__device__ __forceinline__ void finish_claim_body(const FinishClaimArgs& F, int64_t m, const double* __restrict__ inl, const double* __restrict__ rho,
+                                                  double* __restrict__ inl_out, double* __restrict__ zpartials, unsigned* __restrict__ owner,
+                                                  int32_t* __restrict__ ys, double* s_red) {
+    const int64_t stride = (int64_t)gridDim.x * kFB;
+    const int xy_stride = F.xy_stride;
+    double acc = 0.0;
+    for (int64_t i = (int64_t)blockIdx.x * kFB + threadIdx.x; i < m; i += stride) {
+        const double xn = inl[xy_stride * i], yn = inl[xy_stride * i + 1];
+        inl_out[3 * i] = xn;
+        inl_out[3 * i + 1] = yn;
+        const double z = 1.0 / rho[i];
+        inl_out[3 * i + 2] = z;
+        acc += z;
+        const int x = (int)(F.fx * xn + F.cx + 0.5);
+        const int y = (int)(F.fy * yn + F.cy + 0.5);
+        ys[i] = y;
+        if (x >= 0 && x < F.ncols && y >= 0 && y < F.rows) atomicMax(&owner[(int64_t)x * F.rows + y], F.tag | (unsigned)i);
+    }
+    const double r = wave_sum(acc);
+    if ((threadIdx.x & 63) == 0) s_red[threadIdx.x >> 6] = r;
+    __syncthreads();
+    if (threadIdx.x == 0) {
+        double t = s_red[0];
+        for (int w2 = 1; w2 < kFB / 64; ++w2) t += s_red[w2];
+        zpartials[blockIdx.x] = t;
+    }
+}
+
+}
+}
diff --git a/rs-aware-differential-sfm_amd/csrc/refine_host.hip b/rs-aware-differential-sfm_amd/csrc/refine_host.hip
--- a/rs-aware-differential-sfm_amd/csrc/refine_host.hip
+++ b/rs-aware-differential-sfm_amd/csrc/refine_host.hip
@@ -54,6 +54,8 @@
     run->np = np;
     run->rf = !exact && c->lm_arithmetic == 0 && c->refine_arithmetic == 0;
     if (run->rf) c->refine_rf_runs += 1;
+    run->persist = false;
+    run->first_grid_cap = 0;
     run->d_inl_out = d_inl_out;
     run->tail = tail;
     run->launched = 0;
@@ -67,6 +69,7 @@
         if (direct) {
             B.handoff = *handoff;
             B.fin_xy = B.uu, B.fin_stride = 4;
+            run->persist = c->refine_persist != 1 && claim->persist_ok && frames_in_flight(c) == 1 && refine_rf_persist_fits(c, np, B.want_zsum);
         }
     } else if (direct) {
         return fail(c, RSDSFM_ERR_INVALID, "refinement: direct hand-off without the start state in the first pass");
@@ -110,6 +113,28 @@
             refine_rf_debug_dump(cc, B);
         });
     }
+    if (run->rf && run->persist) {
+        if (run->launched != 0) return fail(c, RSDSFM_ERR_NUMERIC, "refinement: a persistent launch left its solve unfinished");
+        int rc = refine_rf_pass_launch(c, run->B, run->np, 0, 0, nullptr, 0, -1, nullptr, false);
+        if (rc != RSDSFM_OK) return rc;
+        run->first_grid_cap = refine_rf_grid_cap(c);
+        FinishClaim& C = run->B.claim;
+        const int64_t npix = (int64_t)C.rows * C.cols;
+        if (run->B.m >= ((int64_t)1 << 31)) return fail(c, RSDSFM_ERR_INVALID, "depth map: more than 2^31 inliers");
+        rc = claim_map_acquire(c, 2, (size_t)std::max<int64_t>(std::max<int64_t>(npix, run->B.m), 1), &C.owner, &C.tag, &C.mask);
+        if (rc != RSDSFM_OK) return rc;
+        rc = refine_rf_persist_launch(c, run->B, run->np, run->d_inl_out, run->first_grid_cap, c->refine_persist == 2 ? 0ull : kRfPersistWaitTicks);
+        if (rc != RSDSFM_OK) return rc;
+        run->launched = 1 + run->chunk;
+        run->tail_done = false;
+        if (run->tail) {
+            rc = (*run->tail)(run->B);
+            run->tail_done = true;
+        }
+        if (rc != RSDSFM_OK) return rc;
+        if (run->prefetch) run->prefetched = true;
+        return rc;
+    }
     if (run->rf) {
         for (int i = 0; i <= run->chunk; ++i) {
             const int g = run->launched + i;
@@ -154,6 +179,11 @@
             if (int rcs = sync_stream(c, "refine_poll line 168")) return rcs;
         }
         if (*h_bad) return fail(c, RSDSFM_ERR_INVALID, "flow index out of range (flow has fewer columns than inliers / bad inlier_idx)");
+        if (first && run->persist) c->refine_persist_runs += 1;
+        if (hs->termination == kTermRestartLaunches) {
+            c->refine_persist_trips += 1;
+            return kRcRefineRestartLaunches;
+        }
         if (hs->termination == kTermRestartExact) {
             c->refine_rf_restarts += 1;
             c->refine_rf_last_guard = hs->rf_guard;
diff --git a/rs-aware-differential-sfm_amd/csrc/refine_kernels.hip b/rs-aware-differential-sfm_amd/csrc/refine_kernels.hip
--- a/rs-aware-differential-sfm_amd/csrc/refine_kernels.hip
+++ b/rs-aware-differential-sfm_amd/csrc/refine_kernels.hip
@@ -472,28 +472,8 @@
     }
     const double* __restrict__ rho = st->cur ? rho_b : rho_a;
     if (m < 0) m = st->m;
-    const int64_t stride = (int64_t)gridDim.x * kFB;
-    double acc = 0.0;
-    for (int64_t i = (int64_t)blockIdx.x * kFB + threadIdx.x; i < m; i += stride) {
-        const double xn = inl[xy_stride * i], yn = inl[xy_stride * i + 1];
-        inl_out[3 * i] = xn;
-        inl_out[3 * i + 1] = yn;
-        const double z = 1.0 / rho[i];
-        inl_out[3 * i + 2] = z;
-        acc += z;
-        const int x = (int)(fx * xn + cx + 0.5);
-        const int y = (int)(fy * yn + cy + 0.5);
-        ys[i] = y;
-        if (x >= 0 && x < ncols && y >= 0 && y < rows) atomicMax(&owner[(int64_t)x * rows + y], tag | (unsigned)i);
-    }
-    const double r = wave_sum(acc);
-    if ((threadIdx.x & 63) == 0) s_red[threadIdx.x >> 6] = r;
-    __syncthreads();
-    if (threadIdx.x == 0) {
-        double t = s_red[0];
-        for (int w2 = 1; w2 < kFB / 64; ++w2) t += s_red[w2];
-        zpartials[blockIdx.x] = t;
-    }
+    const FinishClaimArgs F = {inl, xy_stride, inl_out, zpartials, fx, fy, cx, cy, rows, ncols, owner, tag, ys};
+    finish_claim_body(F, m, inl, rho, inl_out, zpartials, owner, ys, s_red);
 }
 
 __global__ void refine_state_from_best_kernel(const RansacBest* __restrict__ best, RefineState* __restrict__ st, int np, int cap,
diff --git a/rs-aware-differential-sfm_amd/csrc/refine_rf_kernels.hip b/rs-aware-differential-sfm_amd/csrc/refine_rf_kernels.hip
--- a/rs-aware-differential-sfm_amd/csrc/refine_rf_kernels.hip
+++ b/rs-aware-differential-sfm_amd/csrc/refine_rf_kernels.hip
@@ -13,6 +13,7 @@
 
 constexpr int kRfListCap = 64;
 constexpr int kRfEntry = 8;
+__host__ __device__ inline int rf_mod3(int g) { return ((g % 3) + 3) % 3; }
 
 template <int NP>
 struct RfRow {
@@ -360,9 +361,8 @@
 template <int NP>
 __device__ __forceinline__ void rf_apply_body(RefineState* st, RfStageLds<NP>& L, const double* __restrict__ rows, int nrows, int row_stride, RfLists lists,
                               const RfExt* __restrict__ ext_in, RfExt* __restrict__ ext_out, int64_t m_total, double* __restrict__ trace, int trace_rows,
-                              unsigned long long* tks = nullptr, unsigned long long* beat = nullptr) {
+                              unsigned long long* tks = nullptr, unsigned long long* beat = nullptr, const int tid = threadIdx.x) {
     using RR = RfRow<NP>;
-    const int tid = threadIdx.x;
 #define RF_BEAT(code) do { if (beat && tid == 0) beat[1] = (beat[1] & ~255ull) | (code); } while (0)
     RF_BEAT(10);
     if (tid == 0) L.bad = 0;
@@ -652,6 +652,93 @@
     }
     return l;
 }
+
+template <int NP>
+__device__ __forceinline__ void rf_lds_sums_to_registers(double (&acc)[RfRow<NP>::NW], const double* lds_c) {
+    using RR = RfRow<NP>;
+    int tri = 0;
+#pragma unroll
+    for (int a = 0; a < NP; ++a) {
+        acc[RR::OFF_C + a] = lds_c[a * kFB];
+        tri += NP - 1 - a;
+        acc[RR::OFF_JTJ + tri] = lds_c[(NP + a) * kFB];
+        acc[RR::OFF_B + tri] = lds_c[(2 * NP + a) * kFB];
+        tri += 1;
+    }
+}
+
+constexpr unsigned kRfBarrierBroken = 0x80000000u;
+constexpr unsigned kRfDoneState = 1u, kRfDoneBroken = 2u;
+
+__device__ __forceinline__ bool rf_grid_barrier(unsigned* word, unsigned target, unsigned long long wait_ticks, int* s_flag,
+                                                unsigned long long* waited = nullptr) {
+    __syncthreads();
+    if (threadIdx.x == 0) {
+        __builtin_amdgcn_fence(__ATOMIC_RELEASE, "agent");
+        unsigned v = __hip_atomic_fetch_add(word, 1u, __ATOMIC_RELAXED, __HIP_MEMORY_SCOPE_AGENT) + 1u;
+        const unsigned long long t0 = wall_clock64();
+        int ok = 0;
+        for (;;) {
+            if (v & kRfBarrierBroken) break;
+            if (v >= target) {
+                ok = 1;
+                break;
+            }
+            if (wall_clock64() - t0 >= wait_ticks) {
+                unsigned expected = v;
+                if (__hip_atomic_compare_exchange_strong(word, &expected, v | kRfBarrierBroken, __ATOMIC_RELAXED, __ATOMIC_RELAXED, __HIP_MEMORY_SCOPE_AGENT)) break;
+                v = expected;
+                continue;
+            }
+            __builtin_amdgcn_s_sleep(2);
+            v = __hip_atomic_load(word, __ATOMIC_RELAXED, __HIP_MEMORY_SCOPE_AGENT);
+        }
+        __builtin_amdgcn_fence(__ATOMIC_ACQUIRE, "agent");
+        if (waited) *waited += wall_clock64() - t0;
+        *s_flag = ok;
+    }
+    __syncthreads();
+    return *s_flag != 0;
+}
+
+__device__ __forceinline__ bool rf_wait_done(unsigned* done, unsigned long long wait_ticks, int* s_flag) {
+    if (threadIdx.x == 0) {
+        const unsigned long long t0 = wall_clock64();
+        unsigned v = 0;
+        for (;;) {
+            v = __hip_atomic_load(done, __ATOMIC_RELAXED, __HIP_MEMORY_SCOPE_AGENT);
+            if (v != 0) break;
+            if (wall_clock64() - t0 >= wait_ticks) {
+                unsigned expected = 0;
+                if (__hip_atomic_compare_exchange_strong(done, &expected, kRfBarrierBroken, __ATOMIC_RELAXED, __ATOMIC_RELAXED, __HIP_MEMORY_SCOPE_AGENT)) {
+                    v = kRfBarrierBroken;
+                    break;
+                }
+                continue;
+            }
+            __builtin_amdgcn_s_sleep(32);
+        }
+        __builtin_amdgcn_fence(__ATOMIC_ACQUIRE, "agent");
+        *s_flag = v == kRfDoneState ? 1 : 0;
+    }
+    __syncthreads();
+    return *s_flag != 0;
+}
+
+struct RfPersistArgs {
+    const RefineState* st_first;
+    RefineState* cs[2];
+    RefineState* st_pub;
+    RefineState* st_host;
+    double* rows[2];
+    double* list[3];
+    int* counters;
+    RfExt* ext[2];
+    unsigned* barrier;
+    unsigned long long wait_ticks;
+    int max_slots;
+    FinishClaimArgs fin;
+};
 
 }
 
@@ -898,104 +985,9 @@
             }
         }
     } else {
-        RfPoint Pq = rf_point(st->p), Pcq = rf_point(st->pc);
-        const RfPoint P = rf_point_uniform(Pq), Pc = rf_point_uniform(Pcq);
-        double dp[7];
-#pragma unroll
-        for (int c = 0; c < 7; ++c) dp[c] = uniform_d(st->dp[c]);
-        const double inv_radius = uniform_d(1.0 / st->radius);
-        const double psi = uniform_d(1.0 / (1.0 + 1.0 / st->radius));
-        const double* __restrict__ rho = st->cur ? A.rho_b : A.rho_a;
-        double* __restrict__ cand = st->cur ? A.rho_a : A.rho_b;
-        auto body = [&](const RfLoad& l0, int64_t i) {
-            const double x = l0.c4.x, y = l0.c4.y, ux = l0.c4.z, uy = l0.c4.w, rh = l0.rho;
-            const RfGeom g = rf_geom(x, y);
-            double be, dbe, bec, dbec, be0, dbe0;
-            rf_beta<NP>(l0.ab, l0.ak, P, be, dbe);
-            rf_beta<NP>(l0.ab, l0.ak, Pc, bec, dbec);
-            rf_beta<NP>(l0.ab, l0.ak, P0, be0, dbe0);
-            RfEval<NP> o;
-            rf_resid<NP>(g, ux, uy, be, P, rh, o);
-            double da0, da1, db0, db1;
-            rf_av(g, dp[0], dp[1], dp[2], da0, da1);
-            rf_bw(g, dp[3], dp[4], dp[5], db0, db1);
-            double t0 = be * __builtin_fma(rh, da0, db0), t1 = be * __builtin_fma(rh, da1, db1);
-            if (NP == 7) {
-                const double dk = dbe * dp[6];
-                t0 = __builtin_fma(dk, o.in0, t0);
-                t1 = __builtin_fma(dk, o.in1, t1);
-            }
-            double a00, a10;
-            rf_av(g, P0.v0, P0.v1, P0.v2, a00, a10);
-            const double h0 = (be0 * be0) * __builtin_fma(a00, a00, a10 * a10);
-            const double gJ = __builtin_fma(o.J0, o.r0, o.J1 * o.r1), tJ = __builtin_fma(o.J0, t0, o.J1 * t1);
-            const bool flagged = rf_flagged(o.h, h0);
-            double drho = -((psi * (gJ + tJ)) * rcp_core(flagged ? 1.0 : o.h));
-            if (__builtin_amdgcn_ballot_w64(flagged) != 0) {
-                if (flagged) {
-                    asm volatile("; listed inlier: exact e-block inverse" ::: "memory");
-                    double sr, E0, E1;
-                    const double ete_inv = rf_ete_inv_exact(o.J0, o.J1, h0, inv_radius, sr, E0, E1);
-                    drho = -((ete_inv * (sr * (gJ + tJ))) * sr);
-                }
-            }
-            const double m0 = __builtin_fma(o.J0, drho, t0), m1 = __builtin_fma(o.J1, drho, t1);
-            acc[RR::MODEL] -= __builtin_fma(m0, __builtin_fma(0.5, m0, o.r0), m1 * __builtin_fma(0.5, m1, o.r1));
-            const double cd = rh + drho;
-            cand[i] = cd;
-            acc[RR::STEPSQ] = __builtin_fma(drho, drho, acc[RR::STEPSQ]);
-            RfEval<NP> oc;
-            rf_resid<NP>(g, ux, uy, bec, Pc, cd, oc);
-            rf_jac<NP>(g, bec, dbec, cd, oc);
-            acc[RR::COST2] = __builtin_fma(oc.r0, oc.r0, __builtin_fma(oc.r1, oc.r1, acc[RR::COST2]));
-            acc[RR::GMAX] = fmax(acc[RR::GMAX], fabs(__builtin_fma(oc.J0, oc.r0, oc.J1 * oc.r1)));
-            acc[RR::XSQ] = __builtin_fma(cd, cd, acc[RR::XSQ]);
-            if (ZSUM) acc[RR::ZSUM] += 1.0 / cd;
-            const bool flagged_c = rf_flagged(oc.h, h0);
-            const double ihm = flagged_c ? 0.0 : rcp_core(flagged_c ? 1.0 : oc.h);
-            rf_schur_accumulate<NP>(oc, ihm, acc, lds_c);
-            if (flagged_c) rf_list_append(A.list_count, A.list_entries, x, y, ux, uy, l0.ab, l0.ak, cd, i);
-        };
-        const int64_t last = m - 1;
-        if (NP == 6) {
-            RfLoad l0 = rf_load<NP>(A, rho, i0, i0 <= last);
-            RfLoad l1 = rf_load<NP>(A, rho, i0 + stride, i0 + stride <= last);
-            for (int64_t i = i0; i < m; i += stride) {
-                const int64_t i2 = i + 2 * stride;
-                const RfLoad l2 = rf_load<NP>(A, rho, i2, i2 <= last);
-#if RF_LOADS_ONLY
-                acc[0] += l0.c4.x + l0.c4.y + l0.c4.z + l0.c4.w + l0.rho + l0.ab;
-                cand[i] = l0.rho;
-#else
-                body(l0, i);
-#endif
-                l0 = l1;
-                l1 = l2;
-            }
-        } else {
-#if RF_NP7_PREFETCH == 1
-            RfLoad l0 = rf_load<NP>(A, rho, i0, i0 <= last);
-            for (int64_t i = i0; i < m; i += stride) {
-                const RfLoad l1 = rf_load<NP>(A, rho, i + stride, i + stride <= last);
-                body(l0, i);
-                l0 = l1;
-            }
-#else
-            for (int64_t i = i0; i < m; i += stride) body(rf_load<NP>(A, rho, i, true), i);
-#endif
-        }
-    }
-    if (kLdsC) {
-        int tri = 0;
-#pragma unroll
-        for (int a = 0; a < NP; ++a) {
-            acc[RR::OFF_C + a] = lds_c[a * kFB];
-            tri += NP - 1 - a;
-            acc[RR::OFF_JTJ + tri] = lds_c[(NP + a) * kFB];
-            acc[RR::OFF_B + tri] = lds_c[(2 * NP + a) * kFB];
-            tri += 1;
-        }
-    }
+#include "refine_rf_later_loop.hpp"
+    }
+    if (kLdsC) rf_lds_sums_to_registers<NP>(acc, lds_c);
     if (A.beat && threadIdx.x == 0 && blockIdx.x < 512) A.beat[8 + blockIdx.x] = ((unsigned long long)A.slot << 8) | 3;
     if (A.beat && (threadIdx.x & 63) == 0 && blockIdx.x < 64) A.beat[8 + 256 + blockIdx.x * 4 + 0] |= 1ull << (threadIdx.x >> 6);
     if (A.beat && blockIdx.x == 0 && threadIdx.x == 0) A.beat[0] = ((unsigned long long)A.slot << 8) | 3;
@@ -1013,6 +1005,118 @@
         A.stamps[0] += tk[1] - tk[0], A.stamps[1] += tk[2] - tk[1], A.stamps[2] += tk[3] - tk[2], A.stamps[3] += tk[4] - tk[3], A.stamps[4] += 1;
         if (tk[4 + 0]) A.stamps[5] += tk[4 + 0] - tk[1], A.stamps[6] += tk[4 + 1] - tk[4 + 0], A.stamps[7] += tk[2] - tk[4 + 1];
     }
+}
+
+template <int NP, bool ZSUM>
+__global__ __launch_bounds__(kFB) void refine_rf_persist_kernel(const RfPassArgs A0, const RfPersistArgs Q) {
+    using RR = RfRow<NP>;
+    __shared__ RfStageLds<NP> s_stage;
+    __shared__ double s_red[kFB / 64][RR::NW];
+    __shared__ RefineState s_state;
+    __shared__ int s_flag;
+    __shared__ unsigned long long tk[8];
+    constexpr bool kLdsC = NP == 7;
+    __shared__ double s_cacc[kLdsC ? 3 * NP : 1][kLdsC ? kFB : 1];
+    __shared__ int s_tid[kFB];
+    s_tid[threadIdx.x] = threadIdx.x;
+    const bool stamp = A0.stamps && blockIdx.x == 0 && threadIdx.x == 0;
+    unsigned* const bar = Q.barrier;
+    unsigned* const done = Q.barrier + 1;
+    state_to_lds(&s_state, Q.st_first);
+    RefineState* st = &s_state;
+    const int live = st->grid;
+    const int64_t m = st->m;
+    const bool shape_ok = live >= 1 && live <= (int)gridDim.x;
+    bool broken = !shape_ok;
+    if (shape_ok && (int)blockIdx.x >= live) {
+        if (!rf_wait_done(done, Q.wait_ticks * 16ull, &s_flag)) return;
+        state_to_lds(&s_state, Q.st_pub);
+    } else {
+        for (int g = 1; shape_ok; ++g) {
+            const int tid = s_tid[threadIdx.x];
+            if (stamp) {
+                tk[0] = wall_clock64();
+                tk[4] = 0;
+            }
+            if (st->termination < 0 && st->pending_apply) {
+                RfLists lists;
+                lists.counts = Q.counters + rf_mod3(g - 1), lists.count_stride = 0, lists.entries = Q.list[rf_mod3(g - 1)], lists.entry_stride = 0, lists.nlists = 1;
+                rf_apply_body<NP>(st, s_stage, Q.rows[(g - 1) & 1], live, RR::NW, lists, Q.ext[(g - 1) & 1], blockIdx.x == 0 ? Q.ext[g & 1] : nullptr, m,
+                                  nullptr, 0, stamp ? tk + 4 : nullptr, nullptr, tid);
+                __syncthreads();
+            }
+            if (tid == 0) st->pending_apply = st->termination < 0 ? 1 : 0;
+            __syncthreads();
+            if (stamp) tk[1] = wall_clock64();
+            if (blockIdx.x == 0) {
+                state_from_lds(Q.cs[g & 1], st);
+                if (threadIdx.x == 0) Q.counters[rf_mod3(g + 1)] = 0;
+            }
+            if (st->termination >= 0) break;
+            if (g >= Q.max_slots) {
+                broken = true;
+                break;
+            }
+            const int64_t stride = (int64_t)st->grid * kFB;
+            const int64_t i0 = (int64_t)blockIdx.x * kFB + tid;
+            double* const lds_c = kLdsC ? &s_cacc[0][tid] : nullptr;
+            double acc[RR::NW];
+#pragma unroll
+            for (int s = 0; s < RR::NW; ++s) acc[s] = 0.0;
+            if (kLdsC) {
+#pragma unroll
+                for (int a = 0; a < 3 * NP; ++a) lds_c[a * kFB] = 0.0;
+            }
+            RfPassArgs A = A0;
+            A.list_count = Q.counters + rf_mod3(g), A.list_entries = Q.list[rf_mod3(g)];
+            RfPoint P0q = rf_point(st->p0);
+            const RfPoint P0 = rf_point_uniform(P0q);
+            {
+#include "refine_rf_later_loop.hpp"
+            }
+            if (kLdsC) rf_lds_sums_to_registers<NP>(acc, lds_c);
+            if (stamp) tk[2] = wall_clock64();
+            block_reduce_store_halving<RR::NW>(acc, s_red, Q.rows[g & 1] + (int64_t)blockIdx.x * RR::NW);
+            if (stamp) tk[3] = wall_clock64();
+            const bool held = rf_grid_barrier(bar, (unsigned)live * (unsigned)g, Q.wait_ticks, &s_flag, stamp ? A.stamps + 8 : nullptr);
+            if (stamp) {
+                const unsigned long long slot = wall_clock64() - tk[0];
+                A.stamps[1] += tk[1] - tk[0], A.stamps[2] += tk[2] - tk[1], A.stamps[3] += tk[3] - tk[2], A.stamps[4] += 1;
+                if (tk[4]) A.stamps[5] += tk[4] - tk[0], A.stamps[6] += tk[5] - tk[4], A.stamps[7] += tk[1] - tk[5];
+                if (slot > A.stamps[9]) A.stamps[9] = slot;
+                A.stamps[10] += 1;
+            }
+            if (!held) {
+                broken = true;
+                break;
+            }
+        }
+        if (Q.wait_ticks == 0) broken = true;
+        if (blockIdx.x == 0) {
+            for (int round = 0; round < 2; ++round) {
+                if (threadIdx.x == 0 && broken) st->termination = kTermRestartLaunches;
+                __syncthreads();
+                state_from_lds(Q.st_pub, st);
+                if (round == 1) break;
+                __syncthreads();
+                if (threadIdx.x == 0) {
+                    __builtin_amdgcn_fence(__ATOMIC_RELEASE, "agent");
+                    const unsigned old = __hip_atomic_fetch_or(done, broken ? kRfDoneBroken : kRfDoneState, __ATOMIC_RELAXED, __HIP_MEMORY_SCOPE_AGENT);
+                    s_flag = (old & kRfBarrierBroken) ? 1 : 0;
+                }
+                __syncthreads();
+                if (broken || !s_flag) break;
+                broken = true;
+            }
+            if (Q.st_host) {
+                if (threadIdx.x < sizeof(RefineState) / 8) reinterpret_cast<double*>(Q.st_host)[threadIdx.x] = reinterpret_cast<const double*>(st)[threadIdx.x];
+                if (threadIdx.x == 0) *reinterpret_cast<int*>(reinterpret_cast<char*>(Q.st_host) + sizeof(RefineState)) = *A0.bad_index;
+            }
+        }
+    }
+    if (broken) return;
+    const double* rho = st->cur ? A0.rho_b : A0.rho_a;
+    finish_claim_body(Q.fin, m, Q.fin.inl, rho, Q.fin.inl_out, Q.fin.zpartials, Q.fin.owner, Q.fin.ys, &s_red[0][0]);
 }
 
 template <int NP>
@@ -1104,7 +1208,6 @@
     Lo.ext[0] = reinterpret_cast<RfExt*>(p), Lo.ext[1] = reinterpret_cast<RfExt*>(p + kRfExtDoubles);
     return Lo;
 }
-inline int rf_mod3(int g) { return ((g % 3) + 3) % 3; }
 inline int* rf_list_count(const RefineBuffers& B, int g) { return refine_rf_counters(B) + rf_mod3(g); }
 inline double* rf_list_entries(const RfLayout& Lo, int g) { return Lo.list[rf_mod3(g)]; }
 inline RfLists rf_lists_of(const RfLayout& Lo, const RefineBuffers& B, int g, const double* rows_all, int nranks, int nw) {
@@ -1220,6 +1323,71 @@
     return RSDSFM_OK;
 }
 
+int refine_rf_grid_cap(const Ctx* c) { return rf_grid_cap(c); }
+
+namespace {
+template <int NP, bool ZSUM>
+bool rf_persist_fits_t(const Ctx* c) {
+    int per_cu = 0;
+    hipFuncAttributes fa;
+    if (hipOccupancyMaxActiveBlocksPerMultiprocessor(&per_cu, refine_rf_persist_kernel<NP, ZSUM>, kFB, 0) != hipSuccess) return false;
+    if (hipFuncGetAttributes(&fa, reinterpret_cast<const void*>(refine_rf_persist_kernel<NP, ZSUM>)) != hipSuccess) return false;
+    return per_cu >= 1 && rf_grid_cap(c) <= c->num_cus && fa.localSizeBytes == 0;
+}
+}
+
+bool refine_rf_persist_fits(Ctx* c, int np, bool want_zsum) {
+    if (np != 6) return false;
+    int& f = c->refine_persist_fits[want_zsum ? 1 : 0];
+    if (f < 0) {
+        const bool ok = want_zsum ? rf_persist_fits_t<6, true>(c) : rf_persist_fits_t<6, false>(c);
+        (void)hipGetLastError();
+        f = ok ? 1 : 0;
+    }
+    return f == 1;
+}
+
+int refine_rf_persist_launch(Ctx* c, const RefineBuffers& B, int np, double* inl_out, int first_grid_cap, unsigned long long wait_ticks) {
+    const RfLayout Lo = rf_layout(c, B);
+    const int grid = rf_grid_cap(c);
+    if (np != 6 || !B.m_on_device || !B.claim.on || !B.zpartials || grid != first_grid_cap || grid > c->num_cus)
+        return fail(c, RSDSFM_ERR_INVALID, "refinement: persistent launch without its preconditions");
+    static_assert(kRefineStateBlockTail >= 7 * sizeof(int), "flag | barrier | done | - | three list counters");
+    RfPassArgs A = {};
+    A.m = -1;
+    A.xyuv_in = reinterpret_cast<const double4*>(B.uu);
+    A.beta = B.beta;
+    A.alpha = B.alpha;
+    A.alpha_k = B.alpha_k;
+    A.rho_a = B.rho_a;
+    A.rho_b = B.rho_b;
+    A.trace = c->d_refine_trace;
+    A.trace_rows = c->refine_trace_rows;
+    A.m_total = -1;
+    A.bad_index = B.bad_index;
+    A.grid_cap = grid;
+    A.stamps = rf_stamps(c);
+    RfPersistArgs Q = {};
+    Q.st_first = Lo.cs[0];
+    Q.st_pub = B.state;
+    Q.st_host = B.state_host;
+    for (int i = 0; i < 2; ++i) Q.cs[i] = Lo.cs[i], Q.rows[i] = Lo.rows[i], Q.ext[i] = Lo.ext[i];
+    for (int i = 0; i < 3; ++i) Q.list[i] = Lo.list[i];
+    Q.counters = refine_rf_counters(B);
+    Q.barrier = reinterpret_cast<unsigned*>(B.bad_index + 1);
+    Q.wait_ticks = wait_ticks;
+    Q.max_slots = 8 * kMaxIter + 16;
+    const FinishClaim& C = B.claim;
+    Q.fin.inl = B.fin_xy ? B.fin_xy : B.inl, Q.fin.xy_stride = B.fin_xy ? B.fin_stride : 3;
+    Q.fin.inl_out = inl_out, Q.fin.zpartials = B.zpartials;
+    Q.fin.fx = C.fx, Q.fin.fy = C.fy, Q.fin.cx = C.cx, Q.fin.cy = C.cy, Q.fin.rows = C.rows, Q.fin.ncols = C.cols;
+    Q.fin.owner = C.owner, Q.fin.tag = C.tag, Q.fin.ys = C.ys;
+    if (B.want_zsum) hipLaunchKernelGGL((refine_rf_persist_kernel<6, true>), dim3(grid), dim3(kFB), 0, c->stream, A, Q);
+    else hipLaunchKernelGGL((refine_rf_persist_kernel<6, false>), dim3(grid), dim3(kFB), 0, c->stream, A, Q);
+    RSDSFM_HIP_CHECK(c, hipGetLastError());
+    return RSDSFM_OK;
+}
+
 int refine_rf_apply_launch(Ctx* c, const RefineBuffers& B, int np, int g, bool to_published, const double* rows_all, int nranks, int64_t m_total,
                            const int64_t* m_total_dev) {
     const RfLayout Lo = rf_layout(c, B);
diff --git a/rs-aware-differential-sfm_amd/csrc/refine_rf_later_loop.hpp b/rs-aware-differential-sfm_amd/csrc/refine_rf_later_loop.hpp
--- /dev/null
+++ b/rs-aware-differential-sfm_amd/csrc/refine_rf_later_loop.hpp
@@ -0,0 +1,86 @@
+        RfPoint Pq = rf_point(st->p), Pcq = rf_point(st->pc);
+        const RfPoint P = rf_point_uniform(Pq), Pc = rf_point_uniform(Pcq);
+        double dp[7];
+#pragma unroll
+        for (int c = 0; c < 7; ++c) dp[c] = uniform_d(st->dp[c]);
+        const double inv_radius = uniform_d(1.0 / st->radius);
+        const double psi = uniform_d(1.0 / (1.0 + 1.0 / st->radius));
+        const double* __restrict__ rho = st->cur ? A.rho_b : A.rho_a;
+        double* __restrict__ cand = st->cur ? A.rho_a : A.rho_b;
+        auto body = [&](const RfLoad& l0, int64_t i) {
+            const double x = l0.c4.x, y = l0.c4.y, ux = l0.c4.z, uy = l0.c4.w, rh = l0.rho;
+            const RfGeom g = rf_geom(x, y);
+            double be, dbe, bec, dbec, be0, dbe0;
+            rf_beta<NP>(l0.ab, l0.ak, P, be, dbe);
+            rf_beta<NP>(l0.ab, l0.ak, Pc, bec, dbec);
+            rf_beta<NP>(l0.ab, l0.ak, P0, be0, dbe0);
+            RfEval<NP> o;
+            rf_resid<NP>(g, ux, uy, be, P, rh, o);
+            double da0, da1, db0, db1;
+            rf_av(g, dp[0], dp[1], dp[2], da0, da1);
+            rf_bw(g, dp[3], dp[4], dp[5], db0, db1);
+            double t0 = be * __builtin_fma(rh, da0, db0), t1 = be * __builtin_fma(rh, da1, db1);
+            if (NP == 7) {
+                const double dk = dbe * dp[6];
+                t0 = __builtin_fma(dk, o.in0, t0);
+                t1 = __builtin_fma(dk, o.in1, t1);
+            }
+            double a00, a10;
+            rf_av(g, P0.v0, P0.v1, P0.v2, a00, a10);
+            const double h0 = (be0 * be0) * __builtin_fma(a00, a00, a10 * a10);
+            const double gJ = __builtin_fma(o.J0, o.r0, o.J1 * o.r1), tJ = __builtin_fma(o.J0, t0, o.J1 * t1);
+            const bool flagged = rf_flagged(o.h, h0);
+            double drho = -((psi * (gJ + tJ)) * rcp_core(flagged ? 1.0 : o.h));
+            if (__builtin_amdgcn_ballot_w64(flagged) != 0) {
+                if (flagged) {
+                    asm volatile("; listed inlier: exact e-block inverse" ::: "memory");
+                    double sr, E0, E1;
+                    const double ete_inv = rf_ete_inv_exact(o.J0, o.J1, h0, inv_radius, sr, E0, E1);
+                    drho = -((ete_inv * (sr * (gJ + tJ))) * sr);
+                }
+            }
+            const double m0 = __builtin_fma(o.J0, drho, t0), m1 = __builtin_fma(o.J1, drho, t1);
+            acc[RR::MODEL] -= __builtin_fma(m0, __builtin_fma(0.5, m0, o.r0), m1 * __builtin_fma(0.5, m1, o.r1));
+            const double cd = rh + drho;
+            cand[i] = cd;
+            acc[RR::STEPSQ] = __builtin_fma(drho, drho, acc[RR::STEPSQ]);
+            RfEval<NP> oc;
+            rf_resid<NP>(g, ux, uy, bec, Pc, cd, oc);
+            rf_jac<NP>(g, bec, dbec, cd, oc);
+            acc[RR::COST2] = __builtin_fma(oc.r0, oc.r0, __builtin_fma(oc.r1, oc.r1, acc[RR::COST2]));
+            acc[RR::GMAX] = fmax(acc[RR::GMAX], fabs(__builtin_fma(oc.J0, oc.r0, oc.J1 * oc.r1)));
+            acc[RR::XSQ] = __builtin_fma(cd, cd, acc[RR::XSQ]);
+            if (ZSUM) acc[RR::ZSUM] += 1.0 / cd;
+            const bool flagged_c = rf_flagged(oc.h, h0);
+            const double ihm = flagged_c ? 0.0 : rcp_core(flagged_c ? 1.0 : oc.h);
+            rf_schur_accumulate<NP>(oc, ihm, acc, lds_c);
+            if (flagged_c) rf_list_append(A.list_count, A.list_entries, x, y, ux, uy, l0.ab, l0.ak, cd, i);
+        };
+        const int64_t last = m - 1;
+        if (NP == 6) {
+            RfLoad l0 = rf_load<NP>(A, rho, i0, i0 <= last);
+            RfLoad l1 = rf_load<NP>(A, rho, i0 + stride, i0 + stride <= last);
+            for (int64_t i = i0; i < m; i += stride) {
+                const int64_t i2 = i + 2 * stride;
+                const RfLoad l2 = rf_load<NP>(A, rho, i2, i2 <= last);
+#if RF_LOADS_ONLY
+                acc[0] += l0.c4.x + l0.c4.y + l0.c4.z + l0.c4.w + l0.rho + l0.ab;
+                cand[i] = l0.rho;
+#else
+                body(l0, i);
+#endif
+                l0 = l1;
+                l1 = l2;
+            }
+        } else {
+#if RF_NP7_PREFETCH == 1
+            RfLoad l0 = rf_load<NP>(A, rho, i0, i0 <= last);
+            for (int64_t i = i0; i < m; i += stride) {
+                const RfLoad l1 = rf_load<NP>(A, rho, i + stride, i + stride <= last);
+                body(l0, i);
+                l0 = l1;
+            }
+#else
+            for (int64_t i = i0; i < m; i += stride) body(rf_load<NP>(A, rho, i, true), i);
+#endif
+        }
diff --git a/rs-aware-differential-sfm_amd/csrc/rsdsfm_internal.hpp b/rs-aware-differential-sfm_amd/csrc/rsdsfm_internal.hpp
--- a/rs-aware-differential-sfm_amd/csrc/rsdsfm_internal.hpp
+++ b/rs-aware-differential-sfm_amd/csrc/rsdsfm_internal.hpp
@@ -182,6 +182,9 @@
     int refine_arithmetic = 0;
     int64_t refine_rf_runs = 0, refine_rf_restarts = 0, refine_rf_resolves = 0;
     int refine_rf_last_guard = 0;
+    int refine_persist = 0;
+    int64_t refine_persist_runs = 0, refine_persist_trips = 0;
+    int refine_persist_fits[2] = {-1, -1};
     struct RansacCache {
         uint64_t tag = 0, stage_gen = 0;
         const double *d_u = nullptr, *d_inl = nullptr, *d_alpha = nullptr, *d_alpha_k = nullptr;
@@ -426,6 +429,7 @@
     int32_t rf_guard, rf_resolves;
 };
 constexpr int kTermRestartExact = 64;
+constexpr int kTermRestartLaunches = 65;
 struct FinishClaim {
     bool on = false;
     double fx = 0.0, fy = 0.0, cx = 0.0, cy = 0.0;
@@ -433,6 +437,7 @@
     int32_t* ys = nullptr;
     unsigned* owner = nullptr;
     unsigned tag = 0, mask = 0;
+    bool persist_ok = false;
 };
 struct RefineBuffers {
     const double* flow;
@@ -531,6 +536,8 @@
     RefineBuffers B;
     int np = 6, launched = 0, chunk = 5, hint_prev = -1;
     bool rf = false;
+    bool persist = false;
+    int first_grid_cap = 0;
     double* d_inl_out = nullptr;
     const RefineTail* tail = nullptr;
     RefineState* hs = nullptr;
@@ -545,6 +552,8 @@
                  void* ws_base, RefineRun* run, RefineState* hs_prefetch, double* d_zpartials, bool exact = false,
                  const FinishClaim* claim = nullptr, const FrameHandoff* handoff = nullptr);
 constexpr int kRcRefineRestartExact = 1;
+constexpr int kRcRefineRestartLaunches = 2;
+constexpr unsigned long long kRfPersistWaitTicks = 200000ull;
 int refine_device(Ctx* c, const double* d_flow, int64_t n_flow, int64_t m, const double* d_inl, const double* d_alpha,
                   const double* d_alpha_k, const int64_t* d_inlier_idx, const double v_in[3], const double w_in[3], double k_in,
                   int const_acceleration, int flow_index_mode, double* d_inl_out, double v_out[3], double w_out[3], double* k_out,
@@ -567,6 +576,9 @@
                            const int64_t* m_total_dev);
 int refine_rf_row_launch(Ctx* c, const RefineBuffers& B, int np, int g, double* row);
 int refine_rf_row_doubles(int np);
+bool refine_rf_persist_fits(Ctx* c, int np, bool want_zsum);
+int refine_rf_grid_cap(const Ctx* c);
+int refine_rf_persist_launch(Ctx* c, const RefineBuffers& B, int np, double* inl_out, int first_grid_cap, unsigned long long wait_ticks);
 void refine_rf_debug_dump(Ctx* c, const RefineBuffers& B);
 int refine_rf_read_stamps(Ctx* c, unsigned long long out[16]);
 int refine_rf_extra_doubles();
diff --git a/rsdsfm_refine_persist.py b/rsdsfm_refine_persist.py
--- /dev/null
+++ b/rsdsfm_refine_persist.py
@@ -0,0 +1,17 @@
+import ctypes as C
+
+import rsdsfm
+
+REFINE_PERSIST_MODES = (0, 1, 2)
+
+
+def set_refine_persist(solver, mode):
+    if int(mode) not in REFINE_PERSIST_MODES:
+        raise rsdsfm.RsdsfmError("refine persist mode must be 0 (persistent where eligible), 1 (one launch per iteration) or 2 (0 with the wait limit at zero)")
+    solver._check(solver.lib.rsdsfm_set_refine_persist(solver._ctx, C.c_int(int(mode))), "rsdsfm_set_refine_persist")
+
+
+def refine_persist_stats(solver):
+    runs, trips = C.c_int64(0), C.c_int64(0)
+    solver._check(solver.lib.rsdsfm_refine_persist_stats(solver._ctx, C.byref(runs), C.byref(trips)), "rsdsfm_refine_persist_stats")
+    return dict(runs=runs.value, trips=trips.value)
```

Result: slower. 1846 (-7.3%).
